# yozhijk/capsaicin

Measured on AMD Instinct MI355X. Metric: Mrays/sec (primary+secondary), cornell_box 1080p 64spp, higher is better.
Workload: dtype f32; 1 GPU; cornell_box.obj 1920x1080 64spp depth=8 (reference shading: Lambert + directional light + sky), tile-sharded over 1 GPU(s); triangles=32, bvh_depth=8, parallelism=tiles1, exchange=none

## Files before the change

### capsaicin_amd/capi.py

```python
import ctypes as C
import os
import subprocess

import numpy as np

_PKG = os.path.dirname(os.path.abspath(__file__))
_ROOT = os.path.dirname(_PKG)
LIB_PATH = os.path.join(_PKG, "libcapsaicin_hip.so")
if os.environ.get("CAP_LIB_VARIANT"):
    LIB_PATH = os.path.join(_PKG, "variants", "libcapsaicin_hip_%s.so" % os.environ["CAP_LIB_VARIANT"])

RENDER_AOV = 1
RENDER_EXT_MATERIALS = 2
RENDER_STAGE_TIMERS = 4
RENDER_GBUFFER_FEEDBACK = 8
RENDER_LOWRES_INDIRECT = 16

BUF_GBUFFER_GEO, BUF_DIRECT, BUF_ALBEDO, BUF_NORMAL_DEPTH, BUF_INDIRECT, BUF_COMBINED, BUF_ACCUM_SUM, BUF_ACCUM_MEAN, BUF_INDIRECT_LOWRES = range(9)


class CapError(RuntimeError):
    pass


# ... 502 lines not shown
        t = np.ascontiguousarray(rgba8, np.uint8)
        assert t.size == 256 * 256 * 4
        _check(lib().cap_bluenoise_upload(self.ctx, _p(t)), "cap_bluenoise_upload")

    def upload_materials(self, materials):
        m = np.ascontiguousarray(materials, np.float32).reshape(-1, 12)
        _check(lib().cap_materials_upload(self.ctx, _p(m), m.shape[0]), "cap_materials_upload")

    BVH_BUILD_AUTO, BVH_BUILD_LBVH, BVH_BUILD_SAH, BVH_BUILD_PLOC, BVH_BUILD_SAH_DEVICE = 0, 1, 2, 3, 4

    def set_bvh_build(self, mode):
        _check(lib().cap_set_bvh_build(self.ctx, mode), "cap_set_bvh_build")

    def build_bvh(self):
        _check(lib().cap_bvh_build(self.ctx), "cap_bvh_build")
        return self.bvh_info()

    def update_vertices(self, positions=None, normals=None, texcoords=None):
        ptrs, flags, keep = vertex_update_args(self._vertex_count, positions, normals, texcoords)
        if flags:
            import torch
            dev = torch.device("cuda", self.device)
            for a in keep:
                if a.device != dev:
                    raise CapError("update_vertices: tensors must be on %s, got %s" % (dev, a.device))
            torch.cuda.current_stream(dev).synchronize()
        _check(lib().cap_scene_update_vertices(self.ctx, ptrs[0], ptrs[1], ptrs[2], flags), "cap_scene_update_vertices")

    def refit_bvh(self):
        info = RefitInfo()
        _check(lib().cap_bvh_refit(self.ctx, C.byref(info)), "cap_bvh_refit")
        return info

    def bvh_info(self):
        bi = BvhInfo()
        _check(lib().cap_bvh_info(self.ctx, C.byref(bi)), "cap_bvh_info")
        return bi

    def bvh_readback(self):
        bi = self.bvh_info()
        nodes = np.zeros((bi.node_count, 16), np.float32)
        leaves = np.zeros(bi.triangle_count, np.uint32)
        _check(lib().cap_bvh_readback(self.ctx, _p(nodes), _p(leaves)), "cap_bvh_readback")
        return nodes, leaves

    def bvh_wide_readback(self):
        info = np.zeros(3, np.uint32)
        _check(lib().cap_bvh_wide_readback(self.ctx, None, None, _p(info)), "cap_bvh_wide_readback")
        nodes = np.zeros((int(info[0]), 20), np.uint32)
        src = np.zeros(max(1, self.bvh_info().triangle_count), np.uint32)
        _check(lib().cap_bvh_wide_readback(self.ctx, _p(nodes), _p(src), _p(info)), "cap_bvh_wide_readback")
        return nodes, src[:self.bvh_info().triangle_count], int(info[1]), int(info[2])

    def bvh_wide_info(self):
        info = np.zeros(3, np.uint32)
        _check(lib().cap_bvh_wide_readback(self.ctx, None, None, _p(info)), "cap_bvh_wide_readback")
        return int(info[0]), int(info[1]), int(info[2])

    def set_camera(self, cam):
        _check(lib().cap_camera_set(self.ctx, C.byref(cam)), "cap_camera_set")

    def set_prev_camera(self, cam):
        _check(lib().cap_prev_camera_set(self.ctx, C.byref(cam)), "cap_prev_camera_set")

    def set_resolution(self, width, height):
        _check(lib().cap_set_resolution(self.ctx, width, height), "cap_set_resolution")
        self.width, self.height = width, height

    def set_shard(self, index, count):
        _check(lib().cap_set_shard(self.ctx, index, count), "cap_set_shard")

    def set_traversal(self, mode):
        _check(lib().cap_set_traversal(self.ctx, mode), "cap_set_traversal")

    DEBUG_QUEUE_CAPACITY_DIV, DEBUG_WIDE_DEPTH_LIMIT, DEBUG_WIDE_IN_USE, DEBUG_FAIL_LANE1, DEBUG_LANES_USED = 1, 2, 3, 4, 5
    DEBUG_QUEUE_CANARY_FILL, DEBUG_QUEUE_CANARY_BEHIND, DEBUG_QUEUE_CANARY_USED, DEBUG_SELFTEST_DIV, DEBUG_NEE_PAIRS = 6, 7, 8, 9, 10
    DEBUG_SELFTEST_SHADE_UNARY, DEBUG_SELFTEST_SHADE_DIV2, DEBUG_SHADE_TAME = 11, 12, 13
    DEBUG_CAMERA_CULL = 14
    DEBUG_MARK_FORM = 15
    DEBUG_SAMPLE_TABLE = 16
    DEBUG_SELFTEST_SAMPLE_TABLE = 17
    DEBUG_CAMERA_TABLE = 18
    DEBUG_SELFTEST_CAMERA_TABLE = 19

    def debug_set(self, key, value):
        _check(lib().cap_debug_set(self.ctx, key, value), "cap_debug_set")

    DEBUG_SWITCH_BASE = 64

    def debug_switch(self, name, value):
        i = lib().cap_debug_switch_index(name.encode())
        if i < 0:
            raise CapError("unknown switch %s" % name)
        self.debug_set(self.DEBUG_SWITCH_BASE + i, 0xFFFFFFFFFFFFFFFF if value is None else int(value))

    def debug_get(self, key):
        v = _u64()
        _check(lib().cap_debug_get(self.ctx, key, C.byref(v)), "cap_debug_get")
        return int(v.value)

    def set_batch_paths(self, n):
        _check(lib().cap_set_batch_paths(self.ctx, n), "cap_set_batch_paths")

    def render(self, frame_begin, n_frames, num_bounces, flags=0):
        _check(lib().cap_render(self.ctx, frame_begin, n_frames, num_bounces, flags), "cap_render")

    def accum_reset(self):
        _check(lib().cap_accum_reset(self.ctx), "cap_accum_reset")

    def accum_import(self, sum_rgba, frames):
        a = np.ascontiguousarray(sum_rgba, np.float32)
        assert a.shape == (self.height, self.width, 4)
        _check(lib().cap_accum_import(self.ctx, _p(a), int(frames)), "cap_accum_import")

    def sync(self):
        _check(lib().cap_sync(self.ctx), "cap_sync")

    def readback(self, kind):
        if kind == BUF_INDIRECT_LOWRES:
            out = np.zeros((self.height // 2, self.width // 2, 4), np.float32)
        else:
            out = np.zeros((self.height, self.width, 4), np.float32)
        _check(lib().cap_readback(self.ctx, kind, _p(out)), "cap_readback")
        return out

    def stats(self):
        s = Stats()
        _check(lib().cap_stats_get(self.ctx, C.byref(s)), "cap_stats_get")
        return s

    def stats_reset(self):
        _check(lib().cap_stats_reset(self.ctx), "cap_stats_reset")

    RAY_FLAG_ACCEPT_FIRST_HIT, RAY_FLAG_CULL_BACK_FACING, RAY_FLAG_CULL_FRONT_FACING = 0x04, 0x10, 0x20

    def set_instance_masks(self, masks):
        if masks is None:
            _check(lib().cap_scene_set_instance_masks(self.ctx, None, len(self._tri_end)), "cap_scene_set_instance_masks")
            return
        m = np.ascontiguousarray(masks, np.uint8).reshape(-1)
        _check(lib().cap_scene_set_instance_masks(self.ctx, _p(m), m.size), "cap_scene_set_instance_masks")

    def trace_options(self, cull=None, mask=None, first_hit=False):
        if cull not in (None, "back", "front"):
            raise CapError('cull must be None, "back" or "front", got %r' % (cull,))
        if cull is None and mask is None and not first_hit:
            return None
        flags = {None: 0, "back": self.RAY_FLAG_CULL_BACK_FACING, "front": self.RAY_FLAG_CULL_FRONT_FACING}[cull]
        if first_hit:
            flags |= self.RAY_FLAG_ACCEPT_FIRST_HIT
        return TraceOptions(flags, 0 if mask is None else int(mask))

    MULTI_MAX_K, MULTI_CONTINUE = 16, 1

    def _stage_records(self, records, width, what):
        import torch
        dev = torch.device("cuda", self.device)
        if isinstance(records, np.ndarray):
            records = torch.from_numpy(np.ascontiguousarray(records, np.float32).reshape(-1, width)).to(dev)
        if records.dtype != torch.float32 or records.dim() != 2 or records.shape[1] != width or not records.is_contiguous() or records.device != dev:
            raise CapError("%s must be a contiguous (N, %d) float32 tensor on %s, got %s %s on %s"
                           % (what, width, dev, records.dtype, tuple(records.shape), records.device))
        return dev, records, records.shape[0]

    def _out(self, out, shape, dtype, dev):
        host_out = None
# ... 391 lines not shown
```

### capsaicin_amd/csrc/cap_context.h

```cpp
#pragma once

#include <array>
#include <string>
#include <utility>
#include <vector>

#include "../../include/capsaicin_hip.h"

#include "cap_kernels.h"

namespace cap
{
int fail(int code, const char* fmt, ...);

#define HIP_TRY(expr)                                                                                         \
    do                                                                                                        \
    {                                                                                                         \
        hipError_t e_ = (expr);                                                                               \
        if (e_ != hipSuccess) return fail(CAP_ERR_HIP, "%s failed: %s (%s:%d)", #expr, hipGetErrorString(e_), \
                                          __FILE__, __LINE__);                                                \
    } while (0)

template <typename T>
struct DevBuf
// ... 111 lines not shown
    DevBuf<float4>   shade_tris, tris_sorted, nodes, tri_raw, tri_box;
    DevBuf<float4>   nodes8, tris8;
    DevBuf<uint32_t> wide_src;
    DevBuf<uint32_t> wide_task, wide_alloc, wide_cnt;
    uint32_t         wide8_depth = 0, wide8_top = 0, wide8_nodes = 0;
    float            wide8_ms = 0.f;
    DevBuf<uint32_t> query_work, query_defer;
    DevBuf<uint8_t>  tri_mask;
    bool             tri_mask_on = false;
    DevBuf<float4>   inst_desc, inst_rec, inst_box, inst_tlas;
    DevBuf<uint32_t> inst_keys[2], inst_vals[2], inst_hist, inst_scan, inst_misc, inst_level_off;
    uint32_t         inst_count = 0, inst_top = 0, inst_nodes = 0;
    DevBuf<float2>   inst_near;
    DevBuf<uint32_t> inst_obj;
    bool             inst_obj_on = false;
    InstObject       scene_object_host{};
    DevBuf<InstObject> scene_object;
    std::vector<CapObjectInfo> obj_info;
    std::vector<uint32_t>      obj_node_base, obj_rec_base;
    uint32_t                   obj_count = 0, obj_max_depth = 0;
    DevBuf<float4>             forest_nodes, forest_tris;
    DevBuf<InstObject>         obj_table;
    DevBuf<float4>             obj_tri_raw, obj_tri_box;
    DevBuf<uint32_t>           obj_leaf_tri, obj_misc;
    DevBuf<float4>   fan_pairs, fan_singles;
    uint32_t         fan_pair_count = 0, fan_single_count = 0;
    DevBuf<float4>   fan_pairs_nee;
    uint32_t         fan_pair_nee_count = 0;
    std::vector<float>    fan_pairs_host;
    std::vector<uint32_t> light_tris_host;
    DevBuf<uint32_t> leaf_tri, keys0, keys1, vals0, vals1, hist, parent, flags, bvh_misc;
    DevBuf<float4>   ploc_boxes;
    DevBuf<uint32_t> ploc_ints;
    DevBuf<uint32_t> sahdev_words;
    CapBvhInfo       bvh_info{};
    bool             shade_tame = false;
    bool             bvh_ready = false;
    DevBuf<float>        pn_table;
    bool                 pn_ready = false;
    CapPseudonormalsInfo pn_info{};
    DevBuf<float4>       wn_table;
    bool                 wn_ready = false;
    CapWindingInfo       wn_info{};
    DevBuf<double>       wn_root;
    DevBuf<float4>       wi_inst, wi_top, wi_forest;
    DevBuf<double>       wi_top_sums, wi_obj_root, wi_reals;
    DevBuf<uint32_t>     wi_words, wi_count;
    bool                 wi_dirty = true, wi_forest_dirty = true;
    bool                 wi_built = false;
    bool                  bvh_stale = false;
    bool                  positions_host_stale = false;
    bool                  visits_built_known = false;
    double                refit_visits_built = 0.0;
    std::vector<uint32_t> wide_levels;
    DevBuf<float>         wide_boxes;
    DevBuf<double>        refit_sums;

    CapCameraData camera{}, prev_camera{};
    bool          camera_ready = false, prev_camera_ready = false;
    ScreenDev     screen{};
    uint64_t      max_batch_paths = 0;
    SwitchTable   sw{};
    uint32_t      debug_capacity_div = 1;
    uint32_t      debug_wide_depth_limit = 0;
    bool          debug_fail_lane = false;
    uint64_t      lane1_failed_paths = 0;
    uint32_t      lane1_failed_bounces = 0, lane1_retry_tick = 0;
    uint32_t      lanes_last_render = 0;
    uint32_t      last_class_capacity = 0;
    uint32_t      tri_ids_dense = 0;
    uint32_t      last_mark_form = 0;
    uint32_t      last_sample_table = 0;
    struct LastTerms
    {
        const FrameConst* frames = nullptr;
        uint32_t          n_slots = 0, num_bounces = 0, lane = 0;
    } last_terms;
    uint32_t      last_camera_table = 0;
    struct LastCamera
    {
        const FrameConst* frames = nullptr;
        uint32_t          n_slots = 0, n_groups = 0, lane = 0;
    } last_camera;
    uint32_t      last_cull_camera_pairs = 0;
    uint32_t      traversal_mode  = CAP_TRAVERSAL_AUTO;
    uint32_t      bvh_build_mode  = CAP_BVH_BUILD_AUTO;

    DevBuf<float4>     aov_geo, aov_nd, accum, image_tmp;
    DevBuf<uint64_t>   shaded_counter;
    struct Lane
    {
        hipStream_t      stream = nullptr;
        DevBuf<float4>   hits, q_org[2], q_dir[2], q_thr[2], s_org, s_dir, s_con, pl_color, pl_direct, pl_albedo;
        DevBuf<float4>   camera;
        DevBuf<float4>   terms;
        DevBuf<uint32_t> counters;
        DevBuf<uint32_t> stack_spill;
    } lane[2];
    hipStream_t stream2 = nullptr;
    hipEvent_t  lane_ev[2] = {nullptr, nullptr}, fork_ev = nullptr, join_ev = nullptr;
    static constexpr int kFrameRing = 4;
    DevBuf<FrameConst> frames_ring[kFrameRing];
    FrameConst*        frames_pinned[kFrameRing] = {nullptr, nullptr, nullptr, nullptr};
    size_t             frames_pinned_n[kFrameRing] = {0, 0, 0, 0};
    hipEvent_t         frames_event[kFrameRing] = {nullptr, nullptr, nullptr, nullptr};
    uint32_t           frames_next = 0;
    uint32_t           last_slots = 0;
    bool               aov_valid = false;
    bool               aov_lowres = false;
    uint32_t           aov_frame  = 0;
    uint64_t           frames_accumulated = 0;

    DevBuf<float4> post_in[4];
    DevBuf<float4> post_ihist[2], post_mhist[2], post_chist[2], post_prev_nd, post_itemp, post_temp[2], post_normals;
    uint32_t       post_w = 0, post_h = 0;
    int            post_last_dst = -1;

    void*           comm = nullptr;
    uint32_t        comm_rank = 0, comm_size = 0;
    bool            comm_local = false;
    DevBuf<float>   comm_send, comm_gathered, comm_image;
    hipEvent_t      comm_event = nullptr;

    CapStats               stats{};
    std::vector<TimedSpan> spans;
    std::vector<std::array<hipEvent_t, 6>> post_marks;
    std::vector<hipEvent_t> event_pool;
    std::vector<uint32_t*> pinned_pool;
    std::vector<std::pair<uint32_t*, BatchCounted>> pending;
    uint64_t*              pinned_shaded = nullptr;
};

namespace cap
{
struct AovPlanes
{
    const float4 *color, *direct, *albedo;
};

int        sync_and_collect(CapContext* c);
hipEvent_t get_event(CapContext* c);
CameraDev  camera_dev(const CapCameraData& cd);
SceneDev   scene_dev(const CapContext* c);
BvhDev     bvh_dev(const CapContext* c, const CapContext::Lane& lane);
AovPlanes  aov_planes(const CapContext* c);
int        trace_launch(const CapContext* c, const char* fmt, ...);
void       launch_texture_footprints(hipStream_t stream, const uint32_t* src, uint4* dst, uint32_t width, uint32_t height);
bool pair_ids_dense(const float* pairs, uint32_t pair_count, uint32_t single_count, uint32_t tri_count);
int  upload_fan_records(CapContext* c);
int  update_nee_pairs(CapContext* c);
int  ensure_positions_host(CapContext* c);
int  upload_light_table(CapContext* c);
int query_state(CapContext* c, const char* what);
int  winding_instances_ensure(CapContext* c, const char* what);
void winding_instances_release(CapContext* c);
}
```

### capsaicin_amd/csrc/cap_kernels.h

```cpp
#pragma once

#include "cap_device.h"

#include <cstdio>
#include <vector>

namespace cap
{
enum CapSwitch : uint32_t
{
    SW_NO_WIDE8 = 0,
    SW_LANE1_PRIORITY,
    SW_PLOC_RADIUS,
    SW_SAHDEV_LEAF,
    SW_WIDE_HOST_COLLAPSE,
    SW_TRACE_LAUNCHES,
    SW_NO_TWO_LANES,
    SW_LANE_SPLIT_MIN,
    SW_BLOCKS_PER_CU,
    SW_NO_CAMERA_CULL,
    SW_NO_ALBEDO_IN_W,
    SW_NO_INLINE_NEE,
    SW_NO_INLINE_PROBE,
    SW_NO_WAVE_RING,
    SW_ANY_REFILL,
    SW_PRIMARY_WIDE,
    SW_NO_PACKET,
    SW_NO_ANY_PROBE,
    SW_ANY_PROBE,
    SW_ANY_BLOCKS,
    SW_NO_PRIMARY_FUSE,
    SW_W8_REFILL,
    SW_W8_GRID,
    SW_AUTO_SAH_TRIANGLES,
    SW_NO_NEE_PAIR_CULL,
    SW_RAYGEN_KERNEL,
    SW_NO_PLANE_CODE,
    SW_SAMPLE_TABLE,
    SW_NO_CAMERA_TABLE,
    SW_COUNT
};
struct SwitchTable
{
    int64_t v[SW_COUNT];
    bool    on(CapSwitch k) const { return v[k] > 0; }
    int64_t get(CapSwitch k, int64_t dflt) const { return v[k] >= 0 ? v[k] : dflt; }
};

struct LaunchCfg
{
    hipStream_t stream;
    uint32_t    grid_blocks;
    uint32_t    stack_entries;
    uint32_t    cu_count = 0;
    uint32_t    any_no_probe = 0;
    const SwitchTable* sw = nullptr;
    bool    sw_on(CapSwitch k) const { return sw && sw->on(k); }
    int64_t sw_get(CapSwitch k, int64_t dflt) const { return sw ? sw->get(k, dflt) : dflt; }
};

template <auto K>
uint32_t resident_grid(const LaunchCfg& cfg, uint32_t want)
{
    static int per_cu = -1;
    if (per_cu < 0)
    {
        int n = 0;
        per_cu = (hipOccupancyMaxActiveBlocksPerMultiprocessor(&n, K, (int)kBlock, 0) == hipSuccess && n > 0) ? n : 0;
        if (cfg.sw_on(SW_TRACE_LAUNCHES)) fprintf(stderr, "[cap] resident workgroups per CU: %d\n", per_cu);
    }
    if (!cfg.cu_count || !per_cu) return want;
    const uint32_t cap = cfg.cu_count * (uint32_t)per_cu;
    return want < cap ? want : cap;
}
inline uint32_t queue_grid(const LaunchCfg& cfg, uint32_t max_count)
{
    uint32_t g = (max_count + kBlock - 1) / kBlock;
    if (g > cfg.grid_blocks) g = cfg.grid_blocks;
    return g ? g : 1;
}

void launch_trace_primary(const LaunchCfg& cfg, const BvhDev& bvh, const CameraDev& cam, const ScreenDev& screen,
                          const FrameConst* frames, uint32_t n_slots, float4* hits, uint32_t* work);
void launch_raygen_identity(const LaunchCfg& cfg, const CameraDev& cam, const ScreenDev& screen, const FrameConst* frames, uint32_t n_slots,
                            const RayQueue& q);
void launch_trace_closest(const LaunchCfg& cfg, const BvhDev& bvh, const RayQueue& q, uint32_t max_count, float4* hits);
void launch_trace_closest8(const LaunchCfg& cfg, const BvhDev& bvh, const RayQueue& q, uint32_t max_count, float4* hits, uint32_t* work);
void launch_trace_closest8_camera(const LaunchCfg& cfg, const BvhDev& bvh, const RayQueue& q, uint32_t max_count, float4* hits, uint32_t* work,
                                  const CameraDev& cam, const ScreenDev& screen, const FrameConst* frames, uint32_t n_slots);
void launch_trace_any(const LaunchCfg& cfg, const BvhDev& bvh, const ShadowQueue& q, uint32_t max_count, float4* target,
                      uint32_t pixels_padded, uint32_t n_slots, uint64_t* guard, uint32_t* work, bool mostly_unoccluded,
                      const FrameConst* frames, float4* code_plane = nullptr);

void launch_trace_any8_refill(const LaunchCfg& cfg, const BvhDev& bvh, const ShadowQueue& q, uint32_t max_count, float4* target, uint32_t pixels_padded,
                              uint32_t n_slots, uint64_t* guard, uint32_t* work, const FrameConst* frames);

struct QueryArgs
{
    const float4* rays;
    uint32_t      n;
    void*         out;
    uint32_t*     work;
    uint32_t*     defer;
    float         safe;
};
constexpr float kQuerySafeScale = 4.0f;
bool query8_stack_matches();
struct RayFilter;
void launch_query8(const LaunchCfg& cfg, const BvhDev& bvh, const QueryArgs& q, bool any, const RayFilter* f = nullptr, bool first_hit = false);
void launch_query_binary(const LaunchCfg& cfg, const BvhDev& bvh, const QueryArgs& q, bool any, bool deferred);
struct MultiArgs
{
    QueryArgs q;
    uint32_t  k;
    uint32_t* counts;
    uint32_t  resume;
};
constexpr uint32_t kMultiMaxK = 16;
uint32_t multi_bucket(uint32_t k);
void     launch_query8_multi(const LaunchCfg& cfg, const BvhDev& bvh, const MultiArgs& m, const RayFilter* f = nullptr);
void     launch_query_binary_multi(const LaunchCfg& cfg, const BvhDev& bvh, const MultiArgs& m, bool deferred, const RayFilter* f = nullptr);

// ... 50 lines not shown
void launch_closest_instances_multi(const LaunchCfg& cfg, const BvhDev& bvh, const ClosestInstMultiArgs& m, const TlasDev& tl, const RayFilter& f,
                                    uint32_t depth);

struct InstObject
{
    double   blo[3], bhi[3];
    int32_t  root;
    uint32_t reserved;
};
struct InstanceBuildArgs
{
    const float*      descs;
    uint32_t          n;
    const InstObject* objects;
    uint32_t          n_objects;
    const uint32_t*   object_index;
    float4*      rec;
    float4*      box;
    float4*      tlas;
    float2*      near;
    uint32_t*    keys[2];
    uint32_t*    vals[2];
    uint32_t*    hist;
    uint32_t*    scan;
    uint32_t*    misc;
};
constexpr uint32_t kTlasMaxLevels = 25;
uint32_t tlas_layout(uint32_t n, uint32_t level_off[kTlasMaxLevels], uint32_t* total);
void     launch_instances_build(hipStream_t stream, const InstanceBuildArgs& a);
struct TlasDev
{
    const float4*   rec;
    const float4*   tlas;
    const uint32_t* level_off;
    uint32_t        top;
};
void launch_query_instances(const LaunchCfg& cfg, const BvhDev& bvh, const QueryArgs& q, const TlasDev& tl, const RayFilter& f, int mode, uint32_t* inst_out,
                            uint32_t depth);
void launch_query_instances_multi(const LaunchCfg& cfg, const BvhDev& bvh, const MultiArgs& m, const TlasDev& tl, const RayFilter& f, uint32_t* inst_out,
                                  uint32_t depth);
struct ForestRelocArgs
{
    float4*  nodes;
    float4*  tris;
    uint32_t n_tris, node_base, rec_base, first_triangle;
};
void launch_forest_relocate(hipStream_t stream, const ForestRelocArgs& a);

struct ShadeArgs
{
    SceneDev          scene;
    CameraDev         cam;
    ScreenDev         screen;
    const FrameConst* frames;
    union
    {
        const float4* hits;
        const float4* sample_terms;
    };
    RayQueue          in;
    RayQueue          out;
    ShadowQueue       shadow;
    Planes            planes;
    uint32_t          n_slots;
    uint32_t          bounce;
    uint32_t          num_bounces;
    uint32_t          max_count;
    uint32_t          aov_slot;
    uint64_t*         shaded_counter;
    uint32_t*         work;
    FeedbackDev       fb;
    uint32_t          albedo_in_w;
    uint32_t          inline_nee;
    uint32_t          inline_probe;
    uint32_t          wave_ring;
    uint32_t          cull_camera_pairs;
    uint32_t          code_in_color;
};
constexpr float kCodePadding = 0.f, kCodeSky = 1.f, kCodeKd = 2.f, kCodeBlack = 3.f;
constexpr float kCodeLit = 4.f;
constexpr float kCameraCullPad = 2.0f;
void launch_shade(const LaunchCfg& cfg, const ShadeArgs& args, bool ext, bool feedback = false);
bool launch_primary_shade(const LaunchCfg& cfg, const BvhDev& bvh, const ShadeArgs& args, float4* hits, bool ext);
uint32_t launch_trace_shade(const LaunchCfg& cfg, const BvhDev& bvh, const ShadeArgs& args, bool ext, bool feedback = false, bool camera_head = false);
bool trace_shade_has_code_form(const BvhDev& bvh, const SceneDev& scene);
bool trace_shade_has_table_form(const BvhDev& bvh, const SceneDev& scene);
void launch_sample_terms(hipStream_t stream, const float2* bluenoise, const FrameConst* frames, uint32_t n_slots, uint32_t num_bounces, float4* table);
void launch_sample_terms_selftest(hipStream_t stream, const float2* bluenoise, const FrameConst* frames, uint32_t n_slots, uint32_t num_bounces,
                                  const float4* table, unsigned long long* out_device);

void launch_camera_vertices(const LaunchCfg& cfg, const BvhDev& bvh, const ShadeArgs& args, uint32_t rows, float4* tab_p, float4* tab_n,
                            unsigned long long* selftest_out = nullptr);

void launch_resolve(const LaunchCfg& cfg, const Planes& planes, uint32_t n_slots, uint32_t pixels_padded, float4* accum,
                    bool albedo_in_w = false, float kd_untextured = 0.0f, bool code_in_color = false);
void launch_untile(const LaunchCfg& cfg, const ScreenDev& screen, const float4* src, const float4* albedo, const float4* direct,
                   int plane_kind, float4* image);
void launch_tile(const LaunchCfg& cfg, const ScreenDev& screen, const float4* image, float4* dst);
void launch_untile4(const LaunchCfg& cfg, const ScreenDev& screen, const float4* s0, const float4* s1, const float4* s2, const float4* s3,
                    float4* d0, float4* d1, float4* d2, float4* d3);
void launch_tiles_mean(const LaunchCfg& cfg, const float4* accum, uint32_t pixels_padded, float4* dst);
void launch_assemble(const LaunchCfg& cfg, const ScreenDev& screen, const float4* gathered, uint32_t shard_count, float4* image,
                     size_t shard_stride = 0);
void launch_geo_aov(const LaunchCfg& cfg, const SceneDev& scene, const float4* hits_slot, uint32_t pixels_padded, float4* aov_geo);

struct BvhBuildArgs
{
    const float*    positions;
    const float*    normals;
    const float*    texcoords;
    const uint32_t* indices;
    const uint4*    tri_ids;
    const uint4*    mesh_offsets;
    uint32_t        tri_count;
    float4*         shade_tris;
    float4*         tris_sorted;
    float4*         nodes;
    uint32_t*       leaf_tri;
    float4*         tri_raw;
    float4*         tri_box;
    uint32_t*       keys[2];
    uint32_t*       vals[2];
    uint32_t*       hist;
    uint32_t*       parent;
    uint32_t*       flags;
    uint32_t*       bounds;
    uint32_t*       max_depth;
};
size_t bvh_radix_blocks(uint32_t n);
void   launch_bvh_build(hipStream_t stream, const BvhBuildArgs& a);
int    launch_bvh_sort(hipStream_t stream, const BvhBuildArgs& a);
size_t bvh_radix_scan_words(uint32_t n);
int    launch_radix_sort_pairs(hipStream_t stream, uint32_t* const keys[2], uint32_t* const vals[2], uint32_t n, uint32_t* hist, uint32_t* scan);
size_t bvh_scan_scratch_words(uint32_t total);
void   launch_exclusive_scan_u32(hipStream_t stream, uint32_t* v, uint32_t total, uint32_t* scratch);
struct PlocScratch
{
    float4*   boxes;
    uint32_t* ints;
};
int    launch_bvh_build_ploc(hipStream_t stream, const BvhBuildArgs& a, const PlocScratch& s, uint32_t radius);
size_t bvh_sah_device_scratch_words(uint32_t n);
int    launch_bvh_build_sah_device(hipStream_t stream, const BvhBuildArgs& a, const PlocScratch& s, uint32_t* scratch, uint32_t radius, uint32_t leaf);
void launch_bvh_setup(hipStream_t stream, const BvhBuildArgs& a);
void launch_bvh_finish_host(hipStream_t stream, const BvhBuildArgs& a);

void     launch_gather_wide(hipStream_t stream, const uint32_t* tri_src, const float4* tris_sorted, uint32_t n, float4* tris8);
struct WideCollapseArgs
{
    const float4*   bnodes;
    const uint32_t* count;
    uint32_t        n_tris, capacity;
    double          pad;
    uint32_t *      task, *alloc, *nodes8, *tri_src;
    uint32_t*       cnt;
    uint32_t        begin, end;
};
int      launch_wide_collapse(hipStream_t stream, WideCollapseArgs a, uint32_t* node_count, uint32_t* depth, uint32_t* top_nodes,
                          std::vector<uint32_t>* level_begin = nullptr);
struct PseudonormalArgs
{
    const float*    positions;
    const uint32_t* indices;
    const uint4*    tri_ids;
    const uint4*    mesh_offsets;
    uint32_t        tri_count;
    float*          table;
    uint32_t *      kx, *ky, *kz;
    uint32_t*       keys[2];
// ... 112 lines not shown
```

### capsaicin_amd/csrc/cap_shade.h

```cpp
#pragma once

#include "cap_exhaustive.h"
#include "cap_kernels.h"
#include "cap_reproject.h"
#include "cap_unscaled.h"

namespace cap
{
__device__ __forceinline__ void bluenoise4x4(const float2* tex, uint32_t x, uint32_t y, uint32_t count, float& s0, float& s1)
{
    const uint32_t px = (count % 16u) % 4u, py = (count % 16u) / 4u;
    const uint32_t sx = (x * 4u + px) % 256u, sy = (y * 4u + py) % 256u;
    const float2   t  = tex[sy * 256u + sx];
    const float    k  = 0.61803398875f * (float)(count / 16u);
    const float    a = t.x + k, b = t.y + k;
    s0 = a - floorf(a);
    s1 = b - floorf(b);
}

__device__ __forceinline__ v3 ortho_vector(v3 n)
{
    const bool  zn = fabsf(n.z) > 0.0f;
    const float a = zn ? n.z : n.y, b = zn ? n.y : n.x;
    const float k = sqrtf(fmaf(a, a, b * b));
// ... 48 lines not shown
    const bool fast = false;
#else
    const bool  fast = __ballot(!ortho_in_range(a, b, g)) == 0ull;
#endif
    float       q1, q2;
    if (fast)
        div2_unscaled(a, b, sqrt_pos(g), q1, q2);
    else
    {
        const float k = sqrtf(g);
        q1 = a / k, q2 = b / k;
    }
    v3       u = zn ? mk3(0.0f, -q1, q2) : mk3(q1, -q2, 0.0f);
    const v3 v = cross3(u, n);
    u          = cross3(n, v);
    const HemiTerms h = terms();
    const float     cos_theta = h.cos_theta, ca = h.ca, cb = h.cb;
    const v3    d = mk3(fmaf(n.x, cos_theta, fmaf(v.x, cb, u.x * ca)), fmaf(n.y, cos_theta, fmaf(v.y, cb, u.y * ca)),
                        fmaf(n.z, cos_theta, fmaf(v.z, cb, u.z * ca)));
    return fast ? normalize3_tame(d) : normalize3(d);
}
__device__ __forceinline__ v3 map_to_hemisphere_tame(float r1, float r2, v3 n)
{
    return hemisphere_dir_tame(n, [=] { return hemisphere_terms(r1, r2); });
}

__device__ __forceinline__ void oct_encode(v3 n, float& ox, float& oy)
{
    const float s = fabsf(n.x) + fabsf(n.y) + fabsf(n.z);
    n             = mk3(n.x / s, n.y / s, n.z / s);
    ox = n.x, oy = n.y;
    if (!(n.z >= 0.0f))
    {
        ox = (1.0f - fabsf(n.y)) * (n.x >= 0.0f ? 1.0f : -1.0f);
        oy = (1.0f - fabsf(n.x)) * (n.y >= 0.0f ? 1.0f : -1.0f);
    }
    ox = ox * 0.5f + 0.5f;
    oy = oy * 0.5f + 0.5f;
}

__device__ __forceinline__ uint32_t wrap_texel(float f, uint32_t n)
{
    const float m = f - floorf(f / (float)n) * (float)n;
    int         i = (int)m;
    if (i < 0) i = 0;
    if ((uint32_t)i >= n) i = 0;
    return (uint32_t)i;
}

__device__ __forceinline__ v3 sample_texture(const TextureDev& tex, float u, float v)
{
    const float    fx = fmaf(u, (float)tex.width, -0.5f), fy = fmaf(v, (float)tex.height, -0.5f);
    const float    x0f = floorf(fx), y0f = floorf(fy);
    const float    wx = fx - x0f, wy = fy - y0f;
    const uint32_t x0 = wrap_texel(x0f, tex.width), y0 = wrap_texel(y0f, tex.height);
    const uint4  fq   = reinterpret_cast<const uint4*>(tex.quads)[y0 * tex.width + x0];
    auto         rgba = [](uint32_t wd) { return make_uchar4((uint8_t)wd, (uint8_t)(wd >> 8), (uint8_t)(wd >> 16), (uint8_t)(wd >> 24)); };
    const uchar4 c00 = rgba(fq.x), c10 = rgba(fq.y), c01 = rgba(fq.z), c11 = rgba(fq.w);
    auto unorm8 = [](uint8_t b) {
        const float r = 1.0f / 255.0f, fb = (float)b, q = fb * r;
        return fmaf(fmaf(-q, 255.0f, fb), r, q);
    };
    auto           lerp2 = [&](uint8_t a00, uint8_t a10, uint8_t a01, uint8_t a11) {
        const float f00 = unorm8(a00), f10 = unorm8(a10), f01 = unorm8(a01), f11 = unorm8(a11);
        const float top = fmaf(f10 - f00, wx, f00);
        const float bot = fmaf(f11 - f01, wx, f01);
        return fmaf(bot - top, wy, top);
    };
    return mk3(lerp2(c00.x, c10.x, c01.x, c11.x), lerp2(c00.y, c10.y, c01.y, c11.y), lerp2(c00.z, c10.z, c01.z, c11.z));
}

__device__ __forceinline__ uint32_t wave_append(bool emit, uint32_t* counter)
{
    const unsigned long long mask = __ballot(emit);
    if (mask == 0ull) return 0;
    const uint32_t lane   = threadIdx.x & 63u;
    const uint32_t leader = (uint32_t)__ffsll((long long)mask) - 1u;
    uint32_t       base   = 0;
    if (lane == leader) base = atomicAdd(counter, (uint32_t)__popcll(mask));
    base = __shfl(base, (int)leader);
    return base + (uint32_t)__popcll(mask & ((1ull << lane) - 1ull));
}

struct ShadePre
{
    bool  valid;
    v3    L, I;
    float r1, r2;
    float r3, r4, r5, r6;
    float r1n, r2n;
    bool  indirect_on;
};

__device__ __forceinline__ void stage_frames(const ShadeArgs& a, FrameConst* lds_frames)
{
    const uint32_t  words = a.n_slots * (uint32_t)(sizeof(FrameConst) / 4);
    const uint32_t* src   = reinterpret_cast<const uint32_t*>(a.frames);
    uint32_t*       dst   = reinterpret_cast<uint32_t*>(lds_frames);
    for (uint32_t i = threadIdx.x; i < words; i += kBlock) dst[i] = src[i];
    __syncthreads();
}

#if defined(CAP_CHUNK_PLAIN)
constexpr bool kChunkLean = false;
#else
constexpr bool kChunkLean = true;
#endif

#pragma clang diagnostic push
#pragma clang diagnostic ignored "-Wuninitialized"
__device__ __forceinline__ float unread_f()
{
    float x;
    return x;
}
#pragma clang diagnostic pop
__device__ __forceinline__ v3 unread3() { return mk3(unread_f(), unread_f(), unread_f()); }

struct SlotSample
{
    uint32_t off;
    float    k;
};
__device__ __forceinline__ uint32_t bluenoise_offset(uint32_t count) { return (((count % 16u) / 4u) << 8) | ((count % 16u) % 4u); }
__device__ __forceinline__ float    bluenoise_shift(uint32_t count) { return 0.61803398875f * (float)(count / 16u); }
__device__ __forceinline__ uint32_t bluenoise_base(uint32_t x, uint32_t y) { return ((y & 63u) << 10) | ((x & 63u) << 2); }
__device__ __forceinline__ void     bluenoise_at(const float2* tex, uint32_t base, uint32_t off, float k, float& s0, float& s1)
{
    const float2 t = tex[base | off];
    const float  a = t.x + k, b = t.y + k;
    s0 = a - floorf(a);
    s1 = b - floorf(b);
}
template <bool FIRST, bool TAB = false>
__device__ __forceinline__ void stage_frames_samples(const ShadeArgs& a, FrameConst* lds_frames, SlotSample* lds_first)
{
    constexpr uint32_t kWords = (uint32_t)(sizeof(FrameConst) / 4);
    static_assert(kWords == 12 && offsetof(FrameConst, frame_count) == 8 && offsetof(FrameConst, pad1) == 28 && offsetof(FrameConst, pad2) == 44, "FrameConst layout");
    const uint32_t  words = (a.n_slots < kMaxFrameSlots ? a.n_slots : kMaxFrameSlots) * kWords;
    const uint32_t* src   = reinterpret_cast<const uint32_t*>(a.frames);
    uint32_t*       dst   = reinterpret_cast<uint32_t*>(lds_frames);
    for (uint32_t i = threadIdx.x; i < kMaxFrameSlots * kWords; i += kBlock)
    {
        uint32_t v = 0u;
        if (i < words)
        {
            const uint32_t sl = i / kWords, w = i - sl * kWords;
            v = src[i];
            if (!TAB && (w == 7u || w == 11u))
            {
                const uint32_t next = src[sl * kWords + 2u] * 25u + a.bounce + 1u;
                v = w == 7u ? bluenoise_offset(next) : f2u(bluenoise_shift(next));
            }
        }
        dst[i] = v;
    }
    if (FIRST && !TAB)
        for (uint32_t sl = threadIdx.x; sl < kMaxFrameSlots; sl += kBlock)
        {
            SlotSample ss = {0u, 0.0f};
            if (sl < a.n_slots)
            {
                const uint32_t count = a.frames[sl].frame_count * 25u + a.bounce;
                ss.off = bluenoise_offset(count), ss.k = bluenoise_shift(count);
            }
            lds_first[sl] = ss;
// ... 81 lines not shown
        }
    }
    return s;
}

__device__ __forceinline__ void wave_append2(bool& emit_ext, bool& emit_shadow, uint32_t* counter_pair, uint32_t& ext_slot,
                                             uint32_t& shadow_slot, uint32_t capacity, uint64_t* guard)
{
    const unsigned long long me = __ballot(emit_ext), ms = __ballot(emit_shadow);
    ext_slot = shadow_slot = 0;
    if ((me | ms) == 0ull) return;
    const uint32_t lane   = threadIdx.x & 63u;
    const uint32_t leader = (uint32_t)__ffsll((long long)(me | ms)) - 1u;
    uint32_t       lo = 0, hi = 0;
    if (lane == leader)
    {
        const unsigned long long add = ((unsigned long long)__popcll(ms) << 32) | (unsigned long long)__popcll(me);
        const unsigned long long old = atomicAdd(reinterpret_cast<unsigned long long*>(counter_pair), add);
        lo = (uint32_t)old, hi = (uint32_t)(old >> 32);
    }
    lo = __shfl(lo, (int)leader), hi = __shfl(hi, (int)leader);
    const unsigned long long below = (1ull << lane) - 1ull;
    ext_slot    = lo + (uint32_t)__popcll(me & below);
    shadow_slot = hi + (uint32_t)__popcll(ms & below);
    if (lo + (uint32_t)__popcll(me) > capacity || hi + (uint32_t)__popcll(ms) > capacity)
    {
        if (lane == leader)
        {
            atomicAdd((unsigned long long*)guard + 4, 1ull);
            guard[3] = ((uint64_t)lo << 32) | hi;
        }
        emit_ext    = emit_ext && ext_slot < capacity;
        emit_shadow = emit_shadow && shadow_slot < capacity;
    }
}

#ifdef CAP_STAMPS
static __device__ unsigned long long g_stamps[16];
struct Stamps
{
    unsigned long long last, acc[8], t_begin;
    __device__ void    start()
    {
        for (int i = 0; i < 8; ++i) acc[i] = 0;
        last    = __builtin_amdgcn_s_memtime();
        t_begin = __builtin_amdgcn_s_memrealtime();
    }
    __device__ void mark(int i, bool wait)
    {
#ifdef CAP_STAMPS_PHASES
        if (wait) __builtin_amdgcn_s_waitcnt(0);
        const unsigned long long now = __builtin_amdgcn_s_memtime();
        acc[i] += now - last;
        last = now;
#endif
    }
    __device__ void flush()
    {
        if ((threadIdx.x & 63u) == 0)
            for (int i = 0; i < 8; ++i) atomicAdd(&g_stamps[i], acc[i]);
    }
};
#define STAMP(st, i, wait) (st).mark(i, wait)
#else
struct Stamps
{
    __device__ void start() {}
    __device__ void flush() {}
};
#define STAMP(st, i, wait) ((void)0)
#endif

struct ProbeArgs
{
    const float4* rows  = nullptr;
    const float4* pairs = nullptr;
    uint32_t      k     = 0;
    float4*       ring_org = nullptr;
    float4*       ring_con = nullptr;
};
constexpr uint32_t kWaveRing = 128;
template <class C>
__device__ __forceinline__ void shade_vertex(const ShadeArgs& a, const float4* shade_tab, const ShadePre& pre, uint32_t klass,
                                             uint32_t pid, float4 hit, v3 thr, uint32_t& n_shaded, Stamps& st,
                                             const ProbeArgs probe = ProbeArgs(), uint32_t* n_probed = nullptr, uint32_t ring_head = 0,
                                             uint32_t* ring_n = nullptr)
{
    const uint32_t Ppad = a.screen.pixels_padded;
    const uint32_t slot = pid >> kPidShift, pl = pid & kPidMask;
    {
        const size_t plane_idx = (size_t)slot * Ppad + pl;
        bool         valid = pre.valid;
        if (valid && (slot >= a.n_slots || pl >= Ppad))
        {
            atomicAdd((unsigned long long*)a.shaded_counter + 1, 1ull);
            a.shaded_counter[3] = ((uint64_t)a.bounce << 32) | pid;
            valid = false;
        }
        const uint32_t gid = f2u(hit.z);

        bool   emit_shadow = false, emit_ext = false;
        v3     p = mk3(0, 0, 0), dir = mk3(0, 0, 0), contrib = mk3(0, 0, 0);
        if constexpr (C::LEAN) p = unread3(), dir = unread3(), contrib = unread3();

        if (C::FIRST && !valid)
        {
            a.planes.color[plane_idx]  = make_float4(0, 0, 0, 0);
            if (!C::CODE) a.planes.direct[plane_idx] = make_float4(0, 0, 0, 0);
            if (!C::CODE && !a.albedo_in_w) a.planes.albedo[plane_idx] = make_float4(0, 0, 0, 0);
        }
        if (valid && gid == kInvalidId)
        {
            if (C::FIRST)
            {
                a.planes.color[plane_idx]  = make_float4(0.f, 0.f, 0.f, 1.f);
                if (!C::CODE) a.planes.direct[plane_idx] = make_float4(0.7f, 0.7f, 0.85f, 1.f);
                if (!C::CODE && !a.albedo_in_w) a.planes.albedo[plane_idx] = make_float4(1.f, 1.f, 1.f, 1.f);
                if (slot == a.aov_slot) a.planes.aov_normal_depth[pl] = make_float4(0.f, 0.f, 0.f, 0.f);
            }
            else
            {
                if (C::SKY_RMW)
                {
                    const float4 cur = a.planes.color[plane_idx];
                    a.planes.color[plane_idx] = make_float4(cur.x + thr.x * 0.7f, cur.y + thr.y * 0.7f, cur.z + thr.z * 0.85f, cur.w);
                }
                else
                {
                    float* c = reinterpret_cast<float*>(a.planes.color + plane_idx);
                    atomicAdd(c + 0, thr.x * 0.7f);
                    atomicAdd(c + 1, thr.y * 0.7f);
                    atomicAdd(c + 2, thr.z * 0.85f);
                }
            }
        }
        else if (valid)
        {
            ++n_shaded;
            const float4* tab = shade_tab + kShadeRec * (size_t)gid;
            const float4  s0 = tab[0], s1 = tab[1], s2 = tab[2], s3 = tab[3], s4 = tab[4], s5 = tab[5];
            const float   u = hit.x, v = hit.y, w = (1.0f - u) - v;
            auto          mix = [&](float c0, float c1, float c2) { return fmaf(c2, v, fmaf(c1, u, c0 * w)); };
            const v3      nm = mk3(mix(s3.x, s4.x, s5.x), mix(s3.y, s4.y, s5.y), mix(s3.z, s4.z, s5.z));
            const v3      n  = C::TAME ? normalize3_tame(nm) : normalize3(nm);
            p = mk3(mix(s0.x, s1.x, s2.x), mix(s0.y, s1.y, s2.y), mix(s0.z, s1.z, s2.z));
            v3       kd   = mk3(a.scene.kd_untextured, a.scene.kd_untextured, a.scene.kd_untextured);
            uint32_t inst = 0;
            if (a.scene.texture_count != 0 || (C::FIRST && slot == a.aov_slot))
            {
                const float4 idf   = tab[6];
                inst               = f2u(idf.x);
                const uint32_t tex = f2u(idf.z);
                if (tex != kInvalidId && tex < a.scene.texture_count)
                {
                    const float tu = mix(s0.w, s2.w, s4.w), tv = mix(s1.w, s3.w, s5.w);
                    const v3    c  = sample_texture(a.scene.textures[tex], tu, 1.0f - tv);
                    kd             = mk3(pow22_c(c.x), pow22_c(c.y), pow22_c(c.z));
                }
            }
            const bool black = kd.x < 1e-5f && kd.y < 1e-5f && kd.z < 1e-5f;
            if (C::FIRST)
            {
                if (C::CODE)
                    a.planes.color[plane_idx] = make_float4(0.f, 0.f, 0.f, black ? kCodeBlack : kCodeKd);
                else
                {
                    a.planes.color[plane_idx]  = make_float4(0.f, 0.f, 0.f, 1.f);
                    a.planes.direct[plane_idx] = make_float4(0.f, 0.f, 0.f, a.albedo_in_w ? (black ? kCodeBlack : kCodeKd) : 1.f);
                }
                if (!C::CODE && !a.albedo_in_w) a.planes.albedo[plane_idx] = black ? make_float4(0.f, 0.f, 0.f, 0.f) : make_float4(kd.x, kd.y, kd.z, 1.f);
                if (slot == a.aov_slot)
                {
                    float4 nd = make_float4(0.f, 0.f, 0.f, 0.f);
                    if (!black)
                    {
                        oct_encode(n, nd.x, nd.y);
                        nd.z = (float)inst;
                        nd.w = length3(mk3(a.cam.position[0], a.cam.position[1], a.cam.position[2]) - p);
                    }
                    a.planes.aov_normal_depth[pl] = nd;
                }
            }
            bool reused = false;
            if (C::FB && !C::FIRST && !black)
            {
                const uint32_t W = a.screen.width, H = a.screen.height;
                const f2       puv = image_plane_uv(a.fb.prev_cam, p);
                if (puv.x >= 0.0f && puv.y >= 0.0f && puv.x <= 1.0f && puv.y <= 1.0f)
                {
                    const f2    pxy        = uv_to_xy(puv, W, H);
                    const float prev_depth = ldi(Img{a.fb.prev_normal_depth, W, H}, (int)pxy.x, (int)pxy.y).w;
                    const float cur_depth =
                        length3(p - mk3(a.fb.prev_cam.position[0], a.fb.prev_cam.position[1], a.fb.prev_cam.position[2]));
                    if (!(fabsf(prev_depth - cur_depth) / cur_depth > 0.05f))
                    {
                        reused        = true;
                        const v3 hc   = sample_bilinear(Img{a.fb.color_history, W, H}, puv);
                        const float4 cur = a.planes.color[plane_idx];
                        a.planes.color[plane_idx] = make_float4(cur.x + thr.x * hc.x, cur.y + thr.y * hc.y, cur.z + thr.z * hc.z, cur.w);
                    }
                }
            }
            if (!black && !reused)
            {
                const float ndl = fmaxf(0.0f, dot3(n, pre.L));
                v3          c   = mk3(((pre.I.x * kd.x) * kInvPi) * ndl, ((pre.I.y * kd.y) * kInvPi) * ndl, ((pre.I.z * kd.z) * kInvPi) * ndl);
                if (c.x != 0.0f || c.y != 0.0f || c.z != 0.0f)
                {
                    emit_shadow = true;
                    contrib     = C::FIRST ? c : thr * c;
                }
                const bool more = a.bounce < a.num_bounces;
                if (!C::TAME || more)
                {
                    if constexpr (C::TAB)
                        dir = hemisphere_dir_tame(n, [&] { return HemiTerms{pre.r1, pre.r2, pre.r1n}; });
                    else
                        dir = C::TAME ? map_to_hemisphere_tame(pre.r1, pre.r2, n) : map_to_hemisphere(pre.r1, pre.r2, n);
                    const float ndd = dot3(n, dir);
                    const float pdf = C::TAME ? div_unscaled(fmaxf(0.0f, ndd), kPi) : fmaxf(0.0f, ndd) / kPi;
                    if (!(pdf < 1e-5f))
                    {
                        const float fn = kInvPi * fmaxf(ndd, 0.0f);
                        const float f  = C::TAME ? div_unscaled(fn, pdf) : fn / pdf;
                        thr            = thr * f;
                        if (!C::FIRST) thr = thr * kd;
                        emit_ext = more && (!C::FIRST || pre.indirect_on);
                    }
                }
            }
        }

        if (C::PROBE)
        {
            if (probe.rows != nullptr)
            {
                const Ray    sr  = make_ray(p, pre.L, kRayEps, kRayFar);
                const uint32_t ps = valid ? slot : 0u;
                const float4   pa = probe.rows[2u * ps], pb = probe.rows[2u * ps + 1u];
                const bool   occluded = pair_occludes_pre(sr, probe.pairs, probe.k, pa, pb);
                if (emit_shadow && occluded) emit_shadow = false, ++*n_probed;
            }
        }
        uint32_t ei, si;
        STAMP(st, 2, true);
        wave_append2(emit_ext, emit_shadow, a.out.count + klass * kCounterStride, ei, si, a.out.class_capacity, a.shaded_counter);
        STAMP(st, 3, true);
        ei += klass * a.out.class_capacity;
        si += klass * a.shadow.class_capacity;
        if (C::PROBE && probe.ring_org != nullptr)
        {
            const unsigned long long ms = __ballot(emit_shadow);
            if (emit_shadow)
            {
                const uint32_t lane_ = threadIdx.x & 63u;
                const uint32_t pos   = (ring_head + *ring_n + (uint32_t)__popcll(ms & ((1ull << lane_) - 1ull))) & (kWaveRing - 1u);
                probe.ring_org[pos]  = make_float4(p.x, p.y, p.z, u2f(pid));
                probe.ring_con[pos]  = make_float4(contrib.x, contrib.y, contrib.z, 0.0f);
            }
            *ring_n += (uint32_t)__popcll(ms);
            __builtin_amdgcn_fence(__ATOMIC_RELEASE, "wavefront");
        }
        else if (emit_shadow)
        {
            a.shadow.org_tmin[si]    = make_float4(p.x, p.y, p.z, u2f(pid));
            a.shadow.contrib_pid[si] = make_float4(contrib.x, contrib.y, contrib.z, C::CODE ? kCodeKd : 0.0f);
        }
        if (emit_ext)
        {
            a.out.org_tmin[ei] = make_float4(p.x, p.y, p.z, C::CARRY ? pre.r1n : kRayEps);
            a.out.dir_tmax[ei] = make_float4(dir.x, dir.y, dir.z, C::CARRY ? pre.r2n : kRayFar);
            a.out.thr_pid[ei]  = make_float4(thr.x, thr.y, thr.z, u2f(pid));
        }
    }
}

struct ExtBsdf
{
    v3    f;
    float pdf_spec, pdf_diff;
};

__device__ __forceinline__ float lum3(v3 c) { return fmaf(c.z, 0.114f, fmaf(c.y, 0.587f, c.x * 0.299f)); }

struct ExtView
{
    float cos_o, lam_o;
};
__device__ __forceinline__ ExtView ext_view(float a2, v3 nf, v3 wo)
{
    ExtView w;
    w.cos_o = dot3(nf, wo);
    w.lam_o = w.cos_o + sqrtf(fmaf(1.0f - a2, w.cos_o * w.cos_o, a2));
    return w;
}
__device__ __forceinline__ ExtBsdf ext_bsdf(v3 kd, v3 ks, float a2, v3 nf, v3 wo, v3 wi, const ExtView& vw)
{
    const float cos_i = dot3(nf, wi);
    const v3    h     = normalize3(wo + wi);
    const float cos_h = dot3(nf, h), woh = dot3(wo, h);
    const float dd    = fmaf(cos_h * cos_h, a2 - 1.0f, 1.0f);
    const float pdd   = kPi * dd * dd;
    const float lam_i = cos_i + sqrtf(fmaf(1.0f - a2, cos_i * cos_i, a2));
#if defined(CAP_EXT_DIAG) && CAP_EXT_DIAG == 3
    const float spec  = 0.0f * (vw.cos_o + woh);
#else
    const float spec  = a2 / (pdd * (vw.lam_o * lam_i));
#endif
    ExtBsdf     r;
    r.f        = mk3(kd.x * kInvPi + ks.x * spec, kd.y * kInvPi + ks.y * spec, kd.z * kInvPi + ks.z * spec);
    r.pdf_spec = (a2 * cos_h) / (pdd * (4.0f * woh));
    r.pdf_diff = cos_i * kInvPi;
    return r;
}

struct ExtTables
{
    const MaterialDev* materials  = nullptr;
    const float*       light_cdf  = nullptr;
    const float4*      light_rec  = nullptr;
};
constexpr uint32_t kExtLightsMax = 32;

template <bool FIRST, bool INLINE = false>
__device__ __forceinline__ void shade_vertex_ext(const ShadeArgs& a, const float4* shade_tab, const ShadePre& pre, uint32_t klass,
                                                 uint32_t pid, float4 hit, v3 thr,
                                                 v3 d, uint32_t& n_shaded, const BvhDev* bvh = nullptr, v3 acc = mk3(0.f, 0.f, 0.f),
                                                 const ExtTables tabs = ExtTables())
{
    const uint32_t Ppad = a.screen.pixels_padded;
    const uint32_t slot = pid >> kPidShift, pl = pid & kPidMask;
    const size_t   plane_idx = (size_t)slot * Ppad + pl;
    bool           valid = pre.valid;
    if (valid && (slot >= a.n_slots || pl >= Ppad))
    {
        atomicAdd((unsigned long long*)a.shaded_counter + 1, 1ull);
        a.shaded_counter[3] = ((uint64_t)a.bounce << 32) | pid;
        valid = false;
    }
    const uint32_t gid = f2u(hit.z);
    bool  emit_shadow = false, emit_ext = false;
    v3    p = mk3(0, 0, 0), dir = mk3(0, 0, 0), contrib = mk3(0, 0, 0), sdir = mk3(0, 0, 1), first_ke = mk3(0, 0, 0);
    float stmax = 0.0f;

    if (FIRST && !valid)
    {
        a.planes.color[plane_idx]  = make_float4(0, 0, 0, 0);
        a.planes.direct[plane_idx] = make_float4(0, 0, 0, 0);
        if (!a.albedo_in_w) a.planes.albedo[plane_idx] = make_float4(0, 0, 0, 0);
    }
    if (valid && gid == kInvalidId)
// ... 182 lines not shown
```

### capsaicin_amd/csrc/context.hip

```cpp
#include <algorithm>
#include <cmath>
#include <cstdarg>
#include <cstdio>
#include <cstdlib>
#include <cstring>

#include "cap_context.h"
#include "cap_near.h"
#include "cap_wide.h"
#include "query_ranges.h"

namespace
{
thread_local std::string g_error;
}

namespace cap
{
int fail(int code, const char* fmt, ...)
{
    char    buf[512];
    va_list ap;
    va_start(ap, fmt);
    vsnprintf(buf, sizeof(buf), fmt, ap);
// ... 149 lines not shown

int trace_launch(const CapContext* c, const char* fmt, ...)
{
    if (!c->sw.on(SW_TRACE_LAUNCHES)) return CAP_OK;
    va_list ap;
    va_start(ap, fmt);
    fputs("[cap] ", stderr);
    vfprintf(stderr, fmt, ap);
    va_end(ap);
    fputs(" ... ", stderr);
    fflush(stderr);
    hipError_t e = hipStreamSynchronize(c->stream);
    fprintf(stderr, "%s\n", hipGetErrorString(e));
    fflush(stderr);
    return e == hipSuccess ? CAP_OK : CAP_ERR_HIP;
}
}

namespace
{
void update_screen(CapContext* c, uint32_t w, uint32_t h, uint32_t shard_index, uint32_t shard_count)
{
    ScreenDev& s  = c->screen;
    s.width       = w;
    s.height      = h;
    s.tiles_x     = (w + kTileDim - 1) / kTileDim;
    s.tiles_y     = (h + kTileDim - 1) / kTileDim;
    s.tile_count  = s.tiles_x * s.tiles_y;
    s.shard_index = shard_index;
    s.shard_count = shard_count ? shard_count : 1;
    const uint32_t max_local = (s.tile_count + s.shard_count - 1) / s.shard_count;
    s.local_tiles   = s.tile_count > s.shard_index ? (s.tile_count - s.shard_index + s.shard_count - 1) / s.shard_count : 0;
    s.pixels_padded = max_local * kTilePixels;
    tile_div_setup(s.tiles_x, s.tiles_x_mul, s.tiles_x_shift);
    c->frames_accumulated = 0;
    c->aov_valid = false;
}

template <size_t N, class Launch>
int count_on_device(CapContext* c, unsigned long long (&h)[N], Launch launch)
{
    DevBuf<unsigned long long> d;
    HIP_TRY(d.ensure(N));
    HIP_TRY(hipMemsetAsync(d.p, 0, sizeof(h), c->stream));
    launch(d.p);
    HIP_TRY(hipGetLastError());
    HIP_TRY(hipMemcpyAsync(h, d.p, sizeof(h), hipMemcpyDeviceToHost, c->stream));
    HIP_TRY(hipStreamSynchronize(c->stream));
    return CAP_OK;
}
}

__global__ __launch_bounds__(256) void k_texture_footprints(const uint32_t* src, uint4* dst, uint32_t width, uint32_t height)
{
    const size_t i = (size_t)blockIdx.x * 256 + threadIdx.x;
    if (i >= (size_t)width * height) return;
    const uint32_t y = (uint32_t)(i / width), x = (uint32_t)(i - (size_t)y * width);
    const uint32_t x1 = x + 1 == width ? 0 : x + 1, y1 = y + 1 == height ? 0 : y + 1;
    dst[i] = make_uint4(src[(size_t)y * width + x], src[(size_t)y * width + x1], src[(size_t)y1 * width + x], src[(size_t)y1 * width + x1]);
}

void cap::launch_texture_footprints(hipStream_t stream, const uint32_t* src, uint4* dst, uint32_t width, uint32_t height)
{
    const size_t texels = (size_t)width * height;
    hipLaunchKernelGGL(k_texture_footprints, dim3((unsigned)((texels + 255) / 256)), dim3(256), 0, stream, src, dst, width, height);
}

extern "C" {

const char* cap_last_error(void) { return g_error.c_str(); }
void cap_set_error_(const char* msg) { g_error = msg ? msg : ""; }

int cap_device_count(void)
{
    int n = 0;
    if (hipGetDeviceCount(&n) != hipSuccess) return 0;
    return n;
}

static const char* const kSwitchNames[SW_COUNT] = {
    "CAP_NO_WIDE8", "CAP_LANE1_PRIORITY", "CAP_PLOC_RADIUS", "CAP_SAHDEV_LEAF", "CAP_WIDE_HOST_COLLAPSE", "CAP_TRACE_LAUNCHES", "CAP_NO_TWO_LANES",
    "CAP_LANE_SPLIT_MIN", "CAP_BLOCKS_PER_CU", "CAP_NO_CAMERA_CULL", "CAP_NO_ALBEDO_IN_W", "CAP_NO_INLINE_NEE", "CAP_NO_INLINE_PROBE", "CAP_NO_WAVE_RING",
    "CAP_ANY_REFILL", "CAP_PRIMARY_WIDE", "CAP_NO_PACKET", "CAP_NO_ANY_PROBE", "CAP_ANY_PROBE", "CAP_ANY_BLOCKS", "CAP_NO_PRIMARY_FUSE", "CAP_W8_REFILL",
    "CAP_W8_GRID", "CAP_AUTO_SAH_TRIANGLES", "CAP_NO_NEE_PAIR_CULL", "CAP_RAYGEN_KERNEL", "CAP_NO_PLANE_CODE", "CAP_SAMPLE_TABLE", "CAP_NO_CAMERA_TABLE"};

static void switches_from_environment(SwitchTable& t)
{
    for (uint32_t k = 0; k < SW_COUNT; ++k)
    {
        const char* e = getenv(kSwitchNames[k]);
        t.v[k]        = -1;
        if (!e) continue;
        char*           end = nullptr;
        const long long v   = strtoll(e, &end, 10);
        t.v[k]              = (end != e && v >= 0) ? v : 1;
    }
    if (getenv("CAP_BVH_BINARY") && t.v[SW_NO_WIDE8] < 0) t.v[SW_NO_WIDE8] = 1;
}

int cap_debug_switch_index(const char* name)
{
    for (uint32_t k = 0; name && k < SW_COUNT; ++k)
        if (strcmp(name, kSwitchNames[k]) == 0) return (int)k;
    return -1;
}

extern "C" int cap_debug_tile_divmod(uint32_t tiles_x, const uint32_t* n, uint64_t count, uint32_t* quotient, uint32_t* remainder)
{
    if (!tiles_x || !n || !quotient || !remainder) return CAP_ERR_INVALID_ARG;
    uint32_t mul, shift;
    tile_div_setup(tiles_x, mul, shift);
    for (uint64_t k = 0; k < count; ++k)
    {
        quotient[k]  = tile_div(n[k], mul, shift);
        remainder[k] = n[k] - quotient[k] * tiles_x;
    }
    return CAP_OK;
}

int cap_debug_pair_ids_dense(const float* pair_records, uint32_t pair_count, uint32_t single_count, uint32_t tri_count)
{
    if (!pair_records && pair_count) return 0;
    return pair_ids_dense(pair_records, pair_count, single_count, tri_count) ? 1 : 0;
}

int cap_debug_query_ranges(uint64_t n, uint32_t count, const uint64_t* base, const uint64_t* stride, const uint32_t* align)
{
    static const char* const names[4] = {"range 0", "range 1", "range 2", "range 3"};
    if (count > 4 || (count && (!base || !stride || !align))) return fail(CAP_ERR_INVALID_ARG, "cap_debug_query_ranges: at most 4 ranges, no NULL array");
    QueryRange r[4];
    for (uint32_t i = 0; i < count; ++i)
    {
        if (!align[i] || (align[i] & (align[i] - 1u))) return fail(CAP_ERR_INVALID_ARG, "cap_debug_query_ranges: align[%u] is not a power of two", i);
        r[i] = QueryRange{names[i], (uintptr_t)base[i], stride[i], align[i], stride[i] != 0};
    }
    char msg[256];
    return query_ranges_ok("cap_debug_query_ranges", n, r, count, msg, sizeof(msg)) ? CAP_OK : fail(CAP_ERR_INVALID_ARG, "%s", msg);
}

int cap_debug_closest_instance_bound(const float* transform, const float* box_lo, const float* box_hi, const float* point, float best_dist2,
                                     float* world_to_object, float* g, float* xw, float* slack, uint32_t* skip)
{
    if (!transform || !box_lo || !box_hi || !point) return fail(CAP_ERR_INVALID_ARG, "cap_debug_closest_instance_bound: NULL input");
    double m[12], w[12], wd[12], A[12], nA, kappa, blo[3], bhi[3];
    float  wf[12];
    bool   live = true;
    for (int k = 0; k < 12; ++k) m[k] = (double)transform[k], live = live && finite_d(m[k]);
    for (int k = 0; k < 3; ++k) blo[k] = (double)box_lo[k], bhi[k] = (double)box_hi[k];
    live = instance_inverse(m, live, w, wf, wd, A, nA, kappa, (float)CAP_INSTANCE_MAX_CONDITION);
    const float gi = live ? near_sigma_min_bound(w) : 0.0f, xi = live ? near_world_extent(m, blo, bhi) : 0.0f;
    const float pmax = fmaxf(fabsf(point[0]), fmaxf(fabsf(point[1]), fabsf(point[2])));
    const float sl   = near_slack(pmax, xi);
    float       ox, oy, oz;
    near_to_object(wf, point[0], point[1], point[2], ox, oy, oz);
    const float bd2 = box_dist2(ox, oy, oz, box_lo[0], box_lo[1], box_lo[2], box_hi[0], box_hi[1], box_hi[2]);
    if (world_to_object)
        for (int k = 0; k < 12; ++k) world_to_object[k] = wf[k];
    if (g) *g = gi;
    if (xw) *xw = xi;
    if (slack) *slack = sl;
    if (skip) *skip = live && near_skip(bd2, near_bound2_object(sqrtf(best_dist2), sl, gi)) ? 1u : 0u;
    return CAP_OK;
}

int cap_ctx_create(int device_id, void* hip_stream, CapContext** out_ctx)
{
    if (!out_ctx) return fail(CAP_ERR_INVALID_ARG, "cap_ctx_create: out_ctx is NULL");
// ... 169 lines not shown
    }
}

int cap_debug_get(CapContext* c, uint32_t key, uint64_t* value)
{
    if (!c || !value) return fail(CAP_ERR_INVALID_ARG, "cap_debug_get: NULL argument");
    switch (key)
    {
    case CAP_DEBUG_QUEUE_CAPACITY_DIV: *value = c->debug_capacity_div; return CAP_OK;
    case CAP_DEBUG_WIDE_DEPTH_LIMIT: *value = c->debug_wide_depth_limit; return CAP_OK;
    case CAP_DEBUG_FAIL_LANE1: *value = c->debug_fail_lane ? 1u : 0u; return CAP_OK;
    case CAP_DEBUG_LANES_USED: *value = c->lanes_last_render; return CAP_OK;
    case CAP_DEBUG_SELFTEST_DIV:
    {
        HIP_TRY(hipSetDevice(c->device));
        unsigned long long h[3];
        if (int e = count_on_device(c, h, [&](unsigned long long* d) { launch_div_selftest(c->stream, d); })) return e;
        const unsigned long long expected = (0x7f7fffffull - 0x00800000ull + 1ull) + (1ull << 30);
        if (h[2] != expected) return fail(CAP_ERR_HIP, "cap_debug_get: the division self-test compared %llu of %llu cases", h[2], expected);
        *value = h[0] + h[1];
        return CAP_OK;
    }
    case CAP_DEBUG_SELFTEST_SHADE_UNARY:
    case CAP_DEBUG_SELFTEST_SHADE_DIV2:
    {
        HIP_TRY(hipSetDevice(c->device));
        unsigned long long h[2];
        if (int e = count_on_device(c, h, [&](unsigned long long* d) { launch_shade_forms_selftest(c->stream, d, key == CAP_DEBUG_SELFTEST_SHADE_DIV2 ? 1u : 0u); }))
            return e;
        const unsigned long long floats_sqrt = 0x7f7fffffull - ((127ull - 96ull) << 23) + 1ull;
        const unsigned long long least = key == CAP_DEBUG_SELFTEST_SHADE_DIV2 ? (1ull << 30) : 2ull * floats_sqrt + 3ull + (5ull << 23) + 1ull + 0x40000001ull + (8ull << 23);
        if (h[1] < least) return fail(CAP_ERR_HIP, "cap_debug_get: the shading self-test compared %llu of at least %llu cases", h[1], least);
        *value = h[0];
        return CAP_OK;
    }
    case CAP_DEBUG_SHADE_TAME:
        if (!c->bvh_ready || c->bvh_stale) return fail(CAP_ERR_STATE, "cap_debug_get: BVH not built or stale");
        *value = c->shade_tame ? 1u : 0u;
        return CAP_OK;
    case CAP_DEBUG_CAMERA_CULL: *value = c->last_cull_camera_pairs; return CAP_OK;
    case CAP_DEBUG_MARK_FORM:
        if (!c->bvh_ready) return fail(CAP_ERR_STATE, "cap_debug_get: BVH not built");
        *value = ((uint64_t)c->last_mark_form << 8) | c->tri_ids_dense;
        return CAP_OK;
    case CAP_DEBUG_SAMPLE_TABLE: *value = c->last_sample_table; return CAP_OK;
    case CAP_DEBUG_SELFTEST_SAMPLE_TABLE:
    {
        const CapContext::LastTerms& lt = c->last_terms;
        if (!c->last_sample_table || !lt.frames) return fail(CAP_ERR_STATE, "cap_debug_get: the last cap_render built no sample table");
        HIP_TRY(hipSetDevice(c->device));
        if (sync_and_collect(c) != CAP_OK) return CAP_ERR_HIP;
        unsigned long long h[2];
        if (int e = count_on_device(c, h, [&](unsigned long long* d) {
                launch_sample_terms_selftest(c->stream, c->bluenoise.p, lt.frames, lt.n_slots, lt.num_bounces, c->lane[lt.lane].terms.p, d);
            }))
            return e;
        const unsigned long long expected = (unsigned long long)lt.n_slots * lt.num_bounces * 4096ull;
        if (h[1] != expected) return fail(CAP_ERR_HIP, "cap_debug_get: the sample table self-test compared %llu of %llu entries", h[1], expected);
        *value = (h[0] << 32) | (expected >> 12);
        return CAP_OK;
    }
    case CAP_DEBUG_CAMERA_TABLE: *value = c->last_camera_table; return CAP_OK;
    case CAP_DEBUG_SELFTEST_CAMERA_TABLE:
    {
        const CapContext::LastCamera& lc = c->last_camera;
        if (!c->last_camera_table || !lc.frames) return fail(CAP_ERR_STATE, "cap_debug_get: the last cap_render built no camera table");
        HIP_TRY(hipSetDevice(c->device));
        if (sync_and_collect(c) != CAP_OK) return CAP_ERR_HIP;
        ShadeArgs sa{};
        sa.scene = scene_dev(c), sa.cam = camera_dev(c->camera), sa.screen = c->screen, sa.frames = lc.frames, sa.n_slots = lc.n_slots;
        sa.cull_camera_pairs = c->last_cull_camera_pairs;
        LaunchCfg     cfg{c->stream, (uint32_t)c->cu_count * 6u, 0u, (uint32_t)c->cu_count};
        float4* const tab = c->lane[lc.lane].camera.p;
        unsigned long long h[2];
        if (int e = count_on_device(c, h, [&](unsigned long long* d) {
                launch_camera_vertices(cfg, bvh_dev(c, c->lane[lc.lane]), sa, lc.n_slots, tab, tab + (size_t)lc.n_groups * c->screen.pixels_padded, d);
            }))
            return e;
        const unsigned long long expected = (unsigned long long)lc.n_slots * c->screen.pixels_padded;
        if (h[1] != expected) return fail(CAP_ERR_HIP, "cap_debug_get: the camera table self-test compared %llu of %llu entries", h[1], expected);
        *value = (h[0] << 32) | ((uint64_t)lc.n_groups << 16) | lc.n_slots;
        return CAP_OK;
    }
    case CAP_DEBUG_NEE_PAIRS:
        if (!c->bvh_ready) return fail(CAP_ERR_STATE, "cap_debug_get: BVH not built");
        *value = ((uint64_t)(c->fan_pairs_nee.p ? c->fan_pair_nee_count : c->fan_pair_count) << 32) | c->fan_pair_count;
        return CAP_OK;
    case CAP_DEBUG_QUEUE_CANARY_BEHIND: return canary_count(c, true, value);
    case CAP_DEBUG_QUEUE_CANARY_USED: return canary_count(c, false, value);
    case CAP_DEBUG_WIDE_IN_USE:
        if (!c->bvh_ready) return fail(CAP_ERR_STATE, "cap_debug_get: BVH not built");
        *value = bvh_dev(c, c->lane[0]).wide8_ok;
        return CAP_OK;
    default:
        if (key >= CAP_DEBUG_SWITCH_BASE && key < CAP_DEBUG_SWITCH_BASE + SW_COUNT)
        {
            *value = (uint64_t)c->sw.v[key - CAP_DEBUG_SWITCH_BASE];
            return CAP_OK;
        }
        return fail(CAP_ERR_INVALID_ARG, "cap_debug_get: unknown key %u", key);
    }
}

int cap_set_bvh_build(CapContext* c, uint32_t mode)
{
    if (!c) return fail(CAP_ERR_INVALID_ARG, "cap_set_bvh_build: ctx is NULL");
    if (mode > CAP_BVH_BUILD_SAH_DEVICE) return fail(CAP_ERR_INVALID_ARG, "cap_set_bvh_build: unknown mode %u", mode);
    c->bvh_build_mode = mode;
    return CAP_OK;
}

int cap_set_traversal(CapContext* c, uint32_t mode)
{
    if (!c) return fail(CAP_ERR_INVALID_ARG, "cap_set_traversal: ctx is NULL");
    if (mode > CAP_TRAVERSAL_EXHAUSTIVE) return fail(CAP_ERR_INVALID_ARG, "cap_set_traversal: unknown mode %u", mode);
    c->traversal_mode = mode;
    return CAP_OK;
}

int cap_accum_reset(CapContext* c)
{
    if (!c) return fail(CAP_ERR_INVALID_ARG, "cap_accum_reset: ctx is NULL");
    HIP_TRY(hipSetDevice(c->device));
    if (c->accum.p) HIP_TRY(hipMemsetAsync(c->accum.p, 0, sizeof(float4) * c->accum.n, c->stream));
    c->frames_accumulated = 0;
    return CAP_OK;
}

int cap_accum_import(CapContext* c, const float* sum_rgba, uint64_t frames)
{
    if (!c || !sum_rgba) return fail(CAP_ERR_INVALID_ARG, "cap_accum_import: NULL argument");
    if (!c->screen.width) return fail(CAP_ERR_STATE, "cap_accum_import: resolution not set");
    HIP_TRY(hipSetDevice(c->device));
    if (sync_and_collect(c) != CAP_OK) return CAP_ERR_HIP;
    const size_t npix = (size_t)c->screen.width * c->screen.height;
    HIP_TRY(c->image_tmp.ensure(npix));
    HIP_TRY(c->accum.ensure(c->screen.pixels_padded));
    HIP_TRY(hipMemcpyAsync(c->image_tmp.p, sum_rgba, sizeof(float4) * npix, hipMemcpyHostToDevice, c->stream));
    LaunchCfg cfg{c->stream, (uint32_t)c->cu_count * 8u, 32};
    launch_tile(cfg, c->screen, c->image_tmp.p, c->accum.p);
    HIP_TRY(hipGetLastError());
    HIP_TRY(hipStreamSynchronize(c->stream));
    c->frames_accumulated = frames;
    return CAP_OK;
}

int cap_sync(CapContext* c)
{
    if (!c) return fail(CAP_ERR_INVALID_ARG, "cap_sync: ctx is NULL");
    HIP_TRY(hipSetDevice(c->device));
    return sync_and_collect(c);
}

int cap_readback(CapContext* c, CapBufferKind kind, float* dst)
{
    if (!c || !dst) return fail(CAP_ERR_INVALID_ARG, "cap_readback: NULL argument");
    if (!c->screen.width) return fail(CAP_ERR_STATE, "cap_readback: resolution not set");
    HIP_TRY(hipSetDevice(c->device));
    if (sync_and_collect(c) != CAP_OK) return CAP_ERR_HIP;
    const size_t npix = (size_t)c->screen.width * c->screen.height;
    HIP_TRY(c->image_tmp.ensure(npix));
    HIP_TRY(hipMemsetAsync(c->image_tmp.p, 0, sizeof(float4) * npix, c->stream));
    LaunchCfg cfg{c->stream, (uint32_t)c->cu_count * 8u, 32};
    const bool is_aov = kind <= CAP_BUF_COMBINED || kind == CAP_BUF_INDIRECT_LOWRES;
    if (is_aov && !c->aov_valid) return fail(CAP_ERR_STATE, "cap_readback: no frame rendered with CAP_RENDER_AOV");
    if (!is_aov && !c->accum.p) return fail(CAP_ERR_STATE, "cap_readback: nothing rendered");
// ... 83 lines not shown
```

### capsaicin_amd/csrc/ctx_render.hip

```cpp
#include <algorithm>
#include <cmath>
#include <cstring>
#include <memory>

#include "cap_context.h"
#include "cap_wide.h"

namespace
{
constexpr double kPrimaryWideTrianglesPerPixel = 2.0;
constexpr uint64_t kAnyRefillTreeBytes = ~0ull;

struct StageTimer
{
    CapContext* c;
    TimedSpan   sp;
    bool        on;
    StageTimer(CapContext* ctx, int stage, bool enabled = true, int also = ST_NONE) : c(ctx), on(enabled)
    {
        if (!on) return;
        sp.stage = stage;
        sp.also  = also;
        sp.a     = get_event(c);
        sp.b     = get_event(c);
        (void)hipEventRecord(sp.a, c->stream);
    }
    ~StageTimer()
    {
        if (!on) return;
        (void)hipEventRecord(sp.b, c->stream);
        c->spans.push_back(sp);
    }
};

FrameConst frame_const(uint32_t frame_count, bool lowres_indirect)
{
    FrameConst f{};
    halton23(frame_count, f.jitter_x, f.jitter_y);
    f.frame_count = frame_count;
    f.lowres_sel = lowres_indirect ? (4u | (((frame_count % 4u) / 2u) << 1) | ((frame_count % 4u) % 2u)) : 0u;
    const float t = 2.0f * 3.14f * (float)(frame_count % 4096) / 4096.0f;
    float       st, ct;
    sincos_c(t, st, ct);
    const v3 dir = normalize3(mk3(40.0f * st, 100.0f, 40.0f * ct));
    f.light_dir[0] = dir.x, f.light_dir[1] = dir.y, f.light_dir[2] = dir.z;
    f.light_intensity[0] = 1.0f * (2.0f * 14.0f + 0.0f);
    f.light_intensity[1] = 1.0f * (2.0f * 12.0f + 0.0f);
    f.light_intensity[2] = 1.0f * (2.0f * 10.0f + (2.0f + 2.0f * ct));
    return f;
}

struct BatchPolicy
{
    uint32_t slots;
    bool     two_lanes;
    bool     lane1_failed_before;
};

BatchPolicy batch_policy(const CapContext* c, uint32_t n_frames, uint32_t num_bounces, uint32_t flags, bool tree_path)
{
    const uint32_t Ppad = c->screen.pixels_padded;
    uint64_t       budget = c->max_batch_paths ? c->max_batch_paths : (uint64_t)64 << 20;
    if (!c->max_batch_paths && (uint64_t)n_frames * Ppad > budget)
    {
        const uint64_t big       = (uint64_t)128 << 20;
        const uint64_t big_slots = std::max<uint64_t>(1, std::min<uint64_t>(big / std::max(1u, Ppad), kMaxFrameSlots));
        bool           room      = c->lane[0].pl_color.n >= big_slots * Ppad && (!tree_path || c->lane[1].pl_color.n >= big_slots * Ppad);
        if (!room)
        {
            size_t free_b = 0, total_b = 0;
            room = hipMemGetInfo(&free_b, &total_b) == hipSuccess && free_b > 3u * big_slots * Ppad * 256u;
        }
        if (room) budget = big;
    }
    uint32_t       slots  = (uint32_t)std::max<uint64_t>(1, std::min<uint64_t>(budget / std::max(1u, Ppad), kMaxFrameSlots));
    slots                 = std::min(slots, n_frames);
    const bool no_two_lanes = c->sw.on(SW_NO_TWO_LANES);
    bool two_lanes = !no_two_lanes && tree_path && c->bvh_info.stack_entries != 0 && !(flags & CAP_RENDER_GBUFFER_FEEDBACK) &&
                     !(flags & CAP_RENDER_LOWRES_INDIRECT) && n_frames >= 2;
    if (two_lanes && slots >= n_frames)
    {
        const uint64_t split_min = (uint64_t)c->sw.get(SW_LANE_SPLIT_MIN, (int64_t)4 << 20);
        if ((uint64_t)n_frames * Ppad >= split_min)
            slots = (n_frames + 1) / 2;
        else
            two_lanes = false;
    }
    if ((flags & CAP_RENDER_STAGE_TIMERS) || c->sw.on(SW_TRACE_LAUNCHES)) two_lanes = false;
    const bool failed_before =
        two_lanes && c->lane1_failed_paths && (uint64_t)slots * Ppad >= c->lane1_failed_paths && num_bounces >= c->lane1_failed_bounces;
    return BatchPolicy{slots, two_lanes, failed_before};
}

struct RenderPlan
{
    uint32_t frame_begin = 0, n_frames = 0, num_bounces = 0, flags = 0;
    bool     ext = false, feedback = false, lowres = false, aov = false, stage_timers = false;
    bool     tree_path = false, fused = false;
    uint32_t stack_entries = 0;
    uint32_t slots = 0, n_batches = 0;
    bool     two_lanes = false;
    bool     lane1_failed_before = false;
    uint32_t blocks_per_cu = 0;
    bool     sample_table = false;
    bool     camera_table = false;
    std::vector<uint32_t> slot_group, group_first, batch_groups;
    uint32_t camera_groups = 0;
    uint32_t cull_camera_pairs = 0, albedo_in_w = 0, code_in_color = 0, inline_nee = 0, inline_probe = 0;
    bool     ring_form = false;
    uint64_t valid_pixels = 0;
    uint32_t wave_ring = 0;
    bool     camera_head = false, any_refill = false, primary_wide = false;
};

struct Batch
{
    uint32_t          lane, first, ns, index, groups;
    bool              last;
    const FrameConst* frames;
};

struct LaneSizes
{
    size_t planes, queues, rings, counters, terms, camera;
};

LaneSizes lane_sizes(const CapContext* c, const RenderPlan& p)
{
    LaneSizes z;
    z.planes = (size_t)p.slots * c->screen.pixels_padded;
    z.queues = z.planes + (size_t)kQueueClasses * 64;
    z.rings = std::max(z.queues, (size_t)std::max(c->cu_count, 1) * 8 * (kBlock / 64) * 128);
    z.counters = CounterLayout{p.num_bounces}.total();
    z.terms = p.sample_table ? (size_t)p.slots * p.num_bounces * 4096 : 0;
    z.camera = 2 * (size_t)p.camera_groups * c->screen.pixels_padded;
    return z;
}

bool lane_grows(const CapContext::Lane& L, const LaneSizes& z) { return L.pl_color.n < z.planes || L.counters.n < z.counters || L.terms.n < z.terms || L.camera.n < z.camera; }

int ensure_lane(CapContext* c, CapContext::Lane& L, const LaneSizes& z)
{
    for (DevBuf<float4>* b : {&L.hits, &L.q_org[0], &L.q_org[1], &L.q_dir[0], &L.q_dir[1], &L.q_thr[0], &L.q_thr[1], &L.s_dir})
        HIP_TRY(b->ensure(z.queues));
    for (DevBuf<float4>* b : {&L.s_org, &L.s_con}) HIP_TRY(b->ensure(z.rings));
    for (DevBuf<float4>* b : {&L.pl_color, &L.pl_direct, &L.pl_albedo}) HIP_TRY(b->ensure(z.planes));
    HIP_TRY(L.counters.ensure(z.counters));
    if (z.terms) HIP_TRY(L.terms.ensure(z.terms));
    if (z.camera) HIP_TRY(L.camera.ensure(z.camera));
    if (c->lane[0].stack_spill.n) HIP_TRY(L.stack_spill.ensure(c->lane[0].stack_spill.n));
    return CAP_OK;
}

int ensure_frame_buffers(CapContext* c)
{
    HIP_TRY(c->aov_geo.ensure(c->screen.pixels_padded));
    HIP_TRY(c->aov_nd.ensure(c->screen.pixels_padded));
    if (!c->shaded_counter.p)
    {
        HIP_TRY(c->shaded_counter.ensure(kGuardWords));
        HIP_TRY(hipMemsetAsync(c->shaded_counter.p, 0, kGuardWords * sizeof(uint64_t), c->stream));
    }
    if (!c->accum.p || c->accum.n < c->screen.pixels_padded)
    {
        HIP_TRY(c->accum.ensure(c->screen.pixels_padded));
        HIP_TRY(hipMemsetAsync(c->accum.p, 0, sizeof(float4) * c->screen.pixels_padded, c->stream));
        c->frames_accumulated = 0;
    }
    return CAP_OK;
}

int ensure_lane_streams(CapContext* c)
{
    if (!c->stream2)
    {
        if (c->sw.v[SW_LANE1_PRIORITY] >= 0)
            HIP_TRY(hipStreamCreateWithPriority(&c->stream2, hipStreamNonBlocking, (int)c->sw.v[SW_LANE1_PRIORITY]));
        else
            HIP_TRY(hipStreamCreateWithFlags(&c->stream2, hipStreamNonBlocking));
    }
    c->lane[1].stream = c->stream2;
    for (hipEvent_t* e : {&c->lane_ev[0], &c->lane_ev[1], &c->fork_ev, &c->join_ev})
        if (!*e) HIP_TRY(hipEventCreateWithFlags(e, hipEventDisableTiming));
    return CAP_OK;
}

void jitter_groups(RenderPlan& p)
{
    p.slot_group.resize(p.n_frames), p.group_first.assign(p.n_frames, 0u);
    for (uint32_t done = 0; done < p.n_frames; done += p.slots)
    {
        const uint32_t ns = std::min(p.slots, p.n_frames - done);
        uint32_t       ng = 0;
        for (uint32_t s = 0; s < ns; ++s)
        {
            float sx, sy, gx, gy;
            halton23(p.frame_begin + done + s, sx, sy);
            uint32_t g = 0;
            for (; g < ng; ++g)
            {
                halton23(p.frame_begin + done + p.group_first[done + g], gx, gy);
                if (memcmp(&gx, &sx, sizeof(float)) == 0 && memcmp(&gy, &sy, sizeof(float)) == 0) break;
            }
            if (g == ng) p.group_first[done + ng++] = s;
            p.slot_group[done + s] = g;
        }
        p.batch_groups.push_back(ng);
        p.camera_groups = std::max(p.camera_groups, ng);
    }
}

bool cull_camera_pairs(const CapContext* c)
{
    const bool no_cull = c->sw.on(SW_NO_CAMERA_CULL);
    auto dotf = [](const float* x, const float* y) { return x[0] * y[0] + x[1] * y[1] + x[2] * y[2]; };
    const CapCameraData& cd = c->camera;
    const float skew = std::max({std::fabs(dotf(cd.right, cd.up)), std::fabs(dotf(cd.right, cd.forward)), std::fabs(dotf(cd.up, cd.forward)),
                                 std::fabs(dotf(cd.right, cd.right) - 1.f), std::fabs(dotf(cd.up, cd.up) - 1.f),
                                 std::fabs(dotf(cd.forward, cd.forward) - 1.f)});
    const double f = cd.focal_length, sx = cd.sensor_size[0], sy = cd.sensor_size[1];
    const double shift_x = (double)skew * c->screen.width * (f / sx + 1.0 + sy / (2.0 * sx) + (sx + sy) / (4.0 * f));
    const double shift_y = (double)skew * c->screen.height * (f / sy + 1.0 + sx / (2.0 * sy) + (sx + sy) / (4.0 * f));
    const bool   ortho   = skew < 1e-4f && shift_x <= 0.125 * (double)kCameraCullPad && shift_y <= 0.125 * (double)kCameraCullPad;
    return ortho && !no_cull;
}

int plan_render(const CapContext* c, uint32_t frame_begin, uint32_t n_frames, uint32_t num_bounces, uint32_t flags, RenderPlan& p)
{
    if (!c->bvh_ready) return fail(CAP_ERR_STATE, "cap_render: call cap_bvh_build first");
    if (c->bvh_stale) return fail(CAP_ERR_STATE, "cap_render: vertices changed; call cap_bvh_refit or cap_bvh_build");
    if (!c->camera_ready || !c->bluenoise_ready || !c->screen.width) return fail(CAP_ERR_STATE, "cap_render: camera, blue noise and resolution must be set");
    p.frame_begin = frame_begin, p.n_frames = n_frames, p.num_bounces = num_bounces, p.flags = flags;
    p.ext = (flags & CAP_RENDER_EXT_MATERIALS) != 0, p.feedback = (flags & CAP_RENDER_GBUFFER_FEEDBACK) != 0;
    p.lowres = (flags & CAP_RENDER_LOWRES_INDIRECT) != 0, p.aov = (flags & CAP_RENDER_AOV) != 0, p.stage_timers = (flags & CAP_RENDER_STAGE_TIMERS) != 0;
    const bool ext = p.ext, feedback = p.feedback, lowres = p.lowres;
    if (ext && !c->materials_ready) return fail(CAP_ERR_STATE, "cap_render: CAP_RENDER_EXT_MATERIALS needs cap_materials_upload (one material per mesh)");
    static_assert(sizeof(MaterialDev) == sizeof(CapMaterial), "material layouts must match");
    if (num_bounces > 255) return fail(CAP_ERR_INVALID_ARG, "cap_render: num_bounces %u exceeds 255", num_bounces);
    if (!n_frames) return CAP_OK;
    HIP_TRY(hipSetDevice(c->device));
    if (feedback)
    {
        if (ext) return fail(CAP_ERR_UNSUPPORTED, "cap_render: CAP_RENDER_GBUFFER_FEEDBACK is defined for the reference shading model only");
        if (n_frames != 1) return fail(CAP_ERR_INVALID_ARG, "cap_render: CAP_RENDER_GBUFFER_FEEDBACK renders one frame per call (n_frames is %u)", n_frames);
        if (!c->prev_camera_ready) return fail(CAP_ERR_STATE, "cap_render: CAP_RENDER_GBUFFER_FEEDBACK needs cap_prev_camera_set");
    }
    if (lowres)
    {
        if (ext) return fail(CAP_ERR_UNSUPPORTED, "cap_render: CAP_RENDER_LOWRES_INDIRECT is defined for the reference shading model only");
        if (n_frames != 1) return fail(CAP_ERR_INVALID_ARG, "cap_render: CAP_RENDER_LOWRES_INDIRECT renders one frame per call (n_frames is %u)", n_frames);
        if ((c->screen.width | c->screen.height) & 1u) return fail(CAP_ERR_INVALID_ARG, "cap_render: CAP_RENDER_LOWRES_INDIRECT needs even width and height (%ux%u)", c->screen.width, c->screen.height);
    }
    if (c->traversal_mode == CAP_TRAVERSAL_EXHAUSTIVE && c->tri_count > 4096)
        return fail(CAP_ERR_UNSUPPORTED, "cap_render: exhaustive traversal refused for %u triangles", c->tri_count);
    p.tree_path     = c->traversal_mode == CAP_TRAVERSAL_EXHAUSTIVE ? false : !(c->traversal_mode == CAP_TRAVERSAL_AUTO && c->tri_count <= kExhaustiveMax);
    p.stack_entries = p.tree_path ? c->bvh_info.stack_entries : 0u;
    p.fused         = p.stack_entries == 0;
    const bool fused = p.fused;

    const BatchPolicy policy = batch_policy(c, n_frames, num_bounces, flags, p.tree_path);
    p.slots = policy.slots, p.two_lanes = policy.two_lanes, p.lane1_failed_before = policy.lane1_failed_before;
    p.n_batches = (n_frames + p.slots - 1) / p.slots;
    p.blocks_per_cu = fused ? 6u : (p.stack_entries <= 32 ? 5u : 2u);
    if (c->sw.v[SW_BLOCKS_PER_CU] >= 0) p.blocks_per_cu = (uint32_t)std::max<int64_t>(1, c->sw.v[SW_BLOCKS_PER_CU]);

    const BvhDev   bvh   = bvh_dev(c, c->lane[0]);
    const SceneDev scene = scene_dev(c);
    p.sample_table = fused && !ext && !feedback && num_bounces >= 1 && c->sw.get(SW_SAMPLE_TABLE, 1) != 0 && trace_shade_has_table_form(bvh, scene);
    p.cull_camera_pairs = cull_camera_pairs(c) ? 1u : 0u;
    const bool no_albedo_w = c->sw.on(SW_NO_ALBEDO_IN_W);
    p.albedo_in_w = (!no_albedo_w && !feedback && !lowres && !p.aov && (ext || scene.texture_count == 0)) ? 1u : 0u;
    const bool no_plane_code = c->sw.on(SW_NO_PLANE_CODE);
    p.code_in_color = (p.albedo_in_w && fused && !ext && !no_plane_code && trace_shade_has_code_form(bvh, scene)) ? 1u : 0u;
    const bool no_inline_nee = c->sw.on(SW_NO_INLINE_NEE);
    p.inline_nee = (ext && fused && !no_inline_nee) ? 1u : 0u;
    const bool no_inline_probe = c->sw.on(SW_NO_INLINE_PROBE);
    const bool probe_form      = !ext && !feedback && fused && !no_inline_probe;
    p.inline_probe = (probe_form && c->tri_count <= kExhaustiveMax && bvh.fan_pair_count >= 1 && bvh.fan_pair_count <= kExhaustiveMax / 2) ? 1u : 0u;
    const bool no_wave_ring = c->sw.on(SW_NO_WAVE_RING);
    p.ring_form = probe_form && !no_wave_ring;
    p.camera_table = p.sample_table && p.code_in_color && p.ring_form && !c->sw.on(SW_NO_CAMERA_TABLE) && c->debug_capacity_div <= 1;
    if (p.camera_table) jitter_groups(p);

    for (uint32_t lt = 0; lt < c->screen.local_tiles; ++lt)
    {
        const uint32_t gt = lt * c->screen.shard_count + c->screen.shard_index;
        const uint32_t ty = gt / c->screen.tiles_x, tx = gt % c->screen.tiles_x;
        const uint32_t w = std::min(kTileDim, c->screen.width - tx * kTileDim), h = std::min(kTileDim, c->screen.height - ty * kTileDim);
        p.valid_pixels += (uint64_t)w * h;
    }
    return CAP_OK;
}

int ensure_lanes(CapContext* c, RenderPlan& p)
{
    const uint32_t  Ppad = c->screen.pixels_padded;
    const LaneSizes need = lane_sizes(c, p);
    if (lane_grows(c->lane[0], need) || !c->accum.p || c->accum.n < Ppad) HIP_TRY(hipStreamSynchronize(c->stream));
    if (ensure_lane(c, c->lane[0], need) != CAP_OK || ensure_frame_buffers(c) != CAP_OK) return CAP_ERR_HIP;
    if (p.lane1_failed_before)
    {
        size_t free_b = 0, total_b = 0;
        const bool room = hipMemGetInfo(&free_b, &total_b) == hipSuccess && free_b > (size_t)p.slots * Ppad * 256u;
        if (!room && (++c->lane1_retry_tick % 32u) != 0u)
        {
            p.two_lanes = false;
            ++c->stats.lane1_dropped;
        }
    }
    if (p.two_lanes)
    {
        if (lane_grows(c->lane[1], need))
        {
            HIP_TRY(hipStreamSynchronize(c->stream));
            if (c->stream2) HIP_TRY(hipStreamSynchronize(c->stream2));
        }
        if (c->debug_fail_lane || ensure_lane(c, c->lane[1], need) != CAP_OK || ensure_lane_streams(c) != CAP_OK)
        {
            (void)hipGetLastError();
            c->lane[1] = CapContext::Lane{};
            c->lane1_failed_paths = (uint64_t)p.slots * Ppad, c->lane1_failed_bounces = p.num_bounces;
            ++c->stats.lane1_dropped;
            p.two_lanes = false;
        }
    }
    return CAP_OK;
}

void plan_forms(const CapContext* c, RenderPlan& p)
{
    const CapContext::Lane& L   = c->lane[0];
    const BvhDev            bvh = bvh_dev(c, L);
    p.wave_ring = (p.inline_probe && p.ring_form && (size_t)((uint32_t)c->cu_count * p.blocks_per_cu) * (kBlock / 64) * 128 <= std::min(L.s_org.n, L.s_con.n)) ? 1u : 0u;
    p.camera_head = p.camera_table && p.wave_ring;
    const bool wide_tree = !p.fused && bvh.wide8_ok && c->tri_count > kExhaustiveMax;
    if (wide_tree && !p.ext)
    {
        const int force = (int)c->sw.v[SW_ANY_REFILL];
        const uint64_t tree_bytes = (uint64_t)c->wide8_nodes * kWideNodeStride * 4u + (uint64_t)c->tri_count * 64u;
        p.any_refill = force >= 0 ? force != 0 : tree_bytes >= kAnyRefillTreeBytes;
    }
    if (wide_tree)
    {
        const int force = (int)c->sw.v[SW_PRIMARY_WIDE];
        bool inside = true;
        for (int k = 0; k < 3; ++k)
            inside = inside && c->camera.position[k] >= c->bvh_info.bounds_lo[k] && c->camera.position[k] <= c->bvh_info.bounds_hi[k];
        const double per_pixel = (double)c->tri_count / std::max(1.0, (double)c->screen.width * c->screen.height);
        p.primary_wide = inside && (force >= 0 ? force != 0 : per_pixel >= kPrimaryWideTrianglesPerPixel);
    }
}

int upload_frame_constants(CapContext* c, const RenderPlan& p, uint32_t* ring_out)
{
    const uint32_t ring = *ring_out = c->frames_next;
    c->frames_next      = (c->frames_next + 1) % CapContext::kFrameRing;
    if (!c->frames_event[ring]) HIP_TRY(hipEventCreateWithFlags(&c->frames_event[ring], hipEventDisableTiming));
    HIP_TRY(hipEventSynchronize(c->frames_event[ring]));
    if (c->frames_ring[ring].n < p.n_frames)
    {
        HIP_TRY(c->frames_ring[ring].ensure(p.n_frames));
    }
    if (c->frames_pinned_n[ring] < p.n_frames)
    {
        if (c->frames_pinned[ring]) HIP_TRY(hipHostFree(c->frames_pinned[ring]));
        c->frames_pinned[ring] = nullptr;
        HIP_TRY(hipHostMalloc((void**)&c->frames_pinned[ring], sizeof(FrameConst) * p.n_frames, hipHostMallocDefault));
        c->frames_pinned_n[ring] = p.n_frames;
    }
    for (uint32_t f = 0; f < p.n_frames; ++f)
    {
        FrameConst& fc = c->frames_pinned[ring][f] = frame_const(p.frame_begin + f, p.lowres);
        if (p.camera_table) memcpy(&fc.pad1, &p.slot_group[f], 4), memcpy(&fc.pad2, &p.group_first[f], 4);
    }
    HIP_TRY(hipMemcpyAsync(c->frames_ring[ring].p, c->frames_pinned[ring], sizeof(FrameConst) * p.n_frames, hipMemcpyHostToDevice, c->stream));
    return CAP_OK;
}

struct BatchRun
{
    CapContext::Lane& L;
    BvhDev            bvh;
    LaunchCfg         cfg;
    CounterLayout     lay;
};

int fused_bounce(CapContext* c, const RenderPlan& p, const Batch& bt, const BatchRun& r, const ShadeArgs& sa, bool head)
{
    StageTimer     t(c, sa.bounce == 0 ? ST_PRIMARY : ST_CLOSEST, p.stage_timers);
    const uint32_t form = launch_trace_shade(r.cfg, r.bvh, sa, p.ext, p.feedback, head);
    if (sa.bounce) ++c->stats.launches_trace_closest, c->last_mark_form = form;
    if (trace_launch(c, "trace_shade bounce %u batch %u", sa.bounce, bt.index)) return fail(CAP_ERR_HIP, "trace_shade failed");
    return CAP_OK;
}

void tree_bounce(CapContext* c, const RenderPlan& p, const Batch& bt, const BatchRun& r, const ShadeArgs& sa)
{
    CapContext::Lane& L = r.L;
    const uint32_t    Ppad = c->screen.pixels_padded;
    bool              primary_shaded = false;
    if (sa.bounce == 0)
    {
        {
            StageTimer t(c, ST_PRIMARY, p.stage_timers);
            if (p.primary_wide)
            {
                const uint32_t id_cap = (((sa.max_count + kQueueClasses - 1) / kQueueClasses) + 63u) & ~63u;
                const RayQueue idq{L.q_org[0].p, L.q_dir[0].p, nullptr, r.lay.identity(L.counters.p), id_cap, nullptr};
                if (c->sw.on(SW_RAYGEN_KERNEL) || r.bvh.tri_count == 0)
                {
                    launch_raygen_identity(r.cfg, sa.cam, c->screen, bt.frames, bt.ns, idq);
                    launch_trace_closest8(r.cfg, r.bvh, idq, sa.max_count, L.hits.p, sa.work);
                }
                else
                    launch_trace_closest8_camera(r.cfg, r.bvh, idq, sa.max_count, L.hits.p, sa.work, sa.cam, c->screen, bt.frames, bt.ns);
            }
            else
            {
                primary_shaded = launch_primary_shade(r.cfg, r.bvh, sa, L.hits.p, p.ext);
                if (!primary_shaded) launch_trace_primary(r.cfg, r.bvh, sa.cam, c->screen, bt.frames, bt.ns, L.hits.p, sa.work);
            }
        }
        if (sa.aov_slot != ~0u) launch_geo_aov(r.cfg, sa.scene, L.hits.p + (size_t)sa.aov_slot * Ppad, Ppad, c->aov_geo.p);
    }
    if (!primary_shaded)
    {
        StageTimer t(c, ST_SHADE, p.stage_timers, sa.bounce == 0 ? ST_DIRECT : ST_NONE);
        launch_shade(r.cfg, sa, p.ext, p.feedback);
        ++c->stats.launches_shade;
    }
}

int shadow_rays(CapContext* c, const RenderPlan& p, const Batch& bt, const BatchRun& r, const ShadeArgs& sa)
{
    CapContext::Lane& L = r.L;
    const uint32_t    b = sa.bounce, Ppad = c->screen.pixels_padded;
    StageTimer        t(c, ST_ANY, p.stage_timers, b == 0 ? ST_DIRECT : ST_NONE);
    LaunchCfg         cfg_any = r.cfg;
    cfg_any.any_no_probe      = p.inline_probe;
    float4* const   plane = b == 0 ? L.pl_direct.p : L.pl_color.p;
    uint32_t* const work  = r.lay.work_any(L.counters.p, b);
    if (p.any_refill)
        launch_trace_any8_refill(cfg_any, r.bvh, sa.shadow, sa.max_count, plane, Ppad, bt.ns, c->shaded_counter.p, work, bt.frames);
    else
        launch_trace_any(cfg_any, r.bvh, sa.shadow, sa.max_count, plane, Ppad, bt.ns, c->shaded_counter.p, work,
                          p.ext, bt.frames, (b == 0 && p.code_in_color) ? L.pl_color.p : nullptr);
    ++c->stats.launches_trace_any;
    if (trace_launch(c, "trace_any bounce %u batch %u", b, bt.index)) return fail(CAP_ERR_HIP, "trace_any failed");
    return CAP_OK;
}

void tree_next_hits(CapContext* c, const RenderPlan& p, const BatchRun& r, const ShadeArgs& sa)
{
    StageTimer t(c, ST_CLOSEST, p.stage_timers);
    if (r.bvh.wide8_ok)
        launch_trace_closest8(r.cfg, r.bvh, sa.out, sa.max_count, r.L.hits.p, r.lay.work_shade(r.L.counters.p, sa.bounce + 1));
    else
        launch_trace_closest(r.cfg, r.bvh, sa.out, sa.max_count, r.L.hits.p);
    ++c->stats.launches_trace_closest;
}

int render_batch(CapContext* c, const RenderPlan& p, const Batch& bt, const ShadeArgs& call_args, hipEvent_t& last_resolve)
{
    CapContext::Lane& L    = c->lane[bt.lane];
    const uint32_t    Ppad = c->screen.pixels_padded, D = p.num_bounces, ns = bt.ns;
    BatchRun          r{L, bvh_dev(c, L), LaunchCfg{L.stream, (uint32_t)c->cu_count * p.blocks_per_cu, p.stack_entries, (uint32_t)c->cu_count},
               CounterLayout{D}};
    r.cfg.sw = &c->sw;
    HIP_TRY(hipMemsetAsync(L.counters.p, 0, sizeof(uint32_t) * 3 * r.lay.section(), L.stream));
    const uint32_t total_chunks   = ns * (Ppad >> 6);
    uint32_t       class_capacity = ((total_chunks + kQueueClasses - 1) / kQueueClasses) * 64u;
    if (c->debug_capacity_div > 1) class_capacity = std::max(64u, (class_capacity / c->debug_capacity_div) & ~63u);
    c->last_class_capacity = class_capacity;

    ShadeArgs sa = call_args;
    sa.frames    = bt.frames;
    if (!p.fused) sa.hits = L.hits.p;
    sa.planes = Planes{L.pl_color.p, L.pl_direct.p, L.pl_albedo.p, c->aov_geo.p, c->aov_nd.p};
    sa.n_slots = ns, sa.max_count = ns * Ppad, sa.aov_slot = (p.aov && bt.last) ? ns - 1 : ~0u;

    if (p.sample_table)
    {
        launch_sample_terms(L.stream, sa.scene.bluenoise, bt.frames, ns, D, L.terms.p);
        c->last_terms = CapContext::LastTerms{bt.frames, ns, D, bt.lane};
        if (trace_launch(c, "sample_terms batch %u", bt.index)) return fail(CAP_ERR_HIP, "sample_terms failed");
    }
    float4* const tab_p = L.camera.p, *const tab_n = L.camera.p + (size_t)bt.groups * Ppad;
    if (p.camera_head)
    {
        StageTimer t(c, ST_PRIMARY, p.stage_timers);
        launch_camera_vertices(r.cfg, r.bvh, sa, bt.groups, tab_p, tab_n);
        c->last_camera = CapContext::LastCamera{bt.frames, ns, bt.groups, bt.lane};
        ++c->stats.launches_trace_any;
        if (trace_launch(c, "camera_vertices batch %u", bt.index)) return fail(CAP_ERR_HIP, "camera_vertices failed");
    }
    c->last_camera_table = p.camera_head ? 1u : 0u;
    for (uint32_t b = p.camera_head ? 1u : 0u; b <= D; ++b)
    {
        const int pi = (int)(b & 1u), po = pi ^ 1;
        sa.bounce    = b;
        if (p.fused) sa.sample_terms = p.sample_table ? L.terms.p + (size_t)(b < D ? b : 0u) * ns * 4096 : nullptr;
        sa.in     = RayQueue{L.q_org[pi].p, L.q_dir[pi].p, L.q_thr[pi].p, b ? r.lay.ext(L.counters.p, b - 1) : nullptr, class_capacity, pi ? L.s_dir.p : L.s_org.p};
        sa.out    = RayQueue{L.q_org[po].p, L.q_dir[po].p, L.q_thr[po].p, r.lay.ext(L.counters.p, b), class_capacity, po ? L.s_dir.p : L.s_org.p};
        sa.shadow = ShadowQueue{L.s_org.p, L.s_dir.p, L.s_con.p, r.lay.shadow(L.counters.p, b), class_capacity};
        sa.work   = r.lay.work_shade(L.counters.p, b);
        const bool head = p.camera_head && b == 1;
        if (head) sa.in = RayQueue{tab_p, tab_n, L.terms.p, r.lay.ext(L.counters.p, 0), class_capacity, nullptr};
        if (p.fused)
        {
            if (int e = fused_bounce(c, p, bt, r, sa, head)) return e;
        }
        else
            tree_bounce(c, p, bt, r, sa);
        if (!p.inline_nee && !(p.fused && p.wave_ring && b != 0))
            if (int e = shadow_rays(c, p, bt, r, sa)) return e;
        if (!p.fused && b < D) tree_next_hits(c, p, r, sa);
    }
    if (!p.lowres)
    {
        StageTimer t(c, ST_RESOLVE, p.stage_timers);
        if (p.two_lanes && last_resolve) HIP_TRY(hipStreamWaitEvent(L.stream, last_resolve, 0));
        launch_resolve(r.cfg, sa.planes, ns, Ppad, c->accum.p, p.albedo_in_w != 0u, sa.scene.kd_untextured, p.code_in_color != 0u);
        if (p.two_lanes)
        {
            HIP_TRY(hipEventRecord(c->lane_ev[bt.lane], L.stream));
            last_resolve = c->lane_ev[bt.lane];
        }
    }
    uint32_t* pinned = nullptr;
    if (!c->pinned_pool.empty())
    {
        pinned = c->pinned_pool.back();
        c->pinned_pool.pop_back();
    }
    else
        HIP_TRY(hipHostMalloc((void**)&pinned, sizeof(uint32_t) * CounterLayout{255}.section(), hipHostMallocDefault));
    HIP_TRY(hipMemcpyAsync(pinned, L.counters.p, sizeof(uint32_t) * r.lay.section(), hipMemcpyDeviceToHost, L.stream));
    c->pending.push_back({pinned, BatchCounted{D, p.inline_nee == 0u}});
    HIP_TRY(hipGetLastError());

    c->stats.rays_primary += p.valid_pixels * ns;
    c->stats.frames += ns;
    if (!p.lowres) c->frames_accumulated += ns;
    c->last_slots = ns;
    c->aov_valid  = sa.aov_slot != ~0u;
    c->aov_lowres = p.lowres;
    c->aov_frame  = p.frame_begin + bt.first + ns - 1;
    return CAP_OK;
}
}

extern "C" int cap_render(CapContext* c, uint32_t frame_begin, uint32_t n_frames, uint32_t num_bounces, uint32_t flags)
{
    if (!c) return fail(CAP_ERR_INVALID_ARG, "cap_render: ctx is NULL");
    RenderPlan p;
    if (int e = plan_render(c, frame_begin, n_frames, num_bounces, flags, p)) return e;
    if (!p.n_batches) return CAP_OK;
    c->last_mark_form = 0, c->last_sample_table = p.sample_table ? 1u : 0u, c->last_cull_camera_pairs = p.cull_camera_pairs;
    c->last_terms = CapContext::LastTerms{}, c->last_camera_table = 0, c->last_camera = CapContext::LastCamera{};
    if (p.feedback && (c->post_w != c->screen.width || c->post_h != c->screen.height))
        if (int e = cap_post_reset(c)) return e;
    if (c->spans.size() > 2048 || c->pending.size() > 64 || c->post_marks.size() > 256)
        if (sync_and_collect(c) != CAP_OK) return CAP_ERR_HIP;
    if (int e = ensure_lanes(c, p)) return e;
    plan_forms(c, p);
    c->lanes_last_render = p.two_lanes ? 2u : 1u;
    uint32_t ring = 0;
    if (int e = upload_frame_constants(c, p, &ring)) return e;
    if (c->textures_dirty)
    {
        HIP_TRY(hipStreamSynchronize(c->stream));
        HIP_TRY(c->textures.ensure(std::max<size_t>(1, c->texture_host.size())));
        if (!c->texture_host.empty())
            HIP_TRY(hipMemcpy(c->textures.p, c->texture_host.data(), sizeof(TextureDev) * c->texture_host.size(), hipMemcpyHostToDevice));
        c->textures_dirty = false;
    }
    ShadeArgs call_args{};
    call_args.scene = scene_dev(c), call_args.cam = camera_dev(c->camera), call_args.screen = c->screen;
    call_args.num_bounces = num_bounces, call_args.shaded_counter = c->shaded_counter.p;
    call_args.cull_camera_pairs = p.cull_camera_pairs, call_args.albedo_in_w = p.albedo_in_w, call_args.code_in_color = p.code_in_color;
    call_args.inline_nee = p.inline_nee, call_args.inline_probe = p.inline_probe, call_args.wave_ring = p.wave_ring;
    if (p.feedback)
        call_args.fb = FeedbackDev{camera_dev(c->prev_camera), c->post_prev_nd.p, c->post_chist[(frame_begin + 1) % 2].p};
    std::unique_ptr<StageTimer> total(new StageTimer(c, ST_COUNT));

    struct LaneJoin
    {
        CapContext* c;
        bool        armed = false;
        ~LaneJoin()
        {
            if (!armed) return;
            if (hipEventRecord(c->join_ev, c->stream2) != hipSuccess || hipStreamWaitEvent(c->stream, c->join_ev, 0) != hipSuccess)
                (void)hipStreamSynchronize(c->stream2);
        }
    } lane_join{c};
    if (p.two_lanes)
    {
        HIP_TRY(hipEventRecord(c->fork_ev, c->stream));
        HIP_TRY(hipStreamWaitEvent(c->stream2, c->fork_ev, 0));
        lane_join.armed = true;
    }
    hipEvent_t last_resolve = nullptr;
    for (uint32_t k = 0, done = 0; done < n_frames; done += p.slots, ++k)
    {
        const uint32_t ns = std::min(p.slots, n_frames - done);
        const Batch    bt{p.two_lanes ? ((p.n_batches - 1u - k) & 1u) : 0u,
                       done, ns, k, p.camera_head ? p.batch_groups[k] : 0u, done + ns >= n_frames, c->frames_ring[ring].p + done};
        if (int e = render_batch(c, p, bt, call_args, last_resolve)) return e;
        if (c->spans.size() > 4096)
        {
            total.reset();
            if (p.two_lanes) HIP_TRY(hipStreamSynchronize(c->stream2));
            if (sync_and_collect(c) != CAP_OK) return CAP_ERR_HIP;
            total.reset(new StageTimer(c, ST_COUNT));
        }
    }
    if (p.two_lanes)
    {
        HIP_TRY(hipEventRecord(c->join_ev, c->stream2));
        HIP_TRY(hipStreamWaitEvent(c->stream, c->join_ev, 0));
        lane_join.armed = false;
    }
    total.reset();
    HIP_TRY(hipEventRecord(c->frames_event[ring], c->stream));
    return CAP_OK;
}
```

### capsaicin_amd/csrc/kernels.hip

```cpp
#include "cap_exhaustive.h"
#include "cap_kernels.h"
#include "cap_reproject.h"
#include "cap_shade.h"
#include "cap_trace.h"
#include "cap_unscaled.h"
#include "cap_wide_trace.h"

#include <cassert>

namespace cap
{
template <int STACK>
__device__ __forceinline__ void traverse_closest(const BvhDev& bvh, const Ray& r, uint32_t* stack, float& best_t, float& best_u,
                                                 float& best_v, uint32_t& best_gid)
{
    best_t = r.tmax, best_u = 0.0f, best_v = 0.0f, best_gid = kInvalidId;
    if (bvh.tri_count == 0) return;
    int node = bvh.root;
    int sp   = 0;
    while (true)
    {
        if (node >= 0)
        {
            const float4 q0 = bvh.nodes[4 * node + 0], q1 = bvh.nodes[4 * node + 1], q2 = bvh.nodes[4 * node + 2],
// ... 807 lines not shown
    }
    uint32_t       gx     = (chunks + 3) / 4;
    if (gx > cfg.grid_blocks) gx = cfg.grid_blocks;
    if (gx == 0) gx = 1;
    const dim3 grid(gx, n_slots);
    BvhDev     b = bvh;
    b.wide8_ok   = 0;
    if (cfg.stack_entries == 0)
        hipLaunchKernelGGL(k_trace_primary<0>, grid, dim3(kBlock), 0, cfg.stream, b, cam, screen, frames, hits);
    else if (cfg.stack_entries <= 32)
        hipLaunchKernelGGL(k_trace_primary<32>, grid, dim3(kBlock), 0, cfg.stream, b, cam, screen, frames, hits);
    else
        hipLaunchKernelGGL(k_trace_primary<64>, grid, dim3(kBlock), 0, cfg.stream, b, cam, screen, frames, hits);
}

void launch_trace_closest(const LaunchCfg& cfg, const BvhDev& bvh, const RayQueue& q, uint32_t max_count, float4* hits)
{
    dim3 grid(queue_grid(cfg, max_count));
    if (cfg.stack_entries == 0)
        hipLaunchKernelGGL(k_trace_closest<0>, grid, dim3(kBlock), 0, cfg.stream, bvh, q, hits);
    else if (cfg.stack_entries <= 32)
    {
        grid.x = resident_grid<k_trace_closest_refill<32>>(cfg, grid.x);
        hipLaunchKernelGGL(k_trace_closest_refill<32>, grid, dim3(kBlock), 0, cfg.stream, bvh, q, hits);
    }
    else
    {
        grid.x = resident_grid<k_trace_closest_refill<64>>(cfg, grid.x);
        hipLaunchKernelGGL(k_trace_closest_refill<64>, grid, dim3(kBlock), 0, cfg.stream, bvh, q, hits);
    }
}

void launch_trace_any(const LaunchCfg& cfg, const BvhDev& bvh, const ShadowQueue& q, uint32_t max_count, float4* target,
                      uint32_t pixels_padded, uint32_t n_slots, uint64_t* guard, uint32_t* work, bool mostly_unoccluded,
                      const FrameConst* frames, float4* code_plane)
{
    assert(!code_plane || (cfg.stack_entries == 0 && !mostly_unoccluded));
    dim3         grid(queue_grid(cfg, max_count));
    const BvhDev bw = for_grid(bvh, grid.x);
    const uint32_t pre = (cfg.stack_entries == 0 && !mostly_unoccluded) ? pre_table_bytes(n_slots, bvh.fan_pair_count) : 0u;
    const bool     no_probe = cfg.sw_on(SW_NO_ANY_PROBE);
    const uint32_t probe    = (uint32_t)cfg.sw_get(SW_ANY_PROBE, CAP_ANY_PROBE);
    if (pre != 0u && work && !no_probe && !cfg.any_no_probe && bvh.fan_pair_count <= kExhaustiveMax / 2)
    {
        const uint32_t per_cu = (uint32_t)cfg.sw_get(SW_ANY_BLOCKS, 6);
        uint32_t g = (max_count + kBlock - 1) / kBlock;
        const uint32_t cap = cfg.cu_count ? cfg.cu_count * per_cu : cfg.grid_blocks;
        g = g > cap ? cap : (g ? g : 1u);
        grid = dim3(g);
        const auto kernel = code_plane ? k_trace_any_small<true> : k_trace_any_small<false>;
        hipLaunchKernelGGL(kernel, grid, dim3(kBlock), pre, cfg.stream, bw, q, target, pixels_padded, n_slots, guard, work, frames, probe, code_plane);
        return;
    }
#define CAP_LAUNCH_ANY(S, R, ...) \
    hipLaunchKernelGGL((k_trace_any<S, R, ##__VA_ARGS__>), grid, dim3(kBlock), pre, cfg.stream, bw, q, target, pixels_padded, n_slots, guard, work, frames, pre, code_plane)
    if (cfg.stack_entries == 0)
    {
        if (mostly_unoccluded)
            CAP_LAUNCH_ANY(0, true);
        else if (code_plane)
            CAP_LAUNCH_ANY(0, false, true);
        else
            CAP_LAUNCH_ANY(0, false);
    }
    else if (bw.wide8_ok)
    {
        if (mostly_unoccluded) CAP_LAUNCH_ANY((int)kWideLdsEntries, true); else CAP_LAUNCH_ANY((int)kWideLdsEntries, false);
    }
    else if (cfg.stack_entries <= 32)
    {
        if (mostly_unoccluded) CAP_LAUNCH_ANY(32, true); else CAP_LAUNCH_ANY(32, false);
    }
    else
    {
        if (mostly_unoccluded) CAP_LAUNCH_ANY(64, true); else CAP_LAUNCH_ANY(64, false);
    }
#undef CAP_LAUNCH_ANY
}

template <bool FIRST_, bool EXT_, bool FB_ = false>
struct ShadeStageCfg
{
    static constexpr bool FIRST = FIRST_, EXT = EXT_, FB = FB_;
    static constexpr bool CARRY = false, SKY_RMW = true, PROBE = false, TAME = false, LEAN = false, CODE = false, TAB = false;
};

template <bool FIRST, bool EXT, bool FB = false>
__global__ __launch_bounds__(kBlock) void k_shade(ShadeArgs a)
{
    using C = ShadeStageCfg<FIRST, EXT, FB>;
    const uint32_t Ppad = a.screen.pixels_padded;
    const uint32_t chunks   = FIRST ? (Ppad >> 6) : (a.in.class_capacity >> 6) * kQueueClasses;
    uint32_t       n_shaded = 0;
    __shared__ FrameConst lds_frames[kMaxFrameSlots];
    stage_frames(a, lds_frames);
    Stamps st;
    st.start();
    for (uint32_t chunk = wave_global_id(); chunk < chunks; chunk += wave_total())
    {
        uint32_t i, klass;
        bool     active;
        if (FIRST)
        {
            i      = chunk * 64 + (threadIdx.x & 63u);
            active = true;
            klass  = chunk_class(blockIdx.y * (Ppad >> 6) + chunk);
        }
        else
            active = queue_chunk(a.in.count, a.in.class_capacity, chunk, threadIdx.x & 63u, i, klass);
        uint32_t pid = 0;
        float4   hit = make_float4(0.f, 0.f, u2f(kInvalidId), 0.f);
        v3       thr = mk3(1.0f, 1.0f, 1.0f);
        if (active)
        {
            if (FIRST)
            {
                pid = (blockIdx.y << kPidShift) | i;
                hit = a.hits[(size_t)blockIdx.y * Ppad + i];
            }
            else
            {
                const float4 tp = a.in.thr_pid[i];
                thr = mk3(tp.x, tp.y, tp.z), pid = f2u(tp.w);
                hit = a.hits[i];
            }
        }
        const ShadePre pre = shade_prefetch<C>(a, lds_frames, active, pid);
        if constexpr (EXT)
        {
            v3 d = mk3(0.f, 0.f, 1.f);
            if (active)
            {
                if (FIRST)
                {
                    uint32_t x, y;
                    if (local_pixel_to_xy(a.screen, i, x, y)) d = primary_dir(a.cam, a.screen, a.frames[blockIdx.y], x, y);
                }
                else
                {
                    const float4 dq = a.in.dir_tmax[i];
                    d               = mk3(dq.x, dq.y, dq.z);
                }
            }
            shade_vertex_ext<FIRST>(a, a.scene.shade_tris, pre, klass, pid, hit, thr, d, n_shaded);
        }
        else
            shade_vertex<C>(a, a.scene.shade_tris, pre, klass, pid, hit, thr, n_shaded, st);
    }
    flush_stats(a.out.count + (size_t)(wave_global_id() % kQueueClasses) * kCounterStride, n_shaded);
}

#ifndef CAP_PS_BLOCKS
#define CAP_PS_BLOCKS 8
#endif
template <bool EXT>
__global__ __launch_bounds__(kBlock, CAP_PS_BLOCKS) void k_primary_shade(BvhDev bvh, ShadeArgs a, float4* hits_out)
{
    using C = ShadeStageCfg<true, EXT>;
    __shared__ uint32_t   lds_wstack[(kBlock / 64) * kPacketStack];
    __shared__ FrameConst lds_frames[kMaxFrameSlots];
    stage_frames(a, lds_frames);
    uint32_t*      wstack   = lds_wstack + (threadIdx.x >> 6) * kPacketStack;
    const uint32_t Ppad     = a.screen.pixels_padded;
    const uint32_t cps      = Ppad >> 6;
    const uint32_t chunks   = cps * a.n_slots;
    const uint32_t my_class = wave_global_id() % kQueueClasses;
    uint32_t       n_shaded = 0;
// ... 118 lines not shown
```

### capsaicin_amd/csrc/small_scene.hip

```cpp
#include "cap_shade.h"

#include <algorithm>
#include <cassert>

namespace cap
{
#ifndef CAP_TS_FIRST
#define CAP_TS_FIRST 5
#endif
#ifndef CAP_TS_EXT
#define CAP_TS_EXT 6
#endif
#ifndef CAP_TS_NEXT
#define CAP_TS_NEXT 6
#endif
#ifdef CAP_STAMPS
__device__ unsigned long long g_wave_times[2 * 16384];
#endif
template <bool FIRST_, bool EXT_, bool FB_, bool LDS_, bool TAME_, bool CODE_ = false, bool TAB_ = false, bool HEAD_ = false>
struct TraceShadeCfg
{
    static_assert(!TAME_ || (!EXT_ && !FB_ && LDS_), "TAME: reference model, scene in LDS");
    static_assert(!CODE_ || (FIRST_ && TAME_), "CODE: bounce 0 of the reference model, scene in LDS, tame records");
    static_assert(!TAB_ || (TAME_ && kChunkLean), "TAB: the lean kernels (reference model, scene in LDS, tame records)");
    static_assert(!HEAD_ || (TAB_ && !FIRST_), "HEAD: the lean bounce >= 1 kernel with the sample table");
    static constexpr bool FIRST = FIRST_, EXT = EXT_, FB = FB_, LDS = LDS_, TAME = TAME_, CODE = CODE_, TAB = TAB_, HEAD = HEAD_;
    static constexpr bool CARRY = !EXT && !TAB, SKY_RMW = false;
    static constexpr bool PROBE = !EXT && !FB && LDS;
    static constexpr bool LEAN = PROBE && TAME && kChunkLean;
    static constexpr bool ORG  = FIRST && LDS;
    static constexpr bool XT   = EXT && LDS;
    static constexpr int  kBlocksPerCu = FB ? 4 : (EXT ? (FIRST ? 5 : CAP_TS_EXT) : (FIRST ? CAP_TS_FIRST : CAP_TS_NEXT));
};

__device__ __forceinline__ void stage_scene_records(const BvhDev& bvh, const ShadeArgs& a, float4* lds_shade, float4* lds_rec)
{
    const uint32_t n = bvh.tri_count <= kExhaustiveMax ? bvh.tri_count : kExhaustiveMax;
    for (uint32_t k = threadIdx.x; k < kShadeRec * n; k += kBlock) lds_shade[k] = a.scene.shade_tris[k];
    for (uint32_t k = threadIdx.x; k < 4 * n; k += kBlock) lds_rec[k] = bvh.tris_by_id[k];
}
__device__ __forceinline__ void stage_ext_tables(const ShadeArgs& a, float* lds_mat, float* lds_lcdf, float4* lds_lrec)
{
    const float* ms = reinterpret_cast<const float*>(a.scene.materials);
    for (uint32_t k = threadIdx.x; k < 12u * a.scene.material_count; k += kBlock) lds_mat[k] = ms[k];
    for (uint32_t k = threadIdx.x; k < a.scene.light_count; k += kBlock)
    {
        lds_lcdf[k] = a.scene.light_cdf[k];
        const float4* lt = a.scene.shade_tris + kShadeRec * (size_t)a.scene.light_tris[k];
        const float4  l0 = lt[0], l1 = lt[1], l2 = lt[2];
        const v3      q0 = mk3(l0.x, l0.y, l0.z), q1 = mk3(l1.x, l1.y, l1.z), q2 = mk3(l2.x, l2.y, l2.z);
        const v3      nl = normalize3(cross3(q1 - q0, q2 - q0));
        const MaterialDev lm = a.scene.materials[f2u(lt[6].x)];
        lds_lrec[4 * k]     = make_float4(q0.x, q0.y, q0.z, lm.ke[0]);
        lds_lrec[4 * k + 1] = make_float4(q1.x, q1.y, q1.z, lm.ke[1]);
        lds_lrec[4 * k + 2] = make_float4(q2.x, q2.y, q2.z, lm.ke[2]);
        lds_lrec[4 * k + 3] = make_float4(nl.x, nl.y, nl.z, 0.f);
    }
}
__device__ __forceinline__ void stage_camera_pairs(const BvhDev& bvh, const ShadeArgs& a, float4* lds_org, float4* lds_bounds)
{
    const v3     o  = mk3(a.cam.position[0], a.cam.position[1], a.cam.position[2]);
    const float* fp = reinterpret_cast<const float*>(bvh.fan_pairs);
    for (uint32_t k = threadIdx.x; k < bvh.fan_pair_count && 2 * k + 1 < kExhaustiveMax; k += kBlock)
    {
        const float* rec  = fp + 20 * (size_t)k;
        const v3     tvec = o - mk3(rec[0], rec[1], rec[2]);
        lds_org[2 * k]     = make_float4(tvec.x, tvec.y, tvec.z, dot3(tvec, mk3(rec[12], rec[13], rec[14])));
        lds_org[2 * k + 1] = make_float4(dot3(tvec, mk3(rec[15], rec[16], rec[17])), 0.f, 0.f, 0.f);
        const v3 R = mk3(a.cam.right[0], a.cam.right[1], a.cam.right[2]), U = mk3(a.cam.up[0], a.cam.up[1], a.cam.up[2]),
                 F = mk3(a.cam.forward[0], a.cam.forward[1], a.cam.forward[2]);
        float x0 = 3.0e38f, y0 = 3.0e38f, x1 = -3.0e38f, y1 = -3.0e38f;
        bool  behind = false;
        for (int e = 0; e < 4; ++e)
        {
            const v3    d = e == 0 ? tvec * -1.0f : (mk3(rec[3 * e], rec[3 * e + 1], rec[3 * e + 2]) - tvec);
            const float z = dot3(d, F);
            behind |= !(z > 1e-4f);
            const float px = ((a.cam.focal_length * dot3(d, R) / z) / a.cam.sensor_x + 0.5f) * (float)a.screen.width;
            const float py = ((a.cam.focal_length * dot3(d, U) / z) / a.cam.sensor_y + 0.5f) * (float)a.screen.height;
            x0 = fminf(x0, px), x1 = fmaxf(x1, px), y0 = fminf(y0, py), y1 = fmaxf(y1, py);
        }
        const bool usable = a.cull_camera_pairs != 0u && !behind && x0 == x0 && y0 == y0 && x1 == x1 && y1 == y1;
        lds_bounds[k] = usable ? make_float4(x0 - kCameraCullPad, y0 - kCameraCullPad, x1 + kCameraCullPad, y1 + kCameraCullPad) : make_float4(-3.0e38f, -3.0e38f, 3.0e38f, 3.0e38f);
    }
}
__device__ __forceinline__ void stage_probe_rows(const BvhDev& bvh, const ShadeArgs& a, float* lds_pscore, uint32_t& probe_k, float4* lds_probe)
{
    const uint32_t np = bvh.fan_pair_count;
    const float*   fp = reinterpret_cast<const float*>(bvh.fan_pairs);
    if (threadIdx.x < np)
    {
        const float* rec = fp + 20 * (size_t)threadIdx.x;
        const v3     L   = mk3(a.frames[0].light_dir[0], a.frames[0].light_dir[1], a.frames[0].light_dir[2]);
        const v3     v0  = mk3(rec[0], rec[1], rec[2]);
        float        sc  = dot3(v0, L);
        for (int e = 0; e < 3; ++e) sc += dot3(v0 + mk3(rec[3 + 3 * e], rec[4 + 3 * e], rec[5 + 3 * e]), L);
        lds_pscore[threadIdx.x] = sc;
    }
    __syncthreads();
    if (threadIdx.x < np)
    {
        const float sc   = lds_pscore[threadIdx.x];
        uint32_t    rank = 0;
        for (uint32_t j = 0; j < np; ++j)
        {
            const float o = lds_pscore[j];
            rank += (o > sc || (o == sc && j < threadIdx.x)) ? 1u : 0u;
        }
        if (rank == 0) probe_k = threadIdx.x;
    }
    __syncthreads();
    const float* rec = fp + 20 * (size_t)probe_k;
    for (uint32_t sl = threadIdx.x; sl < a.n_slots && sl < kMaxFrameSlots; sl += kBlock)
    {
        const v3 d = mk3(a.frames[sl].light_dir[0], a.frames[sl].light_dir[1], a.frames[sl].light_dir[2]);
        lds_probe[2 * sl]     = tri_pre(d, mk3(rec[12], rec[13], rec[14]), kRayEps, kRayFar);
        lds_probe[2 * sl + 1] = tri_pre(d, mk3(rec[15], rec[16], rec[17]), kRayEps, kRayFar);
    }
}

template <bool FIRST, bool EXT, bool FB = false, bool LDS = false, bool TAME = false, bool CODE = false>
__global__ __launch_bounds__(kBlock, (TraceShadeCfg<FIRST, EXT, FB, LDS, TAME, CODE>::kBlocksPerCu)) void k_trace_shade(BvhDev bvh, ShadeArgs a)
{
    using C            = TraceShadeCfg<FIRST, EXT, FB, LDS, TAME, CODE>;
    constexpr bool TAB = false;
#include "small_scene_body.h"
}
template <bool FIRST, bool CODE>
__global__ __launch_bounds__(kBlock, (TraceShadeCfg<FIRST, false, false, true, true, CODE, kChunkLean>::kBlocksPerCu)) void k_trace_shade_tab(BvhDev bvh, ShadeArgs a)
{
    using C            = TraceShadeCfg<FIRST, false, false, true, true, CODE, kChunkLean>;
    constexpr bool EXT = false, FB = false, LDS = true, TAB = kChunkLean;
#include "small_scene_body.h"
}

__global__ __launch_bounds__(kBlock, (TraceShadeCfg<false, false, false, true, true, false, kChunkLean, kChunkLean>::kBlocksPerCu)) void k_trace_shade_head(BvhDev bvh, ShadeArgs a)
{
    using C              = TraceShadeCfg<false, false, false, true, true, false, kChunkLean, kChunkLean>;
    constexpr bool FIRST = false, EXT = false, FB = false, LDS = true, TAB = kChunkLean;
#include "small_scene_body.h"
}

#ifdef CAP_STAMPS
extern "C" int cap_debug_stamps(unsigned long long* out, int reset)
{
    if (reset == 2) return (int)hipMemcpyFromSymbol(out, HIP_SYMBOL(g_wave_times), 2 * 16384 * sizeof(unsigned long long));
    hipError_t e = hipMemcpyFromSymbol(out, HIP_SYMBOL(g_stamps), 8 * sizeof(unsigned long long));
    if (e == hipSuccess && reset)
    {
        unsigned long long z[16] = {};
        e = hipMemcpyToSymbol(HIP_SYMBOL(g_stamps), z, sizeof(z));
    }
    return (int)e;
}
#endif

__device__ __forceinline__ uint32_t selftest_hash32(uint32_t x)
{
    x ^= x >> 16, x *= 0x7feb352du, x ^= x >> 15, x *= 0x846ca68bu, x ^= x >> 16;
    return x;
}
__global__ __launch_bounds__(kBlock) void k_shade_forms_selftest(unsigned long long* out, uint32_t which)
{
    const uint32_t     tid = blockIdx.x * kBlock + threadIdx.x, total = gridDim.x * kBlock;
    unsigned long long bad = 0, n = 0;
    auto               differ = [](float x, float y) { return f2u(x) != f2u(y) ? 1u : 0u; };
    if (which == 0)
    {
        for (uint64_t b = ((127ull - 96ull) << 23) + tid; b <= 0x7f7fffffull; b += total)
        {
            const float x = u2f((uint32_t)b), s = sqrtf(x);
            bad += differ(sqrt_pos(x), s) + differ(sqrt_unscaled(x), s), n += 2;
        }
        if (tid < 3)
        {
            const float x = tid == 0 ? 0.0f : (tid == 1 ? -0.0f : __builtin_inff());
            bad += differ(sqrt_unscaled(x), sqrtf(x)), ++n;
        }
        for (uint64_t b = (uint64_t)f2u(kNormLo) + tid; b <= f2u(kNormHi); b += total)
        {
            const float x = u2f((uint32_t)b);
            bad += differ(div_unscaled(1.0f, sqrt_pos(x)), 1.0f / sqrtf(x)), ++n;
        }
        for (uint64_t b = tid; b <= f2u(2.0f); b += total)
        {
            const float x = u2f((uint32_t)b), pdf = x / kPi, fast = div_unscaled(x, kPi);
            if (b == 0 || b >= ((127ull - 80ull) << 23))
                bad += differ(fast, pdf);
            else
                bad += (fast < 1e-5f && fast > -1e-5f) ? 0u : 1u;
            ++n;
            if (!(pdf < 1e-5f)) bad += differ(div_unscaled(kInvPi * fmaxf(x, 0.0f), pdf), (kInvPi * fmaxf(x, 0.0f)) / pdf), ++n;
        }
    }
    else
    {
        for (uint64_t i = tid; i < (1ull << 31); i += total)
        {
            const uint32_t h0 = selftest_hash32((uint32_t)i), h1 = selftest_hash32((uint32_t)i ^ 0x9e3779b9u), h2 = selftest_hash32(h0 + h1);
            const uint32_t e1 = 82u + h2 % 90u, d = (h2 >> 8) % 96u, e0 = e1 > d ? e1 - d : 1u;
            float          p = u2f((e1 << 23) | (h0 & 0x007fffffu) | ((h2 << 3) & 0x80000000u));
            float          q = u2f((e0 << 23) | (h1 & 0x007fffffu) | ((h2 << 2) & 0x80000000u));
            if ((h2 >> 24 & 7u) == 0u) q = (h2 & 0x08000000u) ? 0.0f : -0.0f;
            const bool  sw = (h2 >> 27 & 1u) != 0u;
            const float a = sw ? q : p, b = sw ? p : q, g = fmaf(a, a, b * b);
            if (!ortho_in_range(a, b, g)) continue;
            const float k = sqrtf(g), kf = sqrt_pos(g);
            float       qa, qb;
            div2_unscaled(a, b, kf, qa, qb);
            bad += differ(kf, k) + differ(qa, a / k) + differ(qb, b / k), ++n;
        }
    }
    if (bad) atomicAdd(&out[0], bad);
    atomicAdd(&out[1], n);
}

void launch_shade_forms_selftest(hipStream_t stream, unsigned long long* out_device, uint32_t which)
{
    hipLaunchKernelGGL(k_shade_forms_selftest, dim3(4096), dim3(kBlock), 0, stream, out_device, which);
}

// ... 45 lines not shown

__device__ __forceinline__ void camera_vertex(const BvhDev& bvh, const ShadeArgs& a, const FrameConst& fc, uint32_t i, const float4* lds_shade,
                                              const float4* lds_rec, const float4* lds_org, const float4* lds_bounds, float4& cp, float4& cn)
{
    const uint32_t lane = threadIdx.x & 63u;
    Ray            r    = make_ray(mk3(0.f, 0.f, 0.f), mk3(0.f, 0.f, 1.f), 0.0f, 0.0f);
    uint32_t       x, y;
    const bool     valid = local_pixel_to_xy(a.screen, i, x, y);
    if (valid) r = make_ray(mk3(a.cam.position[0], a.cam.position[1], a.cam.position[2]), primary_dir(a.cam, a.screen, fc, x, y), 0.0f, kPrimaryFar);
    uint32_t tx = 0, ty = 0;
    (void)local_pixel_to_xy(a.screen, i & ~63u, tx, ty);
    const float4   b    = lds_bounds[lane < kExhaustiveMax / 2 ? lane : 0u];
    const bool     over = lane < bvh.fan_pair_count && b.x < (float)(tx + 8u) && b.z >= (float)tx && b.y < (float)(ty + 8u) && b.w >= (float)ty;
    const uint32_t pair_mask = (uint32_t)__ballot(over);
    float          t, u, v;
    uint32_t       gid;
    exhaustive_closest<true, false>(bvh, lds_rec, r, t, u, v, gid, lds_org, pair_mask);
    cp = make_float4(0.f, 0.f, 0.f, kCodePadding), cn = make_float4(0.f, 0.f, 0.f, 0.f);
    if (valid && gid == kInvalidId)
        cp.w = kCodeSky;
    else if (valid)
    {
        const float4* tab = lds_shade + kShadeRec * (size_t)gid;
        const float4  s0 = tab[0], s1 = tab[1], s2 = tab[2], s3 = tab[3], s4 = tab[4], s5 = tab[5];
        const float   w = (1.0f - u) - v;
        auto          mix = [&](float c0, float c1, float c2) { return fmaf(c2, v, fmaf(c1, u, c0 * w)); };
        const v3      nm = mk3(mix(s3.x, s4.x, s5.x), mix(s3.y, s4.y, s5.y), mix(s3.z, s4.z, s5.z));
        const v3      n  = normalize3_tame(nm);
        const v3      p  = mk3(mix(s0.x, s1.x, s2.x), mix(s0.y, s1.y, s2.y), mix(s0.z, s1.z, s2.z));
        const float   kd = a.scene.kd_untextured;
        cp = make_float4(p.x, p.y, p.z, kd < 1e-5f ? kCodeBlack : kCodeKd);
        cn = make_float4(n.x, n.y, n.z, 0.0f);
    }
}
template <bool SELFTEST>
__global__ __launch_bounds__(kBlock) void k_camera_vertices(BvhDev bvh, ShadeArgs a, uint32_t rows, float4* tab_p, float4* tab_n, unsigned long long* out)
{
    __shared__ float4 lds_shade[kShadeRec * kExhaustiveMax];
    __shared__ float4 lds_rec[4 * kExhaustiveMax];
    __shared__ float4 lds_org[kExhaustiveMax];
    __shared__ float4 lds_bounds[kExhaustiveMax / 2];
    stage_scene_records(bvh, a, lds_shade, lds_rec);
    stage_camera_pairs(bvh, a, lds_org, lds_bounds);
    __syncthreads();
    const uint32_t Ppad = a.screen.pixels_padded, cps = Ppad >> 6, chunks = cps * rows, lane = threadIdx.x & 63u;
    unsigned long long bad = 0, n = 0;
    for (uint32_t chunk = wave_global_id(); chunk < chunks; chunk += gridDim.x * (kBlock / 64))
    {
        const uint32_t   row = chunk / cps, i = (chunk - row * cps) * 64 + lane;
        const FrameConst fc  = a.frames[SELFTEST ? row : f2u(a.frames[row].pad2)];
        float4           cp, cn;
        camera_vertex(bvh, a, fc, i, lds_shade, lds_rec, lds_org, lds_bounds, cp, cn);
        const size_t at = (size_t)(SELFTEST ? f2u(fc.pad1) : row) * Ppad + i;
        if (!SELFTEST)
            tab_p[at] = cp, tab_n[at] = cn;
        else
        {
            const float4 qp = tab_p[at], qn = tab_n[at];
            const bool   differ = f2u(qp.x) != f2u(cp.x) || f2u(qp.y) != f2u(cp.y) || f2u(qp.z) != f2u(cp.z) || f2u(qp.w) != f2u(cp.w) ||
                                f2u(qn.x) != f2u(cn.x) || f2u(qn.y) != f2u(cn.y) || f2u(qn.z) != f2u(cn.z) || f2u(qn.w) != f2u(cn.w);
            bad += (unsigned long long)__popcll(__ballot(differ)), n += 64ull;
        }
    }
    if (SELFTEST && lane == 0u)
    {
        if (bad) atomicAdd(&out[0], bad);
        if (n) atomicAdd(&out[1], n);
    }
}

void launch_camera_vertices(const LaunchCfg& cfg, const BvhDev& bvh, const ShadeArgs& args, uint32_t rows, float4* tab_p, float4* tab_n,
                            unsigned long long* selftest_out)
{
    assert(bvh.tri_count <= kExhaustiveMax && args.scene.shade_tame != 0 && args.scene.texture_count == 0);
    const uint32_t chunks = (args.screen.pixels_padded >> 6) * rows;
    if (!chunks) return;
    const uint32_t gx = std::max(1u, std::min(cfg.grid_blocks, (chunks + kBlock / 64 - 1) / (kBlock / 64)));
    if (selftest_out)
        hipLaunchKernelGGL(k_camera_vertices<true>, dim3(gx), dim3(kBlock), 0, cfg.stream, bvh, args, rows, tab_p, tab_n, selftest_out);
    else
        hipLaunchKernelGGL(k_camera_vertices<false>, dim3(gx), dim3(kBlock), 0, cfg.stream, bvh, args, rows, tab_p, tab_n, selftest_out);
}

enum : uint32_t { TS_FIRST = 1, TS_EXT = 2, TS_FB = 4, TS_LDS = 8, TS_TAME = 16, TS_CODE = 32, TS_TAB = 64, TS_HEAD = 128 };
struct TraceShadeKernel
{
    uint32_t is;
    void (*kernel)(BvhDev, ShadeArgs);
};
template <uint32_t IS>
constexpr TraceShadeKernel trace_shade_kernel()
{
    if constexpr ((IS & TS_HEAD) != 0)
    {
        static_assert(IS == (TS_LDS | TS_TAME | TS_TAB | TS_HEAD), "HEAD: the lean bounce >= 1 kernel");
        return {IS, k_trace_shade_head};
    }
    else if constexpr ((IS & TS_TAB) != 0)
    {
        static_assert((IS & ~(TS_FIRST | TS_CODE)) == (TS_LDS | TS_TAME | TS_TAB), "TAB: the lean kernels");
        return {IS, k_trace_shade_tab<(IS & TS_FIRST) != 0, (IS & TS_CODE) != 0>};
    }
    else
        return {IS, k_trace_shade<(IS & TS_FIRST) != 0, (IS & TS_EXT) != 0, (IS & TS_FB) != 0, (IS & TS_LDS) != 0, (IS & TS_TAME) != 0, (IS & TS_CODE) != 0>};
}
constexpr TraceShadeKernel kTraceShadeKernels[17] = {
    trace_shade_kernel<TS_FIRST | TS_LDS | TS_TAME | TS_CODE>(),
    trace_shade_kernel<TS_FIRST | TS_EXT | TS_LDS>(), trace_shade_kernel<TS_FIRST | TS_EXT>(),
    trace_shade_kernel<TS_FIRST | TS_LDS | TS_TAME>(), trace_shade_kernel<TS_FIRST | TS_LDS>(), trace_shade_kernel<TS_FIRST>(),
    trace_shade_kernel<TS_EXT | TS_LDS>(), trace_shade_kernel<TS_EXT>(),
    trace_shade_kernel<TS_FB | TS_LDS>(), trace_shade_kernel<TS_FB>(),
    trace_shade_kernel<TS_LDS | TS_TAME>(), trace_shade_kernel<TS_LDS>(), trace_shade_kernel<0>(),
    trace_shade_kernel<TS_FIRST | TS_LDS | TS_TAME | TS_CODE | TS_TAB>(), trace_shade_kernel<TS_FIRST | TS_LDS | TS_TAME | TS_TAB>(), trace_shade_kernel<TS_LDS | TS_TAME | TS_TAB>(),
    trace_shade_kernel<TS_LDS | TS_TAME | TS_TAB | TS_HEAD>(),
};

static bool tame_kernels(const BvhDev& bvh, const SceneDev& scene)
{
#if defined(CAP_SHADE_IEEE)
    return false;
#else
    return bvh.tri_count <= kExhaustiveMax && scene.shade_tame != 0;
#endif
}
bool trace_shade_has_code_form(const BvhDev& bvh, const SceneDev& scene) { return tame_kernels(bvh, scene); }
bool trace_shade_has_table_form(const BvhDev& bvh, const SceneDev& scene) { return kChunkLean && tame_kernels(bvh, scene); }

uint32_t launch_trace_shade(const LaunchCfg& cfg, const BvhDev& bvh, const ShadeArgs& args, bool ext, bool feedback, bool camera_head)
{
    const bool first = args.bounce == 0;
    const bool fb    = feedback && !ext && !first;
    const bool lds   = bvh.tri_count <= kExhaustiveMax;
    const bool tame  = !ext && !fb && tame_kernels(bvh, args.scene);
    const bool code  = first && args.code_in_color != 0u;
    assert(!code || tame);
    const bool tab = args.sample_terms != nullptr;
    assert(!tab || (tame && kChunkLean));
    assert(!camera_head || (args.bounce == 1 && tab && args.inline_probe && args.wave_ring && args.in.org_tmin && args.in.dir_tmax && args.in.thr_pid));
    const uint32_t is = (first ? TS_FIRST : 0u) | (ext ? TS_EXT : 0u) | (fb ? TS_FB : 0u) | (lds ? TS_LDS : 0u) | (tame ? TS_TAME : 0u) | (code ? TS_CODE : 0u) | (tab ? TS_TAB : 0u) |
                        (camera_head ? TS_HEAD : 0u);
    const uint32_t gx = queue_grid(cfg, (first || camera_head) ? args.screen.pixels_padded * args.n_slots : args.max_count);
    const TraceShadeKernel* k = kTraceShadeKernels;
    while (k->is != is && k + 1 < kTraceShadeKernels + 17) ++k;
    assert(k->is == is);
    hipLaunchKernelGGL(k->kernel, dim3(gx), dim3(kBlock), 0, cfg.stream, bvh, args);
#if defined(CAP_CLOSEST_V1)
    return 0u;
#else
    if (!lds || first) return 0u;
    return (kMarkCarry && bvh.tri_ids_dense) ? (bvh.tri_count > 32u ? 3u : 2u) : 1u;
#endif
}
}
```

### capsaicin_amd/csrc/small_scene_body.h

```cpp
    const uint32_t Ppad     = a.screen.pixels_padded;
    const uint32_t cps      = Ppad >> 6;
    const uint32_t chunks   = (FIRST || C::HEAD) ? cps * a.n_slots : (a.in.class_capacity >> 6) * kQueueClasses;
    uint32_t       n_shaded = 0, n_probed = 0;
    uint32_t       head_ext = 0, head_shadow = 0, head_probed = 0, head_shaded = 0;
    __shared__ FrameConst lds_frames[kMaxFrameSlots];
    __shared__ float4     lds_shade[LDS ? kShadeRec * kExhaustiveMax : 1];
    __shared__ float4     lds_rec[LDS ? 4 * kExhaustiveMax : 1];
    __shared__ float4     lds_probe[C::PROBE ? 2 * kMaxFrameSlots : 1];
    __shared__ float      lds_pscore[C::PROBE ? kExhaustiveMax / 2 : 1];
    __shared__ SlotSample lds_first[(C::LEAN && FIRST && !TAB) ? kMaxFrameSlots : 1];
    __shared__ uint32_t   lds_probe_k;
    __shared__ float4     lds_ring[(C::PROBE && !FIRST) ? (kBlock / 64) * kWaveRing : 1];
    __shared__ float4     lds_org[C::ORG ? kExhaustiveMax : 1];
    __shared__ float4     lds_bounds[C::ORG ? kExhaustiveMax / 2 : 1];
    __shared__ float      lds_mat[C::XT ? 12 * kExhaustiveMax : 1];
    __shared__ float      lds_lcdf[C::XT ? kExtLightsMax : 1];
    __shared__ float4     lds_lrec[C::XT ? 4 * kExtLightsMax : 1];
    const bool            ext_tabs = C::XT && a.scene.material_count <= kExhaustiveMax && a.scene.light_count <= kExtLightsMax;
    if (LDS)
    {
        stage_scene_records(bvh, a, lds_shade, lds_rec);
        if (C::XT && ext_tabs) stage_ext_tables(a, lds_mat, lds_lcdf, lds_lrec);
        if (C::ORG) stage_camera_pairs(bvh, a, lds_org, lds_bounds);
    }
    if (C::PROBE && a.inline_probe) stage_probe_rows(bvh, a, lds_pscore, lds_probe_k, lds_probe);
    if constexpr (C::LEAN)
        stage_frames_samples<FIRST, TAB>(a, lds_frames, lds_first);
    else
        stage_frames(a, lds_frames);
    ProbeArgs probe;
    if (C::PROBE && a.inline_probe) probe.rows = lds_probe, probe.pairs = bvh.fan_pairs, probe.k = lds_probe_k;
    uint32_t ring_head = 0, ring_n = 0;
    if (C::PROBE && !FIRST && a.inline_probe && a.wave_ring)
    {
        probe.ring_org = lds_ring + (threadIdx.x >> 6) * kWaveRing;
        probe.ring_con = a.shadow.contrib_pid + (size_t)wave_global_id() * kWaveRing;
    }
    auto trace_ring = [&](uint32_t count) {
        wave_handoff();
        const uint32_t lane_ = threadIdx.x & 63u;
        const bool     on    = lane_ < count;
        const uint32_t pos   = (ring_head + lane_) & (kWaveRing - 1u);
        float4         o     = make_float4(0.f, 0.f, 0.f, 0.f);
        if (on) o = probe.ring_org[pos];
        const uint32_t spid = f2u(o.w);
        const bool     good = on && (spid >> kPidShift) < a.n_slots && (spid & kPidMask) < Ppad;
        const FrameConst& fc = lds_frames[good ? (spid >> kPidShift) : 0u];
        const Ray  sr = make_ray(mk3(o.x, o.y, o.z), mk3(fc.light_dir[0], fc.light_dir[1], fc.light_dir[2]), kRayEps, good ? kRayFar : kRayEps);
        float4* const target = a.bounce == 0 ? a.planes.direct : a.planes.color;
        const size_t  idx    = good ? (size_t)(spid >> kPidShift) * Ppad + (spid & kPidMask) : 0;
        float4        c = make_float4(0.f, 0.f, 0.f, 0.f), cur = c;
        if (good) c = probe.ring_con[pos], cur = target[idx];
        const bool occluded = exhaustive_any<false>(bvh, sr);
        if constexpr (C::HEAD)
        {
            if (good && !occluded)
            {
                if (f2u(c.w) != 0u)
                {
                    a.planes.direct[idx] = make_float4(c.x, c.y, c.z, 0.0f);
                    reinterpret_cast<float*>(a.planes.color + idx)[3] = c.w + kCodeLit;
                }
                else
                {
                    float* const t3 = reinterpret_cast<float*>(a.planes.color + idx);
                    t3[0] = cur.x + c.x, t3[1] = cur.y + c.y, t3[2] = cur.z + c.z;
                }
            }
        }
        else if (good && !occluded) target[idx] = make_float4(cur.x + c.x, cur.y + c.y, cur.z + c.z, cur.w);
        ring_head = (ring_head + count) & (kWaveRing - 1u);
        ring_n -= count;
    };
    const float4* shade_tab = LDS ? lds_shade : a.scene.shade_tris;
    const float4* rec_tab   = LDS ? lds_rec : bvh.tris_by_id;
    ExtTables     xtabs;
    if (C::XT && ext_tabs) xtabs.materials = reinterpret_cast<const MaterialDev*>(lds_mat), xtabs.light_cdf = lds_lcdf, xtabs.light_rec = lds_lrec;
    Stamps st;
    st.start();
    const uint32_t my_class = wave_global_id() % kQueueClasses;
    const uint32_t lane     = threadIdx.x & 63u;
    uint32_t       n_class  = 0;
    if (!FIRST && !C::HEAD)
    {
        n_class = a.in.count[my_class * kCounterStride];
        n_class = n_class < a.in.class_capacity ? n_class : a.in.class_capacity;
    }
    uint32_t grab = grab_issue(a.work, my_class);
    while (true)
    {
        const uint32_t j = grab_value(grab);
        uint32_t       i, pid = 0, slot = 0;
        const uint32_t klass = my_class;
        bool           active;
        v3             thr = mk3(1.0f, 1.0f, 1.0f);
        Ray            r   = make_ray(mk3(0.f, 0.f, 0.f), mk3(0.f, 0.f, 1.f), 0.0f, 0.0f);
        float          carried_r1 = 0.f, carried_r2 = 0.f;
        if constexpr (C::HEAD)
        {
            const uint32_t chunk = class_chunk(j, my_class);
            if (chunk >= chunks) break;
            slot = chunk / cps;
            i    = (chunk - slot * cps) * 64 + lane;
            pid  = (slot << kPidShift) | i;
            const FrameConst& fc = lds_frames[slot];
            const size_t      at = (size_t)f2u(fc.pad1) * Ppad + i;
            const float4      cp = a.in.org_tmin[at], cn = a.in.dir_tmax[at];
            const uint32_t gt   = __umul24(i >> 6, a.screen.shard_count) + a.screen.shard_index;
            const uint32_t ty   = tile_div(gt, a.screen.tiles_x_mul, a.screen.tiles_x_shift);
            const uint32_t tx   = gt + (ty & 7u) * ((0u - a.screen.tiles_x) & 7u);
            const uint32_t base = ((ty & 7u) << 9) | ((i & 0x38u) << 3) | ((tx & 7u) << 3) | (i & 7u);
            const float4   q0   = a.in.thr_pid[(slot << 12) | base];
            grab = grab_issue(a.work, my_class);
            const v3 L = mk3(fc.light_dir[0], fc.light_dir[1], fc.light_dir[2]);
            const v3 I = mk3(fc.light_intensity[0], fc.light_intensity[1], fc.light_intensity[2]);
            a.planes.color[(size_t)slot * Ppad + i] = make_float4(0.f, 0.f, 0.f, cp.w);
            const bool vtx = cp.w == kCodeKd || cp.w == kCodeBlack, lit = cp.w == kCodeKd;
            const v3   p = mk3(cp.x, cp.y, cp.z), n = mk3(cn.x, cn.y, cn.z);
            bool       emit_shadow = false, emit_ext = false;
            v3         dir = unread3(), contrib = unread3();
            float      f = unread_f();
            if (lit)
            {
                const float kd  = a.scene.kd_untextured;
                const float ndl = fmaxf(0.0f, dot3(n, L));
                const v3    c   = mk3(((I.x * kd) * kInvPi) * ndl, ((I.y * kd) * kInvPi) * ndl, ((I.z * kd) * kInvPi) * ndl);
                if (c.x != 0.0f || c.y != 0.0f || c.z != 0.0f) emit_shadow = true, contrib = c;
                dir = hemisphere_dir_tame(n, [&] { return HemiTerms{q0.x, q0.y, q0.z}; });
                const float ndd = dot3(n, dir);
                const float pdf = div_unscaled(fmaxf(0.0f, ndd), kPi);
                if (!(pdf < 1e-5f))
                {
                    f        = 1.0f * div_unscaled(kInvPi * fmaxf(ndd, 0.0f), pdf);
                    emit_ext = true;
                }
            }
            const bool occluded0 = pair_occludes_pre(make_ray(p, L, kRayEps, kRayFar), probe.pairs, probe.k, probe.rows[2u * slot], probe.rows[2u * slot + 1u]);
            const bool probed0   = emit_shadow && occluded0;
            emit_shadow          = emit_shadow && !occluded0;
            const unsigned long long ms = __ballot(emit_shadow);
            head_shaded += (uint32_t)__popcll(__ballot(vtx)), head_probed += (uint32_t)__popcll(__ballot(probed0));
            head_ext += (uint32_t)__popcll(__ballot(emit_ext)), head_shadow += (uint32_t)__popcll(ms);
            if (emit_shadow)
            {
                const uint32_t pos  = (ring_head + ring_n + (uint32_t)__popcll(ms & ((1ull << lane) - 1ull))) & (kWaveRing - 1u);
                probe.ring_org[pos] = make_float4(p.x, p.y, p.z, u2f(pid));
                probe.ring_con[pos] = make_float4(contrib.x, contrib.y, contrib.z, kCodeKd);
            }
            ring_n += (uint32_t)__popcll(ms);
            __builtin_amdgcn_fence(__ATOMIC_RELEASE, "wavefront");
            if (ring_n >= 64u) trace_ring(64u);
            active = emit_ext;
            if (__ballot(active) == 0ull) continue;
            r   = make_ray(p, dir, kRayEps, kRayFar);
            thr = mk3(f, f, f);
        }
        else if (FIRST)
        {
            const uint32_t chunk = class_chunk(j, my_class);
            if (chunk >= chunks) break;
            grab   = grab_issue(a.work, my_class);
            slot   = chunk / cps;
            i      = (chunk - slot * cps) * 64 + lane;
            active = true;
            pid    = (slot << kPidShift) | i;
            uint32_t x, y;
            if (local_pixel_to_xy(a.screen, i, x, y))
                r = make_ray(mk3(a.cam.position[0], a.cam.position[1], a.cam.position[2]),
                             primary_dir(a.cam, a.screen, lds_frames[slot], x, y), 0.0f, kPrimaryFar);
        }
        else
        {
            if (j * 64u >= n_class) break;
            active = j * 64u + lane < n_class;
            if constexpr (C::LEAN)
            {
                const uint32_t local = j * 64u + lane;
                i                    = my_class * a.in.class_capacity + (local < n_class ? local : n_class - 1u);
                const float4 o = a.in.org_tmin[i], d = a.in.dir_tmax[i], tp = a.in.thr_pid[i];
                grab = grab_issue(a.work, my_class);
                r    = make_ray(mk3(o.x, o.y, o.z), mk3(d.x, d.y, d.z), kRayEps, kRayFar);
                thr  = mk3(tp.x, tp.y, tp.z), pid = f2u(tp.w);
                if (!TAB) carried_r1 = o.w, carried_r2 = d.w;
            }
            else
            {
                i      = my_class * a.in.class_capacity + j * 64u + lane;
                float4 o = make_float4(0.f, 0.f, 0.f, 0.f), d = make_float4(0.f, 0.f, 1.f, 0.f), tp = make_float4(1.f, 1.f, 1.f, 0.f);
                if (active) o = a.in.org_tmin[i], d = a.in.dir_tmax[i], tp = a.in.thr_pid[i];
                grab = grab_issue(a.work, my_class);
                if (active)
                {
                    r   = make_ray(mk3(o.x, o.y, o.z), mk3(d.x, d.y, d.z), kRayEps, kRayFar);
                    thr = mk3(tp.x, tp.y, tp.z), pid = f2u(tp.w);
                    carried_r1 = o.w, carried_r2 = d.w;
                }
            }
        }
        float    t, u, v;
        uint32_t gid;
        STAMP(st, 0, true);
        uint32_t pair_mask = ~0u;
        if (C::ORG)
        {
            uint32_t tx = 0, ty = 0;
            (void)local_pixel_to_xy(a.screen, i & ~63u, tx, ty);
            const float4 b    = lds_bounds[lane < kExhaustiveMax / 2 ? lane : 0u];
            const bool   over = lane < bvh.fan_pair_count && b.x < (float)(tx + 8u) && b.z >= (float)tx && b.y < (float)(ty + 8u) && b.w >= (float)ty;
            pair_mask         = (uint32_t)__ballot(over);
        }
        __builtin_amdgcn_s_setprio(0);
#if !defined(CAP_CLOSEST_V1)
        if constexpr (LDS && !C::ORG)
        {
            if (bvh.tri_count > 32u)
                exhaustive_closest_marked<true>(bvh, rec_tab, r, active, t, u, v, gid);
            else
                exhaustive_closest_marked<false>(bvh, rec_tab, r, active, t, u, v, gid);
        }
        else
#endif
            exhaustive_closest<C::ORG, !LDS>(bvh, rec_tab, r, t, u, v, gid, lds_org, pair_mask);
        __builtin_amdgcn_s_setprio(3);
        STAMP(st, 1, true);
        const ShadePre pre = shade_prefetch<C>(a, lds_frames, active, pid, carried_r1, carried_r2, lds_first);
        if (FIRST && slot == a.aov_slot)
        {
            float4 g = make_float4(0.f, 0.f, u2f(kInvalidId), u2f(kInvalidId));
            if (gid != kInvalidId)
            {
                const uint4 id = a.scene.tri_ids[gid];
                g              = make_float4(u, v, u2f(id.x), u2f(id.y));
            }
            a.planes.aov_geo[i] = g;
        }
        if constexpr (EXT)
        {
            if (a.inline_nee)
            {
                v3 acc = mk3(0.f, 0.f, 0.f);
                if (!FIRST && active)
                {
                    const float4 q = a.in.acc[i];
                    acc            = mk3(q.x, q.y, q.z);
                }
                shade_vertex_ext<FIRST, true>(a, shade_tab, pre, klass, pid, make_float4(u, v, u2f(gid), t), thr, r.d, n_shaded, &bvh, acc, xtabs);
            }
            else
                shade_vertex_ext<FIRST>(a, shade_tab, pre, klass, pid, make_float4(u, v, u2f(gid), t), thr, r.d, n_shaded, nullptr, mk3(0.f, 0.f, 0.f), xtabs);
        }
        else
        {
            shade_vertex<C>(a, shade_tab, pre, klass, pid, make_float4(u, v, u2f(gid), t), thr, n_shaded, st, probe, &n_probed, ring_head, &ring_n);
            if (C::PROBE && ring_n >= 64u) trace_ring(64u);
        }
        STAMP(st, 4, false);
    }
    if (!FIRST && !EXT && !FB) st.flush();
#ifdef CAP_STAMPS
    if (!FIRST && !EXT && !FB && (threadIdx.x & 63u) == 0 && wave_global_id() < 16384)
    {
        g_wave_times[2 * wave_global_id() + 0] = st.t_begin;
        g_wave_times[2 * wave_global_id() + 1] = __builtin_amdgcn_s_memrealtime();
    }
#endif
    if (C::PROBE && ring_n != 0u) trace_ring(ring_n);
    flush_stats(a.out.count + (size_t)my_class * kCounterStride, n_shaded, n_probed);
    if constexpr (C::HEAD)
    {
        unsigned long long* const line0 = reinterpret_cast<unsigned long long*>(a.in.count + (size_t)my_class * kCounterStride);
        if (lane == 0u && (head_ext | head_shadow)) atomicAdd(line0, ((unsigned long long)head_shadow << 32) | (unsigned long long)head_ext);
        if (lane == 0u && (head_probed | head_shaded)) atomicAdd(line0 + 1, ((unsigned long long)head_shaded << 32) | (unsigned long long)head_probed);
    }
```

### include/capsaicin_hip.h

```cpp
#ifndef CAPSAICIN_HIP_H
#define CAPSAICIN_HIP_H

#include <stddef.h>
#include <stdint.h>

#ifdef __cplusplus
extern "C" {
#endif

typedef struct CapContext CapContext;

typedef enum CapStatus
{
    CAP_OK                = 0,
    CAP_ERR_INVALID_ARG   = 1,
    CAP_ERR_HIP           = 2,
    CAP_ERR_STATE         = 3,
    CAP_ERR_UNSUPPORTED   = 4,
    CAP_ERR_IO            = 5
} CapStatus;

typedef struct CapCameraData
{
    float position[3];
// ... 78 lines not shown
    uint64_t shadow_entries;
    uint64_t shadow_entries_bounce0;
    uint64_t guard_append;
    uint64_t lane1_dropped;
} CapStats;

typedef struct CapBvhInfo
{
    uint32_t triangle_count;
    uint32_t node_count;
    uint32_t max_depth;
    uint32_t stack_entries;
    float    bounds_lo[3];
    float    bounds_hi[3];
    double   build_ms;
} CapBvhInfo;

const char* cap_last_error(void);
int cap_device_count(void);

int  cap_ctx_create(int device_id, void* hip_stream, CapContext** out_ctx);
void cap_ctx_destroy(CapContext* ctx);

int cap_scene_upload(CapContext* ctx, const float* positions, const float* normals, const float* texcoords,
                     const uint32_t* indices, const CapMeshDesc* meshes, uint32_t vertex_count, uint32_t index_count,
                     uint32_t mesh_count);
int cap_texture_upload(CapContext* ctx, uint32_t index, const uint8_t* rgba8, uint32_t width, uint32_t height);
int cap_bluenoise_upload(CapContext* ctx, const uint8_t* rgba8_256x256);
int cap_materials_upload(CapContext* ctx, const CapMaterial* materials, uint32_t mesh_count);

int cap_bvh_build(CapContext* ctx);
typedef enum CapBvhBuild
{
    CAP_BVH_BUILD_AUTO = 0,
    CAP_BVH_BUILD_LBVH = 1,
    CAP_BVH_BUILD_SAH  = 2,
    CAP_BVH_BUILD_PLOC = 3,
    CAP_BVH_BUILD_SAH_DEVICE = 4
} CapBvhBuild;
int cap_set_bvh_build(CapContext* ctx, uint32_t mode);
int cap_bvh_info(CapContext* ctx, CapBvhInfo* out);
int cap_bvh_readback(CapContext* ctx, float* nodes, uint32_t* leaf_triangles);
int cap_bvh_wide_readback(CapContext* ctx, uint32_t* nodes, uint32_t* tri_src, uint32_t* info);

enum
{
    CAP_VERTICES_DEVICE = 1u << 0
};
int cap_scene_update_vertices(CapContext* ctx, const float* positions, const float* normals, const float* texcoords, uint32_t flags);
typedef struct CapRefitInfo
{
    double ms;
    double expected_node_visits;
    double expected_node_visits_built;
} CapRefitInfo;
int cap_bvh_refit(CapContext* ctx, CapRefitInfo* out);

int cap_camera_set(CapContext* ctx, const CapCameraData* camera);
int cap_prev_camera_set(CapContext* ctx, const CapCameraData* camera);
int cap_set_resolution(CapContext* ctx, uint32_t width, uint32_t height);
int cap_set_shard(CapContext* ctx, uint32_t shard_index, uint32_t shard_count);
int cap_set_batch_paths(CapContext* ctx, uint64_t max_paths);
enum
{
    CAP_DEBUG_QUEUE_CAPACITY_DIV = 1,
    CAP_DEBUG_WIDE_DEPTH_LIMIT   = 2,
    CAP_DEBUG_WIDE_IN_USE        = 3,
    CAP_DEBUG_FAIL_LANE1         = 4,
    CAP_DEBUG_LANES_USED         = 5,
    CAP_DEBUG_QUEUE_CANARY_FILL   = 6,
    CAP_DEBUG_QUEUE_CANARY_BEHIND = 7,
    CAP_DEBUG_QUEUE_CANARY_USED   = 8,
    CAP_DEBUG_SELFTEST_DIV        = 9,
    CAP_DEBUG_NEE_PAIRS           = 10,
    CAP_DEBUG_SELFTEST_SHADE_UNARY = 11,
    CAP_DEBUG_SELFTEST_SHADE_DIV2  = 12,
    CAP_DEBUG_SHADE_TAME           = 13,
    CAP_DEBUG_CAMERA_CULL          = 14,
    CAP_DEBUG_MARK_FORM            = 15,
    CAP_DEBUG_SAMPLE_TABLE          = 16,
    CAP_DEBUG_SELFTEST_SAMPLE_TABLE = 17,
    CAP_DEBUG_CAMERA_TABLE          = 18,
    CAP_DEBUG_SELFTEST_CAMERA_TABLE = 19,
    CAP_DEBUG_SWITCH_BASE         = 64
};
int cap_debug_set(CapContext* ctx, uint32_t key, uint64_t value);
int cap_debug_get(CapContext* ctx, uint32_t key, uint64_t* value);
int cap_debug_switch_index(const char* name);
int cap_debug_pair_ids_dense(const float* pair_records, uint32_t pair_count, uint32_t single_count, uint32_t tri_count);
int cap_debug_query_ranges(uint64_t n, uint32_t count, const uint64_t* base, const uint64_t* stride, const uint32_t* align);
int cap_debug_closest_instance_bound(const float* transform, const float* box_lo, const float* box_hi, const float* point, float best_dist2,
                                     float* world_to_object, float* g, float* xw, float* slack, uint32_t* skip);
typedef enum CapTraversal
{
    CAP_TRAVERSAL_AUTO       = 0,
    CAP_TRAVERSAL_STACK      = 1,
    CAP_TRAVERSAL_EXHAUSTIVE = 2
} CapTraversal;
int cap_set_traversal(CapContext* ctx, uint32_t mode);

int cap_render(CapContext* ctx, uint32_t frame_begin, uint32_t n_frames, uint32_t num_bounces, uint32_t flags);
int cap_accum_reset(CapContext* ctx);
int cap_accum_import(CapContext* ctx, const float* sum_rgba, uint64_t frames);
int cap_sync(CapContext* ctx);

int cap_readback(CapContext* ctx, CapBufferKind kind, float* dst);

int cap_stats_get(CapContext* ctx, CapStats* out);
int cap_stats_reset(CapContext* ctx);

typedef struct CapRayDesc
{
    float origin[3];
    float tmin;
    float direction[3];
    float tmax;
} CapRayDesc;
typedef struct CapHit
{
    float    t;
    float    u;
    float    v;
    uint32_t triangle;
} CapHit;
int cap_trace_rays(CapContext* ctx, const CapRayDesc* device_rays, uint64_t n, CapHit* device_hits, uint32_t flags);
int cap_trace_occlusion(CapContext* ctx, const CapRayDesc* device_rays, uint64_t n, uint32_t* device_occluded, uint32_t flags);

#define CAP_MULTI_MAX_K 16
enum
{
    CAP_MULTI_CONTINUE = 1u << 0
};
int cap_trace_rays_multi(CapContext* ctx, const CapRayDesc* device_rays, uint64_t n, uint32_t k, CapHit* device_hits, uint32_t* device_counts,
                         uint32_t flags);

enum
{
    CAP_RAY_FLAG_ACCEPT_FIRST_HIT  = 0x04,
    CAP_RAY_FLAG_CULL_BACK_FACING  = 0x10,
    CAP_RAY_FLAG_CULL_FRONT_FACING = 0x20
};
typedef struct CapTraceOptions
{
    uint32_t ray_flags;
    uint32_t instance_mask;
    uint32_t reserved[2];
} CapTraceOptions;
int cap_scene_set_instance_masks(CapContext* ctx, const uint8_t* masks, uint32_t mesh_count);
int cap_trace_rays_ex(CapContext* ctx, const CapRayDesc* device_rays, uint64_t n, CapHit* device_hits, const CapTraceOptions* options);
int cap_trace_occlusion_ex(CapContext* ctx, const CapRayDesc* device_rays, uint64_t n, uint32_t* device_occluded,
                           const CapTraceOptions* options);
int cap_trace_rays_multi_ex(CapContext* ctx, const CapRayDesc* device_rays, uint64_t n, uint32_t k, CapHit* device_hits,
                            uint32_t* device_counts, uint32_t multi_flags, const CapTraceOptions* options);

typedef struct CapPointDesc
{
    float point[3];
    float radius;
} CapPointDesc;
typedef struct CapClosest
{
    float    point[3];
    float    dist2;
    float    u, v;
    uint32_t triangle;
    uint32_t feature;
// ... 190 lines not shown
```

Baseline: 61020 Mrays/s.

## Carry scalar gray throughput in 32-byte extension queue entries for untextured scenes

For untextured scenes on the lean sample-table path, path throughput is carried as a single float instead of an RGB vector. The scalar is packed into the origin's w and the pid into the direction's w, so extension queue entries drop from three float4 loads/stores to two. Sky contributions use atomic float adds rather than a read-modify-write. This cuts queue memory traffic and registers, but relies on kd being gray (kd.x used for all channels), which only holds when albedo is achromatic; a switch and a self-test are added to check it.

```diff
diff --git a/capsaicin_amd/capi.py b/capsaicin_amd/capi.py
--- a/capsaicin_amd/capi.py
+++ b/capsaicin_amd/capi.py
@@ -608,6 +608,8 @@
     DEBUG_SELFTEST_SAMPLE_TABLE = 17
     DEBUG_CAMERA_TABLE = 18
     DEBUG_SELFTEST_CAMERA_TABLE = 19
+    DEBUG_GRAY_ENTRIES = 20
+    DEBUG_SELFTEST_GRAY = 21
 
     def debug_set(self, key, value):
         _check(lib().cap_debug_set(self.ctx, key, value), "cap_debug_set")
diff --git a/capsaicin_amd/csrc/cap_context.h b/capsaicin_amd/csrc/cap_context.h
--- a/capsaicin_amd/csrc/cap_context.h
+++ b/capsaicin_amd/csrc/cap_context.h
@@ -217,6 +217,12 @@
         const FrameConst* frames = nullptr;
         uint32_t          n_slots = 0, n_groups = 0, lane = 0;
     } last_camera;
+    uint32_t      last_gray_entries = 0;
+    struct LastQueues
+    {
+        uint32_t num_bounces = 0, first_writer = 0, class_capacity = 0, lane = 0;
+        bool     valid = false;
+    } last_queues;
     uint32_t      last_cull_camera_pairs = 0;
     uint32_t      traversal_mode  = CAP_TRAVERSAL_AUTO;
     uint32_t      bvh_build_mode  = CAP_BVH_BUILD_AUTO;
diff --git a/capsaicin_amd/csrc/cap_kernels.h b/capsaicin_amd/csrc/cap_kernels.h
--- a/capsaicin_amd/csrc/cap_kernels.h
+++ b/capsaicin_amd/csrc/cap_kernels.h
@@ -38,6 +38,7 @@
     SW_NO_PLANE_CODE,
     SW_SAMPLE_TABLE,
     SW_NO_CAMERA_TABLE,
+    SW_NO_GRAY_ENTRIES,
     SW_COUNT
 };
 struct SwitchTable
@@ -254,9 +255,12 @@
 constexpr float kCameraCullPad = 2.0f;
 void launch_shade(const LaunchCfg& cfg, const ShadeArgs& args, bool ext, bool feedback = false);
 bool launch_primary_shade(const LaunchCfg& cfg, const BvhDev& bvh, const ShadeArgs& args, float4* hits, bool ext);
-uint32_t launch_trace_shade(const LaunchCfg& cfg, const BvhDev& bvh, const ShadeArgs& args, bool ext, bool feedback = false, bool camera_head = false);
+uint32_t launch_trace_shade(const LaunchCfg& cfg, const BvhDev& bvh, const ShadeArgs& args, bool ext, bool feedback = false, bool camera_head = false,
+                            bool gray = false);
 bool trace_shade_has_code_form(const BvhDev& bvh, const SceneDev& scene);
 bool trace_shade_has_table_form(const BvhDev& bvh, const SceneDev& scene);
+bool trace_shade_has_gray_form(const BvhDev& bvh, const SceneDev& scene);
+void launch_gray_selftest(hipStream_t stream, const RayQueue& q, unsigned long long* out_device);
 void launch_sample_terms(hipStream_t stream, const float2* bluenoise, const FrameConst* frames, uint32_t n_slots, uint32_t num_bounces, float4* table);
 void launch_sample_terms_selftest(hipStream_t stream, const float2* bluenoise, const FrameConst* frames, uint32_t n_slots, uint32_t num_bounces,
                                   const float4* table, unsigned long long* out_device);
diff --git a/capsaicin_amd/csrc/cap_shade.h b/capsaicin_amd/csrc/cap_shade.h
--- a/capsaicin_amd/csrc/cap_shade.h
+++ b/capsaicin_amd/csrc/cap_shade.h
@@ -154,6 +154,14 @@
     return base + (uint32_t)__popcll(mask & ((1ull << lane) - 1ull));
 }
 
+template <class T>
+__device__ __forceinline__ T thr_of(float x, float y, float z);
+template <>
+__device__ __forceinline__ v3 thr_of<v3>(float x, float y, float z) { return mk3(x, y, z); }
+template <>
+__device__ __forceinline__ float thr_of<float>(float x, float, float) { return x; }
+__device__ __forceinline__ v3 thr3(v3 thr) { return thr; }
+__device__ __forceinline__ v3 thr3(float thr) { return mk3(thr, thr, thr); }
 struct ShadePre
 {
     bool  valid;
@@ -401,7 +409,7 @@
 constexpr uint32_t kWaveRing = 128;
 template <class C>
 __device__ __forceinline__ void shade_vertex(const ShadeArgs& a, const float4* shade_tab, const ShadePre& pre, uint32_t klass,
-                                             uint32_t pid, float4 hit, v3 thr, uint32_t& n_shaded, Stamps& st,
+                                             uint32_t pid, float4 hit, typename C::Thr thr, uint32_t& n_shaded, Stamps& st,
                                              const ProbeArgs probe = ProbeArgs(), uint32_t* n_probed = nullptr, uint32_t ring_head = 0,
                                              uint32_t* ring_n = nullptr)
 {
@@ -439,7 +447,15 @@
             }
             else
             {
-                if (C::SKY_RMW)
+                if constexpr (C::GRAY)
+                {
+                    float*      c  = reinterpret_cast<float*>(a.planes.color + plane_idx);
+                    const float t7 = thr * 0.7f;
+                    atomicAdd(c + 0, t7);
+                    atomicAdd(c + 1, t7);
+                    atomicAdd(c + 2, thr * 0.85f);
+                }
+                else if (C::SKY_RMW)
                 {
                     const float4 cur = a.planes.color[plane_idx];
                     a.planes.color[plane_idx] = make_float4(cur.x + thr.x * 0.7f, cur.y + thr.y * 0.7f, cur.z + thr.z * 0.85f, cur.w);
@@ -516,7 +532,8 @@
                         reused        = true;
                         const v3 hc   = sample_bilinear(Img{a.fb.color_history, W, H}, puv);
                         const float4 cur = a.planes.color[plane_idx];
-                        a.planes.color[plane_idx] = make_float4(cur.x + thr.x * hc.x, cur.y + thr.y * hc.y, cur.z + thr.z * hc.z, cur.w);
+                        const v3     th  = thr3(thr);
+                        a.planes.color[plane_idx] = make_float4(cur.x + th.x * hc.x, cur.y + th.y * hc.y, cur.z + th.z * hc.z, cur.w);
                     }
                 }
             }
@@ -527,7 +544,10 @@
                 if (c.x != 0.0f || c.y != 0.0f || c.z != 0.0f)
                 {
                     emit_shadow = true;
-                    contrib     = C::FIRST ? c : thr * c;
+                    if constexpr (C::GRAY)
+                        contrib = C::FIRST ? c : c * thr;
+                    else
+                        contrib = C::FIRST ? c : thr * c;
                 }
                 const bool more = a.bounce < a.num_bounces;
                 if (!C::TAME || more)
@@ -543,7 +563,12 @@
                         const float fn = kInvPi * fmaxf(ndd, 0.0f);
                         const float f  = C::TAME ? div_unscaled(fn, pdf) : fn / pdf;
                         thr            = thr * f;
-                        if (!C::FIRST) thr = thr * kd;
+                        if constexpr (C::GRAY)
+                        {
+                            if (!C::FIRST) thr = thr * kd.x;
+                        }
+                        else if (!C::FIRST)
+                            thr = thr * kd;
                         emit_ext = more && (!C::FIRST || pre.indirect_on);
                     }
                 }
@@ -585,7 +610,15 @@
             a.shadow.org_tmin[si]    = make_float4(p.x, p.y, p.z, u2f(pid));
             a.shadow.contrib_pid[si] = make_float4(contrib.x, contrib.y, contrib.z, C::CODE ? kCodeKd : 0.0f);
         }
-        if (emit_ext)
+        if constexpr (C::GRAY)
+        {
+            if (emit_ext)
+            {
+                a.out.org_tmin[ei] = make_float4(p.x, p.y, p.z, thr);
+                a.out.dir_tmax[ei] = make_float4(dir.x, dir.y, dir.z, u2f(pid));
+            }
+        }
+        else if (emit_ext)
         {
             a.out.org_tmin[ei] = make_float4(p.x, p.y, p.z, C::CARRY ? pre.r1n : kRayEps);
             a.out.dir_tmax[ei] = make_float4(dir.x, dir.y, dir.z, C::CARRY ? pre.r2n : kRayFar);
diff --git a/capsaicin_amd/csrc/context.hip b/capsaicin_amd/csrc/context.hip
--- a/capsaicin_amd/csrc/context.hip
+++ b/capsaicin_amd/csrc/context.hip
@@ -255,7 +255,8 @@
     "CAP_NO_WIDE8", "CAP_LANE1_PRIORITY", "CAP_PLOC_RADIUS", "CAP_SAHDEV_LEAF", "CAP_WIDE_HOST_COLLAPSE", "CAP_TRACE_LAUNCHES", "CAP_NO_TWO_LANES",
     "CAP_LANE_SPLIT_MIN", "CAP_BLOCKS_PER_CU", "CAP_NO_CAMERA_CULL", "CAP_NO_ALBEDO_IN_W", "CAP_NO_INLINE_NEE", "CAP_NO_INLINE_PROBE", "CAP_NO_WAVE_RING",
     "CAP_ANY_REFILL", "CAP_PRIMARY_WIDE", "CAP_NO_PACKET", "CAP_NO_ANY_PROBE", "CAP_ANY_PROBE", "CAP_ANY_BLOCKS", "CAP_NO_PRIMARY_FUSE", "CAP_W8_REFILL",
-    "CAP_W8_GRID", "CAP_AUTO_SAH_TRIANGLES", "CAP_NO_NEE_PAIR_CULL", "CAP_RAYGEN_KERNEL", "CAP_NO_PLANE_CODE", "CAP_SAMPLE_TABLE", "CAP_NO_CAMERA_TABLE"};
+    "CAP_W8_GRID", "CAP_AUTO_SAH_TRIANGLES", "CAP_NO_NEE_PAIR_CULL", "CAP_RAYGEN_KERNEL", "CAP_NO_PLANE_CODE", "CAP_SAMPLE_TABLE", "CAP_NO_CAMERA_TABLE",
+    "CAP_NO_GRAY_ENTRIES"};
 
 static void switches_from_environment(SwitchTable& t)
 {
@@ -591,6 +592,27 @@
         *value = (h[0] << 32) | ((uint64_t)lc.n_groups << 16) | lc.n_slots;
         return CAP_OK;
     }
+    case CAP_DEBUG_GRAY_ENTRIES: *value = c->last_gray_entries; return CAP_OK;
+    case CAP_DEBUG_SELFTEST_GRAY:
+    {
+        const CapContext::LastQueues& lq = c->last_queues;
+        if (!lq.valid || c->last_gray_entries) return fail(CAP_ERR_STATE, "cap_debug_get: the last cap_render left no 48-byte extension queues (small-scene path, CAP_NO_GRAY_ENTRIES)");
+        HIP_TRY(hipSetDevice(c->device));
+        if (sync_and_collect(c) != CAP_OK) return CAP_ERR_HIP;
+        const CapContext::Lane& L = c->lane[lq.lane];
+        const CounterLayout     lay{lq.num_bounces};
+        unsigned long long      h[2];
+        if (int e = count_on_device(c, h, [&](unsigned long long* d) {
+                for (uint32_t back = 1; back <= 2 && back <= lq.num_bounces && lq.num_bounces - back >= lq.first_writer; ++back)
+                {
+                    const uint32_t b = lq.num_bounces - back, po = (b & 1u) ^ 1u;
+                    launch_gray_selftest(c->stream, RayQueue{L.q_org[po].p, L.q_dir[po].p, L.q_thr[po].p, lay.ext(L.counters.p, b), lq.class_capacity, nullptr}, d);
+                }
+            }))
+            return e;
+        *value = (h[0] << 32) | std::min<unsigned long long>(h[1], 0xffffffffull);
+        return CAP_OK;
+    }
     case CAP_DEBUG_NEE_PAIRS:
         if (!c->bvh_ready) return fail(CAP_ERR_STATE, "cap_debug_get: BVH not built");
         *value = ((uint64_t)(c->fan_pairs_nee.p ? c->fan_pair_nee_count : c->fan_pair_count) << 32) | c->fan_pair_count;
diff --git a/capsaicin_amd/csrc/ctx_render.hip b/capsaicin_amd/csrc/ctx_render.hip
--- a/capsaicin_amd/csrc/ctx_render.hip
+++ b/capsaicin_amd/csrc/ctx_render.hip
@@ -104,6 +104,7 @@
     uint32_t blocks_per_cu = 0;
     bool     sample_table = false;
     bool     camera_table = false;
+    bool     gray_entries = false;
     std::vector<uint32_t> slot_group, group_first, batch_groups;
     uint32_t camera_groups = 0;
     uint32_t cull_camera_pairs = 0, albedo_in_w = 0, code_in_color = 0, inline_nee = 0, inline_probe = 0;
@@ -267,6 +268,7 @@
     const BvhDev   bvh   = bvh_dev(c, c->lane[0]);
     const SceneDev scene = scene_dev(c);
     p.sample_table = fused && !ext && !feedback && num_bounces >= 1 && c->sw.get(SW_SAMPLE_TABLE, 1) != 0 && trace_shade_has_table_form(bvh, scene);
+    p.gray_entries = p.sample_table && trace_shade_has_gray_form(bvh, scene) && !c->sw.on(SW_NO_GRAY_ENTRIES);
     p.cull_camera_pairs = cull_camera_pairs(c) ? 1u : 0u;
     const bool no_albedo_w = c->sw.on(SW_NO_ALBEDO_IN_W);
     p.albedo_in_w = (!no_albedo_w && !feedback && !lowres && !p.aov && (ext || scene.texture_count == 0)) ? 1u : 0u;
@@ -388,7 +390,7 @@
 int fused_bounce(CapContext* c, const RenderPlan& p, const Batch& bt, const BatchRun& r, const ShadeArgs& sa, bool head)
 {
     StageTimer     t(c, sa.bounce == 0 ? ST_PRIMARY : ST_CLOSEST, p.stage_timers);
-    const uint32_t form = launch_trace_shade(r.cfg, r.bvh, sa, p.ext, p.feedback, head);
+    const uint32_t form = launch_trace_shade(r.cfg, r.bvh, sa, p.ext, p.feedback, head, p.gray_entries);
     if (sa.bounce) ++c->stats.launches_trace_closest, c->last_mark_form = form;
     if (trace_launch(c, "trace_shade bounce %u batch %u", sa.bounce, bt.index)) return fail(CAP_ERR_HIP, "trace_shade failed");
     return CAP_OK;
@@ -495,6 +497,7 @@
         if (trace_launch(c, "camera_vertices batch %u", bt.index)) return fail(CAP_ERR_HIP, "camera_vertices failed");
     }
     c->last_camera_table = p.camera_head ? 1u : 0u;
+    c->last_queues = CapContext::LastQueues{D, p.camera_head ? 1u : 0u, class_capacity, bt.lane, p.fused && !p.ext && !p.gray_entries};
     for (uint32_t b = p.camera_head ? 1u : 0u; b <= D; ++b)
     {
         const int pi = (int)(b & 1u), po = pi ^ 1;
@@ -558,6 +561,7 @@
     if (!p.n_batches) return CAP_OK;
     c->last_mark_form = 0, c->last_sample_table = p.sample_table ? 1u : 0u, c->last_cull_camera_pairs = p.cull_camera_pairs;
     c->last_terms = CapContext::LastTerms{}, c->last_camera_table = 0, c->last_camera = CapContext::LastCamera{};
+    c->last_gray_entries = p.gray_entries ? 1u : 0u, c->last_queues = CapContext::LastQueues{};
     if (p.feedback && (c->post_w != c->screen.width || c->post_h != c->screen.height))
         if (int e = cap_post_reset(c)) return e;
     if (c->spans.size() > 2048 || c->pending.size() > 64 || c->post_marks.size() > 256)
diff --git a/capsaicin_amd/csrc/kernels.hip b/capsaicin_amd/csrc/kernels.hip
--- a/capsaicin_amd/csrc/kernels.hip
+++ b/capsaicin_amd/csrc/kernels.hip
@@ -913,7 +913,8 @@
 struct ShadeStageCfg
 {
     static constexpr bool FIRST = FIRST_, EXT = EXT_, FB = FB_;
-    static constexpr bool CARRY = false, SKY_RMW = true, PROBE = false, TAME = false, LEAN = false, CODE = false, TAB = false;
+    static constexpr bool CARRY = false, SKY_RMW = true, PROBE = false, TAME = false, LEAN = false, CODE = false, TAB = false, GRAY = false;
+    using Thr = v3;
 };
 
 template <bool FIRST, bool EXT, bool FB = false>
diff --git a/capsaicin_amd/csrc/small_scene.hip b/capsaicin_amd/csrc/small_scene.hip
--- a/capsaicin_amd/csrc/small_scene.hip
+++ b/capsaicin_amd/csrc/small_scene.hip
@@ -2,6 +2,7 @@
 
 #include <algorithm>
 #include <cassert>
+#include <type_traits>
 
 namespace cap
 {
@@ -17,14 +18,16 @@
 #ifdef CAP_STAMPS
 __device__ unsigned long long g_wave_times[2 * 16384];
 #endif
-template <bool FIRST_, bool EXT_, bool FB_, bool LDS_, bool TAME_, bool CODE_ = false, bool TAB_ = false, bool HEAD_ = false>
+template <bool FIRST_, bool EXT_, bool FB_, bool LDS_, bool TAME_, bool CODE_ = false, bool TAB_ = false, bool HEAD_ = false, bool GRAY_ = false>
 struct TraceShadeCfg
 {
     static_assert(!TAME_ || (!EXT_ && !FB_ && LDS_), "TAME: reference model, scene in LDS");
     static_assert(!CODE_ || (FIRST_ && TAME_), "CODE: bounce 0 of the reference model, scene in LDS, tame records");
     static_assert(!TAB_ || (TAME_ && kChunkLean), "TAB: the lean kernels (reference model, scene in LDS, tame records)");
     static_assert(!HEAD_ || (TAB_ && !FIRST_), "HEAD: the lean bounce >= 1 kernel with the sample table");
-    static constexpr bool FIRST = FIRST_, EXT = EXT_, FB = FB_, LDS = LDS_, TAME = TAME_, CODE = CODE_, TAB = TAB_, HEAD = HEAD_;
+    static_assert(!GRAY_ || TAB_, "GRAY: the lean kernels with the sample table");
+    static constexpr bool FIRST = FIRST_, EXT = EXT_, FB = FB_, LDS = LDS_, TAME = TAME_, CODE = CODE_, TAB = TAB_, HEAD = HEAD_, GRAY = GRAY_;
+    using Thr = typename std::conditional<GRAY_, float, v3>::type;
     static constexpr bool CARRY = !EXT && !TAB, SKY_RMW = false;
     static constexpr bool PROBE = !EXT && !FB && LDS;
     static constexpr bool LEAN = PROBE && TAME && kChunkLean;
@@ -137,6 +140,20 @@
 __global__ __launch_bounds__(kBlock, (TraceShadeCfg<false, false, false, true, true, false, kChunkLean, kChunkLean>::kBlocksPerCu)) void k_trace_shade_head(BvhDev bvh, ShadeArgs a)
 {
     using C              = TraceShadeCfg<false, false, false, true, true, false, kChunkLean, kChunkLean>;
+    constexpr bool FIRST = false, EXT = false, FB = false, LDS = true, TAB = kChunkLean;
+#include "small_scene_body.h"
+}
+
+template <bool FIRST, bool CODE>
+__global__ __launch_bounds__(kBlock, (TraceShadeCfg<FIRST, false, false, true, true, CODE, kChunkLean, false, kChunkLean>::kBlocksPerCu)) void k_trace_shade_tab_gray(BvhDev bvh, ShadeArgs a)
+{
+    using C            = TraceShadeCfg<FIRST, false, false, true, true, CODE, kChunkLean, false, kChunkLean>;
+    constexpr bool EXT = false, FB = false, LDS = true, TAB = kChunkLean;
+#include "small_scene_body.h"
+}
+__global__ __launch_bounds__(kBlock, (TraceShadeCfg<false, false, false, true, true, false, kChunkLean, kChunkLean, kChunkLean>::kBlocksPerCu)) void k_trace_shade_head_gray(BvhDev bvh, ShadeArgs a)
+{
+    using C              = TraceShadeCfg<false, false, false, true, true, false, kChunkLean, kChunkLean, kChunkLean>;
     constexpr bool FIRST = false, EXT = false, FB = false, LDS = true, TAB = kChunkLean;
 #include "small_scene_body.h"
 }
@@ -348,7 +365,37 @@
         hipLaunchKernelGGL(k_camera_vertices<false>, dim3(gx), dim3(kBlock), 0, cfg.stream, bvh, args, rows, tab_p, tab_n, selftest_out);
 }
 
-enum : uint32_t { TS_FIRST = 1, TS_EXT = 2, TS_FB = 4, TS_LDS = 8, TS_TAME = 16, TS_CODE = 32, TS_TAB = 64, TS_HEAD = 128 };
+__global__ __launch_bounds__(kBlock) void k_gray_selftest(RayQueue q, unsigned long long* out)
+{
+    const uint32_t total = kQueueClasses * q.class_capacity;
+    unsigned long long bad = 0, n = 0;
+    for (uint32_t i = blockIdx.x * kBlock + threadIdx.x; i < total; i += gridDim.x * kBlock)
+    {
+        const uint32_t klass = i / q.class_capacity, local = i - klass * q.class_capacity;
+        const uint32_t count = q.count[klass * kCounterStride];
+        bool           in = local < (count < q.class_capacity ? count : q.class_capacity), differ = false;
+        if (in)
+        {
+            const float4 tp = q.thr_pid[i];
+            differ          = f2u(tp.x) != f2u(tp.y) || f2u(tp.x) != f2u(tp.z);
+        }
+        bad += (unsigned long long)__popcll(__ballot(differ)), n += (unsigned long long)__popcll(__ballot(in));
+    }
+    if ((threadIdx.x & 63u) == 0u)
+    {
+        if (bad) atomicAdd(&out[0], bad);
+        if (n) atomicAdd(&out[1], n);
+    }
+}
+
+void launch_gray_selftest(hipStream_t stream, const RayQueue& q, unsigned long long* out_device)
+{
+    if (!q.class_capacity) return;
+    const uint32_t total = kQueueClasses * q.class_capacity;
+    hipLaunchKernelGGL(k_gray_selftest, dim3(std::min(4096u, (total + kBlock - 1) / kBlock)), dim3(kBlock), 0, stream, q, out_device);
+}
+
+enum : uint32_t { TS_FIRST = 1, TS_EXT = 2, TS_FB = 4, TS_LDS = 8, TS_TAME = 16, TS_CODE = 32, TS_TAB = 64, TS_HEAD = 128, TS_GRAY = 256 };
 struct TraceShadeKernel
 {
     uint32_t is;
@@ -359,8 +406,14 @@
 {
     if constexpr ((IS & TS_HEAD) != 0)
     {
-        static_assert(IS == (TS_LDS | TS_TAME | TS_TAB | TS_HEAD), "HEAD: the lean bounce >= 1 kernel");
-        return {IS, k_trace_shade_head};
+        static_assert((IS & ~TS_GRAY) == (TS_LDS | TS_TAME | TS_TAB | TS_HEAD), "HEAD: the lean bounce >= 1 kernel");
+        return {IS, (IS & TS_GRAY) != 0 ? k_trace_shade_head_gray : k_trace_shade_head};
+    }
+    else if constexpr ((IS & TS_GRAY) != 0)
+    {
+        static_assert((IS & ~(TS_FIRST | TS_CODE)) == (TS_LDS | TS_TAME | TS_TAB | TS_GRAY), "GRAY: the lean kernels with the sample table");
+        static_assert((IS & TS_FIRST) != 0 || (IS & TS_CODE) == 0, "CODE: bounce 0");
+        return {IS, k_trace_shade_tab_gray<(IS & TS_FIRST) != 0, (IS & TS_CODE) != 0>};
     }
     else if constexpr ((IS & TS_TAB) != 0)
     {
@@ -370,7 +423,8 @@
     else
         return {IS, k_trace_shade<(IS & TS_FIRST) != 0, (IS & TS_EXT) != 0, (IS & TS_FB) != 0, (IS & TS_LDS) != 0, (IS & TS_TAME) != 0, (IS & TS_CODE) != 0>};
 }
-constexpr TraceShadeKernel kTraceShadeKernels[17] = {
+constexpr uint32_t         kTraceShadeKernelCount = 21;
+constexpr TraceShadeKernel kTraceShadeKernels[kTraceShadeKernelCount] = {
     trace_shade_kernel<TS_FIRST | TS_LDS | TS_TAME | TS_CODE>(),
     trace_shade_kernel<TS_FIRST | TS_EXT | TS_LDS>(), trace_shade_kernel<TS_FIRST | TS_EXT>(),
     trace_shade_kernel<TS_FIRST | TS_LDS | TS_TAME>(), trace_shade_kernel<TS_FIRST | TS_LDS>(), trace_shade_kernel<TS_FIRST>(),
@@ -379,6 +433,8 @@
     trace_shade_kernel<TS_LDS | TS_TAME>(), trace_shade_kernel<TS_LDS>(), trace_shade_kernel<0>(),
     trace_shade_kernel<TS_FIRST | TS_LDS | TS_TAME | TS_CODE | TS_TAB>(), trace_shade_kernel<TS_FIRST | TS_LDS | TS_TAME | TS_TAB>(), trace_shade_kernel<TS_LDS | TS_TAME | TS_TAB>(),
     trace_shade_kernel<TS_LDS | TS_TAME | TS_TAB | TS_HEAD>(),
+    trace_shade_kernel<TS_FIRST | TS_LDS | TS_TAME | TS_CODE | TS_TAB | TS_GRAY>(), trace_shade_kernel<TS_FIRST | TS_LDS | TS_TAME | TS_TAB | TS_GRAY>(),
+    trace_shade_kernel<TS_LDS | TS_TAME | TS_TAB | TS_GRAY>(), trace_shade_kernel<TS_LDS | TS_TAME | TS_TAB | TS_HEAD | TS_GRAY>(),
 };
 
 static bool tame_kernels(const BvhDev& bvh, const SceneDev& scene)
@@ -391,8 +447,9 @@
 }
 bool trace_shade_has_code_form(const BvhDev& bvh, const SceneDev& scene) { return tame_kernels(bvh, scene); }
 bool trace_shade_has_table_form(const BvhDev& bvh, const SceneDev& scene) { return kChunkLean && tame_kernels(bvh, scene); }
-
-uint32_t launch_trace_shade(const LaunchCfg& cfg, const BvhDev& bvh, const ShadeArgs& args, bool ext, bool feedback, bool camera_head)
+bool trace_shade_has_gray_form(const BvhDev& bvh, const SceneDev& scene) { return trace_shade_has_table_form(bvh, scene) && scene.texture_count == 0; }
+
+uint32_t launch_trace_shade(const LaunchCfg& cfg, const BvhDev& bvh, const ShadeArgs& args, bool ext, bool feedback, bool camera_head, bool gray)
 {
     const bool first = args.bounce == 0;
     const bool fb    = feedback && !ext && !first;
@@ -403,11 +460,12 @@
     const bool tab = args.sample_terms != nullptr;
     assert(!tab || (tame && kChunkLean));
     assert(!camera_head || (args.bounce == 1 && tab && args.inline_probe && args.wave_ring && args.in.org_tmin && args.in.dir_tmax && args.in.thr_pid));
+    assert(!gray || (tab && args.scene.texture_count == 0));
     const uint32_t is = (first ? TS_FIRST : 0u) | (ext ? TS_EXT : 0u) | (fb ? TS_FB : 0u) | (lds ? TS_LDS : 0u) | (tame ? TS_TAME : 0u) | (code ? TS_CODE : 0u) | (tab ? TS_TAB : 0u) |
-                        (camera_head ? TS_HEAD : 0u);
+                        (camera_head ? TS_HEAD : 0u) | (gray ? TS_GRAY : 0u);
     const uint32_t gx = queue_grid(cfg, (first || camera_head) ? args.screen.pixels_padded * args.n_slots : args.max_count);
     const TraceShadeKernel* k = kTraceShadeKernels;
-    while (k->is != is && k + 1 < kTraceShadeKernels + 17) ++k;
+    while (k->is != is && k + 1 < kTraceShadeKernels + kTraceShadeKernelCount) ++k;
     assert(k->is == is);
     hipLaunchKernelGGL(k->kernel, dim3(gx), dim3(kBlock), 0, cfg.stream, bvh, args);
 #if defined(CAP_CLOSEST_V1)
diff --git a/capsaicin_amd/csrc/small_scene_body.h b/capsaicin_amd/csrc/small_scene_body.h
--- a/capsaicin_amd/csrc/small_scene_body.h
+++ b/capsaicin_amd/csrc/small_scene_body.h
@@ -93,7 +93,7 @@
         uint32_t       i, pid = 0, slot = 0;
         const uint32_t klass = my_class;
         bool           active;
-        v3             thr = mk3(1.0f, 1.0f, 1.0f);
+        typename C::Thr thr = thr_of<typename C::Thr>(1.0f, 1.0f, 1.0f);
         Ray            r   = make_ray(mk3(0.f, 0.f, 0.f), mk3(0.f, 0.f, 1.f), 0.0f, 0.0f);
         float          carried_r1 = 0.f, carried_r2 = 0.f;
         if constexpr (C::HEAD)
@@ -153,7 +153,7 @@
             active = emit_ext;
             if (__ballot(active) == 0ull) continue;
             r   = make_ray(p, dir, kRayEps, kRayFar);
-            thr = mk3(f, f, f);
+            thr = thr_of<typename C::Thr>(f, f, f);
         }
         else if (FIRST)
         {
@@ -177,11 +177,21 @@
             {
                 const uint32_t local = j * 64u + lane;
                 i                    = my_class * a.in.class_capacity + (local < n_class ? local : n_class - 1u);
-                const float4 o = a.in.org_tmin[i], d = a.in.dir_tmax[i], tp = a.in.thr_pid[i];
-                grab = grab_issue(a.work, my_class);
-                r    = make_ray(mk3(o.x, o.y, o.z), mk3(d.x, d.y, d.z), kRayEps, kRayFar);
-                thr  = mk3(tp.x, tp.y, tp.z), pid = f2u(tp.w);
-                if (!TAB) carried_r1 = o.w, carried_r2 = d.w;
+                if constexpr (C::GRAY)
+                {
+                    const float4 o = a.in.org_tmin[i], d = a.in.dir_tmax[i];
+                    grab = grab_issue(a.work, my_class);
+                    r    = make_ray(mk3(o.x, o.y, o.z), mk3(d.x, d.y, d.z), kRayEps, kRayFar);
+                    thr  = thr_of<typename C::Thr>(o.w, o.w, o.w), pid = f2u(d.w);
+                }
+                else
+                {
+                    const float4 o = a.in.org_tmin[i], d = a.in.dir_tmax[i], tp = a.in.thr_pid[i];
+                    grab = grab_issue(a.work, my_class);
+                    r    = make_ray(mk3(o.x, o.y, o.z), mk3(d.x, d.y, d.z), kRayEps, kRayFar);
+                    thr  = thr_of<typename C::Thr>(tp.x, tp.y, tp.z), pid = f2u(tp.w);
+                    if (!TAB) carried_r1 = o.w, carried_r2 = d.w;
+                }
             }
             else
             {
@@ -192,7 +202,7 @@
                 if (active)
                 {
                     r   = make_ray(mk3(o.x, o.y, o.z), mk3(d.x, d.y, d.z), kRayEps, kRayFar);
-                    thr = mk3(tp.x, tp.y, tp.z), pid = f2u(tp.w);
+                    thr = thr_of<typename C::Thr>(tp.x, tp.y, tp.z), pid = f2u(tp.w);
                     carried_r1 = o.w, carried_r2 = d.w;
                 }
             }
@@ -244,10 +254,10 @@
                     const float4 q = a.in.acc[i];
                     acc            = mk3(q.x, q.y, q.z);
                 }
-                shade_vertex_ext<FIRST, true>(a, shade_tab, pre, klass, pid, make_float4(u, v, u2f(gid), t), thr, r.d, n_shaded, &bvh, acc, xtabs);
+                shade_vertex_ext<FIRST, true>(a, shade_tab, pre, klass, pid, make_float4(u, v, u2f(gid), t), thr3(thr), r.d, n_shaded, &bvh, acc, xtabs);
             }
             else
-                shade_vertex_ext<FIRST>(a, shade_tab, pre, klass, pid, make_float4(u, v, u2f(gid), t), thr, r.d, n_shaded, nullptr, mk3(0.f, 0.f, 0.f), xtabs);
+                shade_vertex_ext<FIRST>(a, shade_tab, pre, klass, pid, make_float4(u, v, u2f(gid), t), thr3(thr), r.d, n_shaded, nullptr, mk3(0.f, 0.f, 0.f), xtabs);
         }
         else
         {
diff --git a/include/capsaicin_hip.h b/include/capsaicin_hip.h
--- a/include/capsaicin_hip.h
+++ b/include/capsaicin_hip.h
@@ -184,6 +184,8 @@
     CAP_DEBUG_SELFTEST_SAMPLE_TABLE = 17,
     CAP_DEBUG_CAMERA_TABLE          = 18,
     CAP_DEBUG_SELFTEST_CAMERA_TABLE = 19,
+    CAP_DEBUG_GRAY_ENTRIES          = 20,
+    CAP_DEBUG_SELFTEST_GRAY         = 21,
     CAP_DEBUG_SWITCH_BASE         = 64
 };
 int cap_debug_set(CapContext* ctx, uint32_t key, uint64_t value);
```

Result: faster. 65550 Mrays/s, median of 6 (+7.4%).
